# Stylish-TTS/stylish-tts

Measured on AMD Instinct MI355X. Metric: audio frames/sec/GPU (24 kHz) forward+backward; DDP scaling 1/2/4/8 MI355X, higher is better.
Workload: dtype bf16 GEMM operands, f32 accumulation/storage; 1 GPU; c3: B=32/GPU T=520 frames (6.5 s) L=100

## Files before the change

include/stylish_hip.h:

```cpp
#ifndef STYLISH_HIP_H
#define STYLISH_HIP_H

#include <stddef.h>
#include <stdint.h>

#ifdef __cplusplus
extern "C" {
#endif

typedef enum {
  STY_OK = 0,
  STY_EINVAL = -1,
  STY_ESHAPE = -2,
  STY_EHIP = -3,
  STY_ENOMEM = -4,
  STY_ESTATE = -5
} sty_status;

typedef struct sty_model sty_model;

int sty_version(void);
const char *sty_last_error(void);

int sty_model_create(const char *kind, sty_model **out);
void sty_model_destroy(sty_model *m);
int sty_model_bind(sty_model *m, const char *key, const float *ptr, int ndim, const int64_t *shape);
int sty_model_finalize(sty_model *m);
int sty_model_num_keys(const sty_model *m);
const char *sty_model_key(const sty_model *m, int i);
int sty_model_prepare(sty_model *m, void *stream);
int sty_model_invalidate(sty_model *m);

typedef struct {
  int B, T;
  const float *mel, *style, *pitch, *voiced, *noise, *prior_override;
  uint64_t seed;
  float *audio;
  float *tap_conformer_out;
  float *tap_prior;
  float *tap_har_spec;
  float *tap_har_phase;
  float *tap_logamp_prior;
  float *tap_phase_prior;
  float *tap_trunk;
  float *tap_logamp;
} sty_vocoder_io;
int sty_vocoder_workspace_bytes(const sty_model *m, int B, int T, size_t *bytes);
int sty_vocoder_fwd(sty_model *m, const sty_vocoder_io *io, void *workspace, size_t ws_bytes, void *stream);

typedef struct {
  int B, L, T;
  const int64_t *texts, *text_lengths;
  const float *alignment, *pitch, *energy, *voiced, *style, *denormal_pitch, *noise, *prior_override;
  uint64_t seed;
  float *audio;
  float *tap_text_encoding;
  float *tap_decoder_out;
  sty_vocoder_io voc_taps;
  void *style_stream;
} sty_speech_io;
int sty_speech_workspace_bytes(const sty_model *m, int B, int L, int T, size_t *bytes);
int sty_speech_fwd(sty_model *m, const sty_speech_io *io, void *workspace, size_t ws_bytes, void *stream);

int sty_style_workspace_bytes(const sty_model *m, int B, int T, size_t *bytes);
int sty_style_fwd(sty_model *m, int B, int T, const float *mel, float *style, void *workspace, size_t ws_bytes,
                  void *stream);

int sty_mel_workspace_bytes(int B, int N, int n_fft, int hop, size_t *bytes);
int sty_mel_fwd(int B, int N, const float *audio, int n_fft, int win_length, int hop, float mean, float std,
                float *mel, float *energy, void *workspace, size_t ws_bytes, void *stream);

int sty_multispec_workspace_bytes(int B, int N, size_t *bytes);
int sty_multispec_fwd(int B, int N, const float *audio, float *const *mag, float *const *phase,
                      float *const *fft_mag, void *workspace, size_t ws_bytes, void *stream);

int sty_alignment_fwd(int B, int L, int T, const float *durations, float *alignment, void *stream);

int sty_duration_workspace_bytes(const sty_model *m, int B, int L, size_t *bytes);
int sty_duration_fwd(sty_model *m, int B, int L, const int64_t *texts, const int64_t *text_lengths, const float *style,
                     float *dur_pred, void *workspace, size_t ws_bytes, void *stream);
int sty_pitch_energy_workspace_bytes(const sty_model *m, int B, int L, int T, size_t *bytes);
int sty_pitch_energy_fwd(sty_model *m, int B, int L, int T, const int64_t *texts, const int64_t *text_lengths,
                         const float *alignment, const float *style, float *pitch, float *energy, void *workspace,
                         size_t ws_bytes, void *stream);

int sty_pitch_style_workspace_bytes(const sty_model *m, int B, int T, size_t *bytes);
int sty_pitch_style_fwd(sty_model *m, int B, int T, const float *mel, const float *pitch, const float *energy,
                        float *style, void *workspace, size_t ws_bytes, void *stream);

int sty_aligner_workspace_bytes(const sty_model *m, int B, int T, size_t *bytes);
int sty_aligner_fwd(sty_model *m, int B, int T, const float *mel, const int64_t *mel_lengths, float *log_probs,
                    void *workspace, size_t ws_bytes, void *stream);
int sty_forced_align_workspace_bytes(int B, int T, int U, size_t *bytes);
int sty_forced_align(int B, int T, int V1, int U, const float *log_probs, const int64_t *targets,
                     const int64_t *input_lengths, const int64_t *target_lengths, int blank, int32_t *labels,
                     float *scores, int32_t *status, void *workspace, size_t ws_bytes, void *stream);

int sty_aligner_train_workspace_bytes(sty_model *m, int B, int T, size_t *bytes);
int sty_aligner_fwd_train(sty_model *m, int B, int T, const float *mel, const int64_t *mel_lengths, float drop_p,
                          unsigned drop_seed, float *log_probs, void *workspace, size_t ws_bytes, void *stream);
int sty_aligner_bwd(sty_model *m, const float *d_logits, void *stream);
int sty_ctc_loss_workspace_bytes(int B, int T, int V1, int U, size_t *bytes);
int sty_ctc_loss_fwd_bwd(int B, int T, int V1, int U, const float *log_probs, const float *log_priors, float prior_scale,
                         const int64_t *targets, const int64_t *input_lengths, const int64_t *target_lengths, int blank,
                         float weight, double *nll, float *loss, int32_t *status, float *d_logits, void *workspace,
                         size_t ws_bytes, void *stream);

int sty_convnext_fwd(sty_model *m, const char *prefix, int B, int C, int T, const float *x, const float *style,
                     float *y, void *workspace, size_t ws_bytes, void *stream);
int sty_resblock_fwd(sty_model *m, const char *prefix, int B, int T, const float *x, const float *style, float *y,
                     void *workspace, size_t ws_bytes, void *stream);
int sty_block_train_workspace_bytes(sty_model *m, const char *kind, const char *prefix, int B, int C, int T,
                                    size_t *bytes);
int sty_block_fwd_bwd(sty_model *m, const char *kind, const char *prefix, int B, int C, int T, const float *x,
                      const float *style, const float *gy, float *y, float *gx, float *d_style, void *workspace,
                      size_t ws_bytes, void *stream);
int sty_attention_workspace_bytes(int B, int H, int T, size_t *bytes);
int sty_attention_fwd_bwd(int B, int H, int DH, int T, const float *q, const float *k, const float *v,
                          const int64_t *lengths, const float *d_o, float *o, float *dq, float *dk, float *dv,
                          void *workspace, size_t ws_bytes, void *stream);
int sty_stft64_fwd(int B, int N, const float *wave, float *spec, float *phase, void *stream);
void sty_stft64_bases_host(float *out);
int sty_istft64_fwd(int B, int F, const float *logamp, const float *real, const float *imag, float *audio,
                    void *stream);
int sty_source_fwd(int B, int T, const float *pitch, const float *voiced, const float *noise, uint64_t seed,
                   const float *lin_w, const float *lin_b, float *prior, void *workspace, size_t ws_bytes,
                   void *stream);
int sty_source_workspace_bytes(int B, int T, size_t *bytes);

int sty_model_enable_training(sty_model *m);
typedef struct {
  int bn_batch_stats;
  int sn_power_iter;
  int f0_smooth;
  int energy_smooth;
  float bn_momentum;
  unsigned dropout_seed;
  float text_dropout;
  int compute_bf16;
  int frozen;
  float block_dropout;
} sty_train_opts;
int sty_model_set_train_opts(sty_model *m, const sty_train_opts *opts);

typedef void (*sty_grad_hook)(void *user, int segment);
int sty_model_set_grad_hook(sty_model *m, sty_grad_hook hook, void *user);
int sty_model_bind_grad(sty_model *m, const char *key, float *grad);
int sty_vocoder_train_workspace_bytes(sty_model *m, int B, int T, size_t *bytes);
int sty_vocoder_fwd_train(sty_model *m, const sty_vocoder_io *io, void *workspace, size_t ws_bytes, void *stream);
int sty_vocoder_bwd(sty_model *m, const float *d_audio, float *d_mel, float *d_style, void *stream);
int sty_speech_train_workspace_bytes(sty_model *m, int B, int L, int T, size_t *bytes);
int sty_speech_fwd_train(sty_model *m, const sty_speech_io *io, void *workspace, size_t ws_bytes, void *stream);
int sty_speech_bwd(sty_model *m, const float *d_audio, float *d_style, float *d_energy, void *stream);
int sty_speech_prepare_train(sty_model *m, void *stream);
int sty_speech_bwd_pe(sty_model *m, const float *d_audio, float *d_style, float *d_pitch, float *d_energy, void *stream);
int sty_speech_d_style_ready(sty_model *m, void *stream);
int sty_speech_branch_stream(sty_model *m, void **stream);
int sty_style_train_workspace_bytes(sty_model *m, int B, int T, size_t *bytes);
int sty_style_fwd_train(sty_model *m, int B, int T, const float *mel, float *style, void *workspace, size_t ws_bytes,
                        void *stream);
int sty_style_bwd(sty_model *m, const float *d_style, void *stream);
int sty_style_prepare_train(sty_model *m, void *stream);
int sty_style_tap(sty_model *m, int index, int grad, float *dst, int *C, int *H, int *W, void *stream);
int sty_pitch_loss_fwd_bwd(int B, int T, const float *target, const float *pred, float weight, int normalize,
                           float *loss, float *d_pred, void *workspace, size_t ws_bytes, void *stream);
int sty_prediction_to_duration(int B, int L, int NC, const float *pred, const int64_t *text_lengths,
                               const float *class_table, float *duration, void *stream);
int sty_duration_loss_fwd_bwd(int B, int L, int NC, const float *pred, const int64_t *text_lengths,
                              const float *target_dur, const int64_t *target_class, const float *class_table,
                              const float *ce_weight, float w_duration, float w_ce, const float *d_duration_extra,
                              float *losses, float *d_pred, void *workspace, size_t ws_bytes, void *stream);
int sty_duration_train_workspace_bytes(sty_model *m, int B, int L, size_t *bytes);
int sty_duration_fwd_train(sty_model *m, int B, int L, const int64_t *texts, const int64_t *text_lengths,
                           const float *style, float *out, void *workspace, size_t ws_bytes, void *stream);
int sty_duration_bwd(sty_model *m, const float *d_out, float *d_style, void *stream);
int sty_pitch_energy_train_workspace_bytes(sty_model *m, int B, int L, int T, size_t *bytes);
int sty_pitch_energy_fwd_train(sty_model *m, int B, int L, int T, const int64_t *texts, const int64_t *text_lengths,
                               const float *alignment, const float *style, float *pitch, float *energy, void *workspace,
                               size_t ws_bytes, void *stream);
int sty_pitch_energy_bwd(sty_model *m, const float *d_pitch, const float *d_energy, float *d_style, void *stream);
int sty_pitch_style_train_workspace_bytes(sty_model *m, int B, int T, size_t *bytes);
int sty_pitch_style_fwd_train(sty_model *m, int B, int T, const float *mel, const float *pitch, const float *energy,
                              float *style, void *workspace, size_t ws_bytes, void *stream);

int sty_conv1d_workspace_bytes(int Cout, int Cin, int K, size_t *bytes);
int sty_conv1d_fwd(int B, int Cin, int Cout, int K, int dil, int T, const float *x, const float *w, const float *bias,
                   float *y, void *workspace, size_t ws_bytes, int compute_bf16, void *stream);
int sty_conv1d_bwd_workspace_bytes(int B, int Cin, int Cout, int K, int T, size_t *bytes);
int sty_conv1d_bwd(int B, int Cin, int Cout, int K, int dil, int T, const float *x, const float *w, const float *gy,
                   float *dw, float *dbias, float *dx, void *workspace, size_t ws_bytes, int compute_bf16,
                   void *stream);
int sty_partial_sum(int dw_form, const float *part, int C, int K, int nblk, float *dw, float *db, void *stream);

int sty_adamw_step(size_t n, float *p, const float *g, float *m, float *v, float lr, float beta1, float beta2,
                   float eps, float weight_decay, int step, float grad_scale, void *stream);
int sty_adamw_step_scaled(size_t n, float *p, const float *g, float *m, float *v, double lr, const double *lr_mult,
                          float beta1, float beta2, float eps, float weight_decay, int step, float grad_scale,
                          void *stream);
int sty_disc_lr_track(double *state, const float *loss, double ideal_loss, double f_max, double h_min, double x_max,
                      double x_min, void *stream);

int sty_acoustic_loss_workspace_bytes(int B, int N, size_t *bytes);
int sty_acoustic_loss_target(int B, int N, const float *audio_gt, void *workspace, size_t ws_bytes, void *stream);
int sty_acoustic_loss_fwd_bwd(int B, int N, const float *audio_gt, const float *audio_pred, float w_mel,
                              float w_phase, float *losses, float *d_audio_pred, void *workspace, size_t ws_bytes,
                              void *stream);

typedef struct {
  const float *g[10];
  const float *v[10];
  const float *bias[10];
} sty_specdisc_params;
typedef struct {
  float *g[10];
  float *v[10];
  float *bias[10];
} sty_specdisc_grads;
int sty_specdisc_workspace_bytes(int B, int H, int W, int with_grads, size_t *bytes);
int sty_specdisc_forward(const sty_specdisc_params *p, int B, int H, int W, const float *x, float *scores,
                         int compute_bf16, void *workspace, size_t ws_bytes, void *stream);
int sty_specdisc_losses(const sty_specdisc_params *p, int B, int H, int W, const float *target, const float *pred,
                        float gen_scale, float *gen_loss, float *d_pred, float disc_scale, float *disc_loss,
                        const sty_specdisc_grads *grads, int compute_bf16, void *workspace, size_t ws_bytes,
                        void *stream);

int sty_pitchdisc_workspace_bytes(int B, int dim_in, int kernel, int T, int with_grads, size_t *bytes);
int sty_pitchdisc_forward(const sty_specdisc_params *p, int B, int dim_in, int kernel, int T, const float *x,
                          float *scores, void *workspace, size_t ws_bytes, void *stream);
int sty_pitchdisc_losses(const sty_specdisc_params *p, int B, int dim_in, int kernel, int T, const float *target,
                         const float *pred, float gen_scale, float *gen_loss, float *d_pred, float disc_scale,
                         float *disc_loss, const sty_specdisc_grads *grads, void *workspace, size_t ws_bytes,
                         void *stream);

typedef struct {
  const float *conv_w[12];
  const float *conv_b[12];
  const float *bn_w[9];
  const float *bn_b[9];
  float *bn_rm[9];
  float *bn_rv[9];
} sty_cfdisc_params;
typedef struct {
  float *conv_w[12];
  float *conv_b[12];
  float *bn_w[9];
  float *bn_b[9];
} sty_cfdisc_grads;
int sty_cfdisc_workspace_bytes(int B, int N, int with_grads, size_t *bytes);
int sty_cfdisc_forward(const sty_cfdisc_params *p, int B, int N, const float *x, float *scores, float bn_momentum,
                       int compute_bf16, void *workspace, size_t ws_bytes, void *stream);
int sty_cfdisc_losses(const sty_cfdisc_params *p, int B, int N, const float *target, const float *pred, float gen_scale,
                      float *gen_loss, float *d_pred, float disc_scale, float *disc_loss, const sty_cfdisc_grads *grads,
                      float bn_momentum, int compute_bf16, void *workspace, size_t ws_bytes, void *stream);

int sty_acoustic_gan_workspace_bytes(int B, int N, int with_grads, size_t *bytes);
int sty_acoustic_gan_loss_fwd_bwd(int B, int N, const float *audio_gt, const float *audio_pred, float w_mel,
                                  float w_phase, float w_gen, const sty_specdisc_params *mrd, float disc_scale,
                                  const sty_specdisc_grads *mrd_grads, int step_mask, float *losses, float *gan_losses,
                                  float *d_audio_pred, void *workspace, size_t ws_bytes, void *gan_workspace,
                                  size_t gan_ws_bytes, int compute_bf16, void *stream);

typedef struct sty_comm sty_comm;
int sty_comm_unique_id(void *id128);
int sty_comm_init(const void *id128, int rank, int world, int stream_priority, sty_comm **out);
int sty_comm_allreduce_bucket(sty_comm *c, float *buf, size_t n, void *producer_stream);
int sty_comm_wait(sty_comm *c, void *consumer_stream);
int sty_comm_set_stream(sty_comm *c, void *stream);
int sty_comm_stats(sty_comm *c, uint64_t *buckets, uint64_t *reduce_scatter_all_gather, double *bytes);
int sty_comm_destroy(sty_comm *c);

int sty_pack_accumulate(int n, int D, int rows, const float *styles, const int64_t *text_lengths, double *sums,
                        int64_t *counts, void *stream);
int sty_pack_finalize(int rows, int D, const double *sums, const int64_t *counts, const int32_t *lo, const int32_t *hi,
                      float *pack, void *stream);

typedef struct {
  char name[48];
  char inst[144];
  uint64_t launches;
  double ms;
  double flops;
// ... 12 lines not shown
```

stylish_tts_amd/csrc/api.hip:

```cpp
#include <math.h>
#include <stdarg.h>
#include <string.h>
#include <stdlib.h>
#include <cxxabi.h>

#include <map>
#include <string>

#include "model.h"

namespace sty {

static thread_local char g_err[1024] = "";
void set_error(const char* fmt, ...) {
  va_list ap;
  va_start(ap, fmt);
  vsnprintf(g_err, sizeof(g_err), fmt, ap);
  va_end(ap);
}
int hip_fail(hipError_t e, const char* what) {
  set_error("HIP error %d (%s) at %s", (int)e, hipGetErrorString(e), what);
  return STY_EHIP;
}

// ... 2426 lines not shown
  PackedConv pc;
  pc.Cin = Cin;
  pc.Cout = Cout;
  pc.K = K;
  pc.CinP = (int)align_up(Cin, CI_CHUNK);
  pc.CoutP = (int)align_up(Cout, 32);
  float* wp = reinterpret_cast<float*>(align_up(reinterpret_cast<size_t>(workspace), 256));
  float* bp = wp + (size_t)K * pc.CinP * pc.CoutP;
  STY_HIP(hipMemsetAsync(wp, 0, ((size_t)K * pc.CinP * pc.CoutP + pc.CoutP) * sizeof(float), S(stream)));
  rc = launch_pack_conv(w, nullptr, nullptr, bias, Cout, Cin, K, wp, bp, pc.CinP, pc.CoutP, S(stream));
  if (rc) return rc;
  pc.wp = wp;
  pc.bias = bias ? bp : nullptr;
  ConvArgs a;
  a.x[0] = x;
  a.xc[0] = Cin;
  a.nsrc = 1;
  a.B = B;
  a.T = T;
  a.w = pc;
  a.dil = dil;
  a.pad = (K - 1) * dil / 2;
  a.y = y;
  a.bf16 = compute_bf16 != 0;
  if (compute_bf16 == 2) {
    const size_t tw = ((size_t)B * (Cin + Cout) * T) * sizeof(__bf16) + 512;
    if (ws_bytes < need + tw) {
      set_error("sty_conv1d_fwd: compute_bf16 = 2 needs %zu more workspace bytes for the operand twins", tw);
      return STY_EINVAL;
    }
    __bf16* x16 = reinterpret_cast<__bf16*>(align_up(reinterpret_cast<size_t>(static_cast<char*>(workspace) + need), 256));
    if ((rc = launch_twin_cast(x, nullptr, PRO_NONE, B, Cin, T, x16, S(stream)))) return rc;
    a.x16 = x16;
    a.y16 = x16 + (size_t)B * Cin * T;
    a.y16_act = PRO_LRELU;
  }
  return launch_conv1d(a, S(stream));
}
static PackedConv unit_conv_dims(int Cin, int Cout, int K) {
  PackedConv pc;
  pc.Cin = Cin;
  pc.Cout = Cout;
  pc.K = K;
  pc.CinP = (int)align_up(Cin, CI_CHUNK);
  pc.CoutP = (int)align_up(Cout, 32);
  return pc;
}
int sty_conv1d_bwd_workspace_bytes(int B, int Cin, int Cout, int K, int T, size_t* bytes) {
  if (!bytes || B <= 0 || Cin <= 0 || Cout <= 0 || K <= 0 || T <= 0) {
    set_error("sty_conv1d_bwd_workspace_bytes: bad argument");
    return STY_EINVAL;
  }
  const PackedConv pc = unit_conv_dims(Cin, Cout, K);
  const size_t plane = (size_t)K * pc.CinP * pc.CoutP + pc.CoutP;
  *bytes = (3 * plane + wgrad_partial_floats(pc, B, T)) * sizeof(float) + 1024;
  *bytes += (size_t)B * (Cin + Cout) * T * sizeof(__bf16) + 512;
  return STY_OK;
}
int sty_conv1d_bwd(int B, int Cin, int Cout, int K, int dil, int T, const float* x, const float* w, const float* gy,
                   float* dw, float* dbias, float* dx, void* workspace, size_t ws_bytes, int compute_bf16,
                   void* stream) {
  size_t need = 0;
  int rc = sty_conv1d_bwd_workspace_bytes(B, Cin, Cout, K, T, &need);
  if (rc) return rc;
  if (!x || !w || !gy || !dw || !workspace || dil <= 0 || (K - 1) * dil > 128 || ws_bytes < need) {
    set_error("sty_conv1d_bwd: bad argument, halo > 128 or workspace too small");
    return STY_EINVAL;
  }
  hipStream_t st = S(stream);
  PackedConv pc = unit_conv_dims(Cin, Cout, K);
  const size_t plane = (size_t)K * pc.CinP * pc.CoutP;
  float* wp = reinterpret_cast<float*>(align_up(reinterpret_cast<size_t>(workspace), 256));
  float* bp = wp + plane;
  float* gwp = bp + pc.CoutP;
  float* gbp = gwp + plane;
  PackedConv pd;
  pd.Cin = Cout;
  pd.Cout = Cin;
  pd.K = K;
  pd.CinP = pc.CoutP;
  pd.CoutP = pc.CinP;
  float* wd = gbp + pc.CoutP;
  float* partial = wd + plane + pc.CoutP;
  STY_HIP(hipMemsetAsync(wp, 0, (size_t)(partial - wp) * sizeof(float), st));
  rc = launch_pack_conv(w, nullptr, nullptr, nullptr, Cout, Cin, K, wp, bp, pc.CinP, pc.CoutP, st);
  if (rc) return rc;
  pc.wp = wp;
  pc.bias = dbias ? bp : nullptr;
  ConvArgs a;
  a.x[0] = x;
  a.xc[0] = Cin;
  a.nsrc = 1;
  a.B = B;
  a.T = T;
  a.w = pc;
  a.dil = dil;
  a.pad = (K - 1) * dil / 2;
  a.bf16 = compute_bf16 != 0;
  if (compute_bf16 == 3) {
    if (dx || T % 2) {
      set_error("sty_conv1d_bwd: a two-byte x (compute_bf16 = 3) is for dw / dbias only (dx == NULL), T even");
      return STY_EINVAL;
    }
    a.xh = 1;
  }
  if (compute_bf16 == 2) {
    __bf16* x16 = reinterpret_cast<__bf16*>(align_up(reinterpret_cast<size_t>(partial + wgrad_partial_floats(pc, B, T)), 256));
    __bf16* g16 = x16 + (size_t)B * Cin * T;
    if ((rc = launch_twin_cast(x, nullptr, PRO_NONE, B, Cin, T, x16, st))) return rc;
    if ((rc = launch_twin_cast(gy, nullptr, PRO_NONE, B, Cout, T, g16, st))) return rc;
    a.x16 = x16;
    a.g16 = g16;
  }
  bool bias_done = false;
  rc = launch_conv1d_wgrad(a, gy, nullptr, 1.0f, gwp, partial, dbias ? gbp : nullptr, &bias_done, st);
  if (rc) return rc;
  if (dbias && !bias_done) {
    set_error("sty_conv1d_bwd: this conv's bias gradient is a separate pass (launch_bias_grad), not wired here");
    return STY_EINVAL;
  }
  STY_HIP(hipMemsetAsync(dw, 0, (size_t)Cout * Cin * K * sizeof(float), st));
  rc = launch_unpack_grad(gwp, nullptr, nullptr, Cout, Cin, K, pc.CinP, pc.CoutP, dw, nullptr, nullptr, st);
  if (rc) return rc;
  if (dbias) STY_HIP(hipMemcpyAsync(dbias, gbp, (size_t)Cout * sizeof(float), hipMemcpyDeviceToDevice, st));
  if (dx) {
    PackedConv pdm = pd;
    rc = launch_pack_dgrad(wp, K, pc.CinP, pc.CoutP, wd, st);
    if (rc) return rc;
    pdm.wp = wd;
    pdm.bias = nullptr;
    ConvArgs d;
    d.x[0] = gy;
    d.xc[0] = Cout;
    d.nsrc = 1;
    d.B = B;
    d.T = T;
    d.w = pdm;
    d.dil = dil;
    d.pad = (K - 1) * dil - a.pad;
    d.bf16 = a.bf16;
    d.y = dx;
    d.x16 = a.g16;
    rc = launch_conv1d(d, st);
  }
  return rc;
}
int sty_partial_sum(int dw_form, const float* part, int C, int K, int nblk, float* dw, float* db, void* stream) {
  if (!part || !db || C <= 0 || nblk <= 0 || (dw_form && (!dw || K <= 0))) {
    set_error("sty_partial_sum: bad argument");
    return STY_EINVAL;
  }
  return launch_partial_sum(dw_form, part, C, K, nblk, dw, db, S(stream));
}
int sty_mel_workspace_bytes(int B, int N, int n_fft, int hop, size_t* bytes) {
  if (!bytes || B <= 0 || N <= n_fft / 2 || n_fft <= 0 || hop <= 0) {
    set_error("sty_mel_workspace_bytes: bad argument");
    return STY_EINVAL;
  }
  *bytes = mel_workspace_floats(B, N, n_fft, hop, 80) * sizeof(float);
  return STY_OK;
}
int sty_mel_fwd(int B, int N, const float* audio, int n_fft, int win_length, int hop, float mean, float std_,
                float* mel, float* energy, void* workspace, size_t ws_bytes, void* stream) {
  if (!audio || !mel || !workspace || B <= 0 || N <= n_fft / 2 || win_length > n_fft || hop <= 0 || std_ == 0.f) {
    set_error("sty_mel_fwd: bad argument");
    return STY_EINVAL;
  }
  if (ws_bytes < mel_workspace_floats(B, N, n_fft, hop, 80) * sizeof(float)) {
    set_error("sty_mel_fwd: workspace too small");
    return STY_ENOMEM;
  }
  return launch_mel(B, N, audio, n_fft, win_length, hop, 80, 24000, mean, std_, mel, energy, (float*)workspace,
                    S(stream));
}
int sty_multispec_workspace_bytes(int B, int N, size_t* bytes) {
  if (!bytes || B <= 0 || N <= 1024) {
    set_error("sty_multispec_workspace_bytes: bad argument");
    return STY_EINVAL;
  }
  size_t mx = 0;
  const int res[3][2] = {{512, 128}, {1024, 256}, {2048, 512}};
  for (auto& r : res) {
    const size_t n = multispec_workspace_floats(B, N, r[0], r[1]);
    mx = n > mx ? n : mx;
  }
  *bytes = mx * sizeof(float);
  return STY_OK;
}
int sty_multispec_fwd(int B, int N, const float* audio, float* const* mag, float* const* phase, float* const* fft_mag,
                      void* workspace, size_t ws_bytes, void* stream) {
  if (!audio || !mag || !fft_mag || !workspace || B <= 0 || N <= 1024) {
    set_error("sty_multispec_fwd: bad argument");
    return STY_EINVAL;
  }
  size_t need = 0;
  int rc = sty_multispec_workspace_bytes(B, N, &need);
  if (rc) return rc;
  if (ws_bytes < need) {
    set_error("sty_multispec_fwd: workspace too small");
    return STY_ENOMEM;
  }
  const int res[3][2] = {{512, 128}, {1024, 256}, {2048, 512}};
  for (int i = 0; i < 3; ++i) {
    rc = launch_multispec_single(B, N, audio, res[i][0], res[i][1], 24000, mag[i], phase ? phase[i] : nullptr,
                                 fft_mag[i], (float*)workspace, S(stream));
    if (rc) return rc;
  }
  return STY_OK;
}

int sty_acoustic_loss_workspace_bytes(int B, int N, size_t* bytes) {
  if (!bytes || B <= 0 || N <= 1024) {
    set_error("sty_acoustic_loss_workspace_bytes: bad argument");
    return STY_EINVAL;
  }
  *bytes = acoustic_loss_workspace_floats(B, N) * sizeof(float);
  return STY_OK;
}
int sty_acoustic_loss_fwd_bwd(int B, int N, const float* audio_gt, const float* audio_pred, float w_mel, float w_phase,
                              float* losses, float* d_audio_pred, void* workspace, size_t ws_bytes, void* stream) {
  if (!audio_pred || !losses || !d_audio_pred || !workspace || B <= 0 || N <= 1024) {
    set_error("sty_acoustic_loss_fwd_bwd: bad argument");
    return STY_EINVAL;
  }
  if (ws_bytes < acoustic_loss_workspace_floats(B, N) * sizeof(float)) {
    set_error("sty_acoustic_loss_fwd_bwd: workspace too small");
    return STY_ENOMEM;
  }
  return launch_acoustic_loss(B, N, audio_gt, audio_pred, w_mel, w_phase, losses, d_audio_pred, (float*)workspace,
                              S(stream));
}

int sty_acoustic_loss_target(int B, int N, const float* audio_gt, void* workspace, size_t ws_bytes, void* stream) {
  if (!audio_gt || !workspace || B <= 0 || N <= 1024) {
    set_error("sty_acoustic_loss_target: bad argument");
    return STY_EINVAL;
  }
  if (ws_bytes < acoustic_loss_workspace_floats(B, N) * sizeof(float)) {
    set_error("sty_acoustic_loss_target: workspace too small");
    return STY_ENOMEM;
  }
  return launch_acoustic_loss(B, N, audio_gt, nullptr, 0.f, 0.f, nullptr, nullptr, (float*)workspace, S(stream));
}

int sty_acoustic_gan_workspace_bytes(int B, int N, int with_grads, size_t* bytes) {
  if (!bytes || B <= 0 || N <= 1024) {
    set_error("sty_acoustic_gan_workspace_bytes: bad argument");
    return STY_EINVAL;
  }
  *bytes = acoustic_gan_workspace_bytes(B, N, with_grads);
  return STY_OK;
}
int sty_acoustic_gan_loss_fwd_bwd(int B, int N, const float* audio_gt, const float* audio_pred, float w_mel, float w_phase,
                                  float w_gen, const sty_specdisc_params* mrd, float disc_scale,
                                  const sty_specdisc_grads* mrd_grads, int step_mask, float* losses, float* gan_losses,
                                  float* d_audio_pred, void* workspace, size_t ws_bytes, void* gan_workspace,
                                  size_t gan_ws_bytes, int compute_bf16, void* stream) {
  if (!audio_pred || !losses || !gan_losses || !d_audio_pred || !workspace || !gan_workspace || !mrd ||
      B <= 0 || N <= 1024 || (step_mask && !mrd_grads)) {
    set_error("sty_acoustic_gan_loss_fwd_bwd: bad argument");
    return STY_EINVAL;
  }
  if (ws_bytes < acoustic_loss_workspace_floats(B, N) * sizeof(float) ||
      gan_ws_bytes < acoustic_gan_workspace_bytes(B, N, step_mask != 0)) {
    set_error("sty_acoustic_gan_loss_fwd_bwd: workspace too small");
    return STY_ENOMEM;
  }
  AcousticGan gan;
  for (int r = 0; r < 3; ++r) {
    for (int i = 0; i < 10; ++i)
      if (!mrd[r].g[i] || !mrd[r].v[i] || !mrd[r].bias[i] ||
          (((step_mask >> r) & 1) && (!mrd_grads[r].g[i] || !mrd_grads[r].v[i] || !mrd_grads[r].bias[i]))) {
        set_error("sty_acoustic_gan_loss_fwd_bwd: null parameter / gradient pointer (discriminator %d, conv %d)", r, i);
        return STY_EINVAL;
      }
    gan.p[r] = &mrd[r];
    gan.g[r] = ((step_mask >> r) & 1) ? &mrd_grads[r] : nullptr;
  }
  gan.w_gen = w_gen;
  gan.disc_scale = disc_scale;
  gan.out = gan_losses;
  gan.bf16 = compute_bf16;
  gan.ws = gan_workspace;
  gan.ws_bytes = gan_ws_bytes;
  STY_HIP(hipMemsetAsync(gan_losses, 0, 7 * sizeof(float), S(stream)));
  return launch_acoustic_loss_gan(B, N, audio_gt, audio_pred, w_mel, w_phase, losses, d_audio_pred, (float*)workspace, &gan,
                                  S(stream));
}

}
```

stylish_tts_amd/csrc/bwd.hip:

```cpp
#include "sty_common.h"

namespace sty {

__device__ __forceinline__ double wave_sum(double v) {
  for (int o = 32; o > 0; o >>= 1) v += __shfl_xor(v, o);
  return v;
}

template <int N>
__device__ __forceinline__ void block_sum(double (&v)[N], double (*red)[4]) {
  const int lane = threadIdx.x & 63, wave = threadIdx.x >> 6;
#pragma unroll
  for (int i = 0; i < N; ++i) {
    v[i] = wave_sum(v[i]);
    if (lane == 0) red[i][wave] = v[i];
  }
  __syncthreads();
  if (threadIdx.x == 0) {
#pragma unroll
    for (int i = 0; i < N; ++i) v[i] = red[i][0] + red[i][1] + red[i][2] + red[i][3];
  }
}

__global__ __launch_bounds__(256) void pro_bwd_kernel(int mode_, const float* __restrict__ u, int Cu, int cu0,
// ... 151 lines not shown
    const bool big = __any(amax > 8192.0f);
    if (hw && !big) {
#pragma unroll
      for (int e = 0; e < 8; ++e) {
        float sn, cs;
        sty_sincos_hw(al * z[e], sn, cs);
        fin(e, sn, cs);
      }
    } else if (!big) {
#pragma unroll
      for (int e = 0; e < 8; ++e) {
        float sn, cs;
        sty_sincos_fast(al * z[e], sn, cs);
        fin(e, sn, cs);
      }
    } else {
#pragma unroll
      for (int e = 0; e < 8; ++e) {
        float sn, cs;
        sty_sincos(al * z[e], sn, cs);
        fin(e, sn, cs);
      }
    }
  };
  double acc[3] = {0.0, 0.0, 0.0};
  for (int i = threadIdx.x; i < n8; i += 256) {
    float uv[8], xv[8];
    ld8_any(u, r8 + i, uh != 0, uv);
    ld8_any(x, r8 + i, xh != 0, xv);
    float p0 = 0.f, p1 = 0.f, p2 = 0.f, g[8], dal[8];
    deriv8(uv, xv, g, dal);
#pragma unroll
    for (int e = 0; e < 8; ++e) {
      p0 = fmaf(g[e], xv[e], p0);
      p1 += g[e];
      p2 += dal[e];
    }
    acc[0] += (double)p0;
    acc[1] += (double)p1;
    acc[2] += (double)p2;
  }
  block_sum<3>(acc, red);
  if (threadIdx.x == 0) {
    const float mu = mean[row], r = rstd[row], g1 = 1.f + gb[(size_t)b * 2 * C + c];
    const float dA = (float)acc[0], dS = (float)acc[1];
    dgb[(size_t)b * 2 * C + c] += r * (dA - mu * dS);
    dgb[(size_t)b * 2 * C + C + c] += dS;
    const float dmu = -(g1 * r) * dS, dr = g1 * (dA - mu * dS);
    const float k1 = -dr * r * r * r / (float)T;
    cc[1] = k1;
    cc[0] = dmu / (float)T - k1 * mu;
    if (dalpha) atomicAdd(&dalpha[c], (float)acc[2]);
  }
  __syncthreads();
  const float c0 = cc[0], c1 = cc[1];
  for (int i = n8 - 1 - (int)threadIdx.x; i >= 0; i -= 256) {
    float uv[8], xv[8], d[8];
    ld8_any(u, r8 + i, uh != 0, uv);
    ld8_any(x, r8 + i, xh != 0, xv);
    if (accumulate) {
      ld8_any(dsrc ? dsrc : dx, r8 + i, dh != 0, d);
    } else {
#pragma unroll
      for (int e = 0; e < 8; ++e) d[e] = 0.f;
    }
    float g[8], dal[8];
    deriv8(uv, xv, g, dal);
#pragma unroll
    for (int e = 0; e < 8; ++e) d[e] += fmaf(g[e], a, fmaf(c1, xv[e], c0));
    st8_any(dx, r8 + i, dh != 0, d);
  }
}
int launch_pro_bwd_adain(const void* u, int uh, const void* x, int xh, int B, int C, int T, const float* pa, const float* ps,
                         const float* alpha, const float* mean, const float* rstd, const float* gb, void* dx, int dh,
                         int accumulate, float* dgb, float* dalpha, int hw, hipStream_t st, const void* dsrc) {
  if (T % 8 != 0 || ((((size_t)u | (size_t)x | (size_t)dx | (size_t)dsrc) & 15) != 0)) {
    set_error("pro_bwd_adain: T %% 8 != 0 or unaligned rows");
    return STY_EINVAL;
  }
  char detail[40];
  snprintf(detail, sizeof(detail), "C%d T%d acc%d h%d%d%d", C, T, accumulate, uh, xh, dh);
  const double n = (double)B * C * T;
  ProfScope prof("pro_bwd_adain_kernel", 0.0, n * (2.0 * ((uh ? 2 : 4) + (xh ? 2 : 4)) + (accumulate ? 2.0 : 1.0) * (dh ? 2 : 4)), st,
                 detail);
  hipLaunchKernelGGL(pro_bwd_adain_kernel, dim3(C, B), dim3(256), 0, st, u, uh, x, xh, C, T, pa, ps, alpha, mean, rstd, gb, dx,
                     dh, accumulate, dgb, dalpha, hw, dsrc);
  STY_LAUNCH_CHECK();
  return STY_OK;
}

__global__ void adain_fold_bwd_kernel(const float* __restrict__ da, const float* __restrict__ ds,
                                      const float* __restrict__ mean, const float* __restrict__ rstd,
                                      const float* __restrict__ gb, int B, int C, int T, float* __restrict__ dgb,
                                      float* __restrict__ c0, float* __restrict__ c1) {
  const int i = blockIdx.x * blockDim.x + threadIdx.x;
  if (i >= B * C) return;
  const int b = i / C, c = i % C;
  const float mu = mean[i], r = rstd[i], g1 = 1.f + gb[(size_t)b * 2 * C + c];
  const float dA = da[i], dS = ds[i];
  const float a = g1 * r;
  dgb[(size_t)b * 2 * C + c] += r * (dA - mu * dS);
  dgb[(size_t)b * 2 * C + C + c] += dS;
  const float dmu = -a * dS, dr = g1 * (dA - mu * dS);
  const float k1 = -dr * r * r * r / (float)T;
  c1[i] = k1;
  c0[i] = dmu / (float)T - k1 * mu;
}
int launch_adain_fold_bwd(const float* da, const float* ds, const float* mean, const float* rstd, const float* gb, int B,
                          int C, int T, float* dgb, float* c0, float* c1, hipStream_t st) {
  hipLaunchKernelGGL(adain_fold_bwd_kernel, dim3(cdiv(B * C, 256)), dim3(256), 0, st, da, ds, mean, rstd, gb, B, C, T,
                     dgb, c0, c1);
  STY_LAUNCH_CHECK();
  return STY_OK;
}

__global__ void row_axpb_kernel(const float* __restrict__ x, const float* __restrict__ c0,
                                const float* __restrict__ c1, int T, float* __restrict__ dx) {
  const int t = blockIdx.x * 256 + threadIdx.x, row = blockIdx.y;
  if (t >= T) return;
  const size_t o = (size_t)row * T + t;
  dx[o] += c0[row] + c1[row] * x[o];
}
__global__ __launch_bounds__(256) void row_axpb4_kernel(const float* __restrict__ x, const float* __restrict__ c0,
                                                        const float* __restrict__ c1, unsigned T4, unsigned n4,
                                                        float* __restrict__ dx) {
  const unsigned idx = blockIdx.x * 256u + threadIdx.x;
  if (idx >= n4) return;
  const unsigned row = idx / T4;
  const float a = c0[row], b = c1[row];
  const float4 xv = reinterpret_cast<const float4*>(x)[idx];
  float4 d = reinterpret_cast<float4*>(dx)[idx];
  d.x += a + b * xv.x;
  d.y += a + b * xv.y;
  d.z += a + b * xv.z;
  d.w += a + b * xv.w;
  reinterpret_cast<float4*>(dx)[idx] = d;
}
static inline bool vec4_ok(size_t n4, int T, const void* p0, const void* p1, const void* p2 = nullptr) {
  return T % 4 == 0 && n4 < ((size_t)1 << 31) && ((((size_t)p0 | (size_t)p1 | (size_t)p2) & 15) == 0);
}
int launch_row_axpb(const float* x, const float* c0, const float* c1, int rows, int T, float* dx, hipStream_t st) {
  const size_t n4 = (size_t)rows * (T / 4);
  if (vec4_ok(n4, T, x, dx)) {
    hipLaunchKernelGGL(row_axpb4_kernel, dim3((unsigned)((n4 + 255) / 256)), dim3(256), 0, st, x, c0, c1, (unsigned)(T / 4),
                       (unsigned)n4, dx);
    STY_LAUNCH_CHECK();
    return STY_OK;
  }
  hipLaunchKernelGGL(row_axpb_kernel, dim3(cdiv(T, 256), rows), dim3(256), 0, st, x, c0, c1, T, dx);
  STY_LAUNCH_CHECK();
  return STY_OK;
}

__global__ __launch_bounds__(256) void adain_stats_kernel(const double* __restrict__ part, int nseg, int rows, int T,
                                                          float eps, float* __restrict__ mean, float* __restrict__ rstd) {
  const int i = blockIdx.x * 4 + (threadIdx.x >> 6), lane = threadIdx.x & 63;
  if (i >= rows) return;
  double sum = 0.0, sq = 0.0;
  for (int k = lane; k < nseg; k += 64) {
    sum += part[((size_t)i * nseg + k) * 2];
    sq += part[((size_t)i * nseg + k) * 2 + 1];
  }
  for (int o = 32; o > 0; o >>= 1) {
    sum += __shfl_xor(sum, o);
    sq += __shfl_xor(sq, o);
  }
  if (lane) return;
  const double m = sum / T;
  double var = sq / T - m * m;
  if (var < 0.0) var = 0.0;
  mean[i] = (float)m;
  rstd[i] = (float)(1.0 / sqrt(var + (double)eps));
}
int launch_adain_stats(const double* part, int nseg, int rows, int T, float eps, float* mean, float* rstd,
                       hipStream_t st) {
  hipLaunchKernelGGL(adain_stats_kernel, dim3(cdiv(rows, 4)), dim3(256), 0, st, part, nseg, rows, T, eps, mean, rstd);
  STY_LAUNCH_CHECK();
  return STY_OK;
}

template <int TC, int NR>
__global__ __launch_bounds__(256) void chan_ln_bwd_dx_reg_kernel(const float* __restrict__ x, const float* __restrict__ dy,
                                                                 const float* __restrict__ y, int C, int T, float eps,
                                                                 int ada, const float* __restrict__ w,
                                                                 const float* __restrict__ gb, int relu,
                                                                 const float* __restrict__ out_mask,
                                                                 float* __restrict__ dx, int accumulate,
                                                                 float* __restrict__ mu_out, float* __restrict__ r_out) {
  constexpr int CG = 256 / TC;
  __shared__ float red[2][CG][TC];
  const int col = threadIdx.x % TC, cg = threadIdx.x / TC;
  const int t = blockIdx.x * TC + col, b = blockIdx.y;
  const bool in = t < T;
  const size_t base = (size_t)b * C * T + (in ? t : 0);
  auto combine = [&](float a, float bb, float& ra, float& rb) {
    red[0][cg][col] = a;
    red[1][cg][col] = bb;
    __syncthreads();
    float s0 = 0.f, s1 = 0.f;
#pragma unroll
    for (int k = 0; k < CG; ++k) {
      s0 += red[0][k][col];
      s1 += red[1][k][col];
    }
    __syncthreads();
    ra = s0;
    rb = s1;
  };
  const float om = (in && out_mask) ? out_mask[(size_t)b * T + t] : 1.f;
  float xr[NR], gr[NR];
#pragma unroll
  for (int i = 0; i < NR; ++i) {
    const int c = cg + i * CG;
    xr[i] = gr[i] = 0.f;
    if (in && c < C) {
      const size_t o = base + (size_t)c * T;
      xr[i] = x[o];
      float g = dy[o] * om;
      if (relu && !(y[o] > 0.f)) g = 0.f;
      const float A = ada ? 1.f + gb[(size_t)b * 2 * C + c] : w[c];
      gr[i] = g * A;
    }
  }
  float p0 = 0.f, p1 = 0.f, mean, dummy;
#pragma unroll
  for (int i = 0; i < NR; ++i)
    if (in && cg + i * CG < C) p0 += xr[i];
  combine(p0, 0.f, mean, dummy);
  mean /= (float)C;
  p0 = 0.f;
#pragma unroll
  for (int i = 0; i < NR; ++i)
    if (in && cg + i * CG < C) {
      const float d = xr[i] - mean;
      p0 += d * d;
    }
  float var;
  combine(p0, 0.f, var, dummy);
  const float r = 1.0f / sqrtf(var / (float)C + eps);
  p0 = p1 = 0.f;
#pragma unroll
  for (int i = 0; i < NR; ++i)
    if (in && cg + i * CG < C) {
      const float dxh = gr[i], xh = (xr[i] - mean) * r;
      p0 += dxh;
      p1 += dxh * xh;
    }
  float s1, s2;
  combine(p0, p1, s1, s2);
  s1 /= (float)C;
  s2 /= (float)C;
  if (!in) return;
#pragma unroll
  for (int i = 0; i < NR; ++i) {
    const int c = cg + i * CG;
    if (c < C) {
      const size_t o = base + (size_t)c * T;
      const float xh = (xr[i] - mean) * r;
      const float d = r * (gr[i] - s1 - xh * s2);
      dx[o] = accumulate ? dx[o] + d : d;
    }
  }
  if (cg == 0) {
    mu_out[(size_t)b * T + t] = mean;
    r_out[(size_t)b * T + t] = r;
  }
}
template <int TC>
__global__ __launch_bounds__(256) void chan_ln_bwd_dx_kernel(const float* __restrict__ x, const float* __restrict__ dy,
                                                             const float* __restrict__ y, int C, int T, float eps,
                                                             int ada, const float* __restrict__ w,
                                                             const float* __restrict__ gb, int relu,
                                                             const float* __restrict__ out_mask,
                                                             float* __restrict__ dx, int accumulate,
                                                             float* __restrict__ mu_out, float* __restrict__ r_out) {
  constexpr int CG = 256 / TC;
  __shared__ float red[2][CG][TC];
  const int col = threadIdx.x % TC, cg = threadIdx.x / TC;
  const int t = blockIdx.x * TC + col, b = blockIdx.y;
  const bool in = t < T;
  const size_t base = (size_t)b * C * T + (in ? t : 0);
  auto combine = [&](float a, float bb, float& ra, float& rb) {
    red[0][cg][col] = a;
    red[1][cg][col] = bb;
    __syncthreads();
    float s0 = 0.f, s1 = 0.f;
#pragma unroll
    for (int k = 0; k < CG; ++k) {
      s0 += red[0][k][col];
      s1 += red[1][k][col];
    }
    __syncthreads();
    ra = s0;
    rb = s1;
  };
  float p0 = 0.f, p1 = 0.f, mean, dummy;
  if (in)
    for (int c = cg; c < C; c += CG) p0 += x[base + (size_t)c * T];
  combine(p0, 0.f, mean, dummy);
  mean /= (float)C;
  p0 = 0.f;
  if (in)
    for (int c = cg; c < C; c += CG) {
      const float d = x[base + (size_t)c * T] - mean;
      p0 += d * d;
    }
  float var;
  combine(p0, 0.f, var, dummy);
  const float r = 1.0f / sqrtf(var / (float)C + eps);
  const float om = (in && out_mask) ? out_mask[(size_t)b * T + t] : 1.f;
  p0 = p1 = 0.f;
  if (in)
    for (int c = cg; c < C; c += CG) {
      const size_t o = base + (size_t)c * T;
      float g = dy[o] * om;
      if (relu && !(y[o] > 0.f)) g = 0.f;
      const float A = ada ? 1.f + gb[(size_t)b * 2 * C + c] : w[c];
      const float dxh = g * A, xh = (x[o] - mean) * r;
      p0 += dxh;
      p1 += dxh * xh;
    }
  float s1, s2;
  combine(p0, p1, s1, s2);
  s1 /= (float)C;
  s2 /= (float)C;
  if (!in) return;
  for (int c = cg; c < C; c += CG) {
    const size_t o = base + (size_t)c * T;
    float g = dy[o] * om;
    if (relu && !(y[o] > 0.f)) g = 0.f;
    const float A = ada ? 1.f + gb[(size_t)b * 2 * C + c] : w[c];
    const float xh = (x[o] - mean) * r;
    const float d = r * (g * A - s1 - xh * s2);
// ... 23 lines not shown
    const float xh = (x[row + t] - mu[(size_t)b * T + t]) * r[(size_t)b * T + t];
    acc[0] += (double)g * xh;
    acc[1] += (double)g;
  }
  block_sum<2>(acc, red);
  if (threadIdx.x == 0) {
    if (ada) {
      dgb[(size_t)b * 2 * C + c] += (float)acc[0];
      dgb[(size_t)b * 2 * C + C + c] += (float)acc[1];
    } else {
      atomicAdd(&dw[c], (float)acc[0]);
      atomicAdd(&db[c], (float)acc[1]);
    }
  }
}
__global__ __launch_bounds__(256) void chan_ln32_bwd_kernel(const void* __restrict__ x, const void* __restrict__ dy, int T,
                                                            float eps, int ada, const float* __restrict__ w,
                                                            const float* __restrict__ gb, const float* __restrict__ out_mask,
                                                            void* __restrict__ dx, int accumulate, float* __restrict__ part,
                                                            int h16) {
  __shared__ float A_s[32];
  __shared__ float red[64];
  const int tid = threadIdx.x, b = blockIdx.y;
  const int t = blockIdx.x * 256 + tid;
  const bool in = t < T;
  if (tid < 32) A_s[tid] = ada ? 1.f + gb[(size_t)b * 64 + tid] : w[tid];
  if (tid < 64) red[tid] = 0.f;
  __syncthreads();
  const size_t base = (size_t)b * 32 * T + (in ? t : 0);
  float xv[32], gv[32];
#pragma unroll
  for (int c = 0; c < 32; ++c) {
    xv[c] = in ? sty_ld_any(x, base + (size_t)c * T, h16 & 1) : 0.f;
    gv[c] = in ? sty_ld_any(dy, base + (size_t)c * T, h16 & 2) : 0.f;
  }
  const float om = (in && out_mask) ? out_mask[(size_t)b * T + t] : 1.f;
  float mean = 0.f;
#pragma unroll
  for (int c = 0; c < 32; ++c) mean += xv[c];
  mean *= (1.0f / 32.0f);
  float var = 0.f;
#pragma unroll
  for (int c = 0; c < 32; ++c) {
    xv[c] -= mean;
    var = fmaf(xv[c], xv[c], var);
  }
  const float r = 1.0f / sqrtf(var * (1.0f / 32.0f) + eps);
  float s1 = 0.f, s2 = 0.f;
#pragma unroll
  for (int c = 0; c < 32; ++c) {
    xv[c] *= r;
    gv[c] *= om;
    const float dxh = gv[c] * A_s[c];
    s1 += dxh;
    s2 = fmaf(dxh, xv[c], s2);
  }
  s1 *= (1.0f / 32.0f);
  s2 *= (1.0f / 32.0f);
  if (in) {
#pragma unroll
    for (int c = 0; c < 32; ++c) {
      const float d = r * (gv[c] * A_s[c] - s1 - xv[c] * s2);
      if (h16 & 4) {
        sty_st_any(dx, base + (size_t)c * T, d, true);
      } else {
        float* o = reinterpret_cast<float*>(dx) + base + (size_t)c * T;
        *o = accumulate ? *o + d : d;
      }
    }
  }
#pragma unroll
  for (int c = 0; c < 32; ++c) {
    const float a0 = sty_half_sum_to_lane31(gv[c] * xv[c]);
    const float a1 = sty_half_sum_to_lane31(gv[c]);
    if ((tid & 31) == 31) {
      atomicAdd(&red[c], a0);
      atomicAdd(&red[32 + c], a1);
    }
  }
  __syncthreads();
  if (tid < 64) part[((size_t)b * gridDim.x + blockIdx.x) * 64 + tid] = red[tid];
}
__global__ __launch_bounds__(64) void chan_ln32_param_sum_kernel(const float* __restrict__ part, int B, int nblk, int ada,
                                                                 float* __restrict__ dgb, float* __restrict__ dw,
                                                                 float* __restrict__ db) {
  const int i = blockIdx.x, lane = threadIdx.x;
  const int slot = ada ? (i & 63) : i, b0 = ada ? i >> 6 : 0, nb = ada ? 1 : B;
  double s = 0.0;
  for (int b = b0; b < b0 + nb; ++b)
    for (int k = lane; k < nblk; k += 64) s += (double)part[((size_t)b * nblk + k) * 64 + slot];
  s = wave_sum(s);
  if (lane == 0) {
    if (ada)
      dgb[(size_t)b0 * 64 + slot] += (float)s;
    else if (slot < 32)
      dw[slot] += (float)s;
    else
      db[slot - 32] += (float)s;
  }
}

__global__ void cast_any_kernel(const void* __restrict__ x, size_t n, void* __restrict__ y, int to16) {
  const size_t i = (size_t)blockIdx.x * 256 + threadIdx.x;
  if (i < n) sty_st_any(y, i, sty_ld_any(x, i, !to16), to16);
}
int launch_cast_f32_to_16(const float* x, size_t n, void* y16, hipStream_t st) {
  hipLaunchKernelGGL(cast_any_kernel, dim3((unsigned)((n + 255) / 256)), dim3(256), 0, st, x, n, y16, 1);
  STY_LAUNCH_CHECK();
  return STY_OK;
}
int launch_cast_16_to_f32(const void* x16, size_t n, float* y, hipStream_t st) {
  hipLaunchKernelGGL(cast_any_kernel, dim3((unsigned)((n + 255) / 256)), dim3(256), 0, st, x16, n, y, 0);
  STY_LAUNCH_CHECK();
  return STY_OK;
}
bool chan_ln32_eligible(int B, int C, int T, int relu) {
  return C == 32 && !relu && (size_t)B * T >= 65536 && getenv("STY_NO_LN32_BWD") == nullptr;
}
int launch_chan_ln_bwd(const float* x, const float* dy, const float* y, int B, int C, int T, float eps, int ada,
                       const float* w, const float* gb, int relu, const float* out_mask, float* dx, int accumulate,
                       float* mu_tmp, float* r_tmp, float* dgb, float* dw, float* db, hipStream_t st, int h16) {
  const bool no32 = getenv("STY_NO_LN32_BWD") != nullptr;
  if (C == 32 && !relu && (size_t)B * T >= 65536 && !no32) {
    const int nblk = cdiv(T, 256);
    if ((h16 & 4) && accumulate) {
      set_error("chan_ln_bwd: a two-byte dx cannot be accumulated into");
      return STY_EINVAL;
    }
    hipLaunchKernelGGL(chan_ln32_bwd_kernel, dim3(nblk, B), dim3(256), 0, st, x, dy, T, eps, ada, w, gb, out_mask, dx, accumulate,
                       mu_tmp, h16);
    hipLaunchKernelGGL(chan_ln32_param_sum_kernel, dim3(ada ? B * 64 : 64), dim3(64), 0, st, mu_tmp, B, nblk, ada, dgb, dw, db);
    STY_LAUNCH_CHECK();
    return STY_OK;
  }
  if (h16) {
    set_error("chan_ln_bwd: two-byte tensors only on the C = 32 long-row kernel (chan_ln32_eligible)");
    return STY_EINVAL;
  }
  if ((size_t)B * T < 65536 && C <= 256)
    hipLaunchKernelGGL((chan_ln_bwd_dx_reg_kernel<16, 16>), dim3(cdiv(T, 16), B), dim3(256), 0, st, x, dy, y, C, T, eps, ada, w,
                       gb, relu, out_mask, dx, accumulate, mu_tmp, r_tmp);
  else if ((size_t)B * T >= 65536)
    hipLaunchKernelGGL(chan_ln_bwd_dx_kernel<64>, dim3(cdiv(T, 64), B), dim3(256), 0, st, x, dy, y, C, T, eps, ada, w, gb,
                       relu, out_mask, dx, accumulate, mu_tmp, r_tmp);
  else
    hipLaunchKernelGGL(chan_ln_bwd_dx_kernel<16>, dim3(cdiv(T, 16), B), dim3(256), 0, st, x, dy, y, C, T, eps, ada, w, gb,
                       relu, out_mask, dx, accumulate, mu_tmp, r_tmp);
  hipLaunchKernelGGL(chan_ln_bwd_param_kernel, dim3(C, B), dim3(256), 0, st, x, dy, y, mu_tmp, r_tmp, C, T, ada, relu,
                     out_mask, dgb, dw, db);
  STY_LAUNCH_CHECK();
  return STY_OK;
}

__global__ __launch_bounds__(256) void grn_bwd_kernel(const double* __restrict__ part, int nseg,
                                                      const float* __restrict__ gamma,
                                                      const float* __restrict__ ds, int C4,
                                                      float* __restrict__ coef, float* __restrict__ dgamma) {
  __shared__ float gxs[1024];
  __shared__ double red[2][4];
  const int b = blockIdx.x;
  if (nseg < 32) {
    for (int c = threadIdx.x; c < C4; c += 256) {
      double sq = 0.0;
      for (int k = 0; k < nseg; ++k) sq += part[(((size_t)b * C4 + c) * nseg + k) * 2 + 1];
      gxs[c] = (float)sqrt(sq);
    }
  } else {
    const int lane = threadIdx.x & 63, wave = threadIdx.x >> 6;
    for (int c = wave; c < C4; c += 4) {
      const double* pp = part + ((size_t)b * C4 + c) * nseg * 2 + 1;
      double sq = 0.0;
      for (int k = lane; k < nseg; k += 64) sq += pp[(size_t)k * 2];
      for (int o = 32; o > 0; o >>= 1) sq += __shfl_xor(sq, o);
      if (lane == 0) gxs[c] = (float)sqrt(sq);
    }
  }
  __syncthreads();
  double acc[1] = {0.0};
  for (int c = threadIdx.x; c < C4; c += 256) acc[0] += gxs[c];
  __shared__ float mean_s, dot_s;
  block_sum<1>(acc, red);
  if (threadIdx.x == 0) mean_s = (float)(acc[0] / C4);
  __syncthreads();
  const float m = mean_s + 1e-6f;
  double d2[1] = {0.0};
  for (int c = threadIdx.x; c < C4; c += 256) {
    const float dnx = ds[(size_t)b * C4 + c] * gamma[c];
    d2[0] += (double)dnx * gxs[c];
    atomicAdd(&dgamma[c], ds[(size_t)b * C4 + c] * (gxs[c] / m));
  }
  __syncthreads();
  block_sum<1>(d2, red);
  if (threadIdx.x == 0) dot_s = (float)d2[0];
  __syncthreads();
  for (int c = threadIdx.x; c < C4; c += 256) {
    const float dnx = ds[(size_t)b * C4 + c] * gamma[c];
    const float dgx = dnx / m - dot_s / (m * m) / (float)C4;
    coef[(size_t)b * C4 + c] = gxs[c] > 0.f ? dgx / gxs[c] : 0.f;
  }
}
int launch_grn_bwd(const double* part, int nseg, const float* gamma, const float* ds, int B, int C4, float* coef,
                   float* dgamma, hipStream_t st) {
  if (C4 > 1024) {
    set_error("grn_bwd: 4C > 1024");
    return STY_EINVAL;
  }
  hipLaunchKernelGGL(grn_bwd_kernel, dim3(B), dim3(256), 0, st, part, nseg, gamma, ds, C4, coef, dgamma);
  STY_LAUNCH_CHECK();
  return STY_OK;
}

__global__ void act_fwd_kernel(int kind, const float* __restrict__ x, const float* __restrict__ alpha, int C, int T,
                               float* __restrict__ y) {
  const int t = blockIdx.x * 256 + threadIdx.x, c = blockIdx.y, b = blockIdx.z;
  if (t >= T) return;
  if (kind == ACT_GLU) {
    const float a = x[((size_t)b * 2 * C + c) * T + t], g = x[((size_t)b * 2 * C + C + c) * T + t];
    y[((size_t)b * C + c) * T + t] = a / (1.f + expf(-g));
    return;
  }
  const size_t o = ((size_t)b * C + c) * T + t;
  const float v = x[o];
  float r = v;
  if (kind == ACT_RELU) r = fmaxf(v, 0.f);
  else if (kind == ACT_SWISH) r = v / (1.f + expf(-v));
  else if (kind == ACT_SNAKE) r = sty_snake(v, alpha[c], 1.f / alpha[c]);
  else if (kind == 100) r = tanhf(v);
  else if (kind == ACT_GELU) r = 0.5f * v * (1.0f + erff(v * 0.70710678118654752f));
  y[o] = r;
}
__device__ __forceinline__ float act_apply1(int kind, float v, float al, float ral) {
  float r = v;
  if (kind == ACT_RELU) r = fmaxf(v, 0.f);
  else if (kind == ACT_SWISH) r = v / (1.f + expf(-v));
  else if (kind == ACT_SNAKE) r = sty_snake(v, al, ral);
  else if (kind == 100) r = tanhf(v);
  else if (kind == ACT_GELU) r = 0.5f * v * (1.0f + erff(v * 0.70710678118654752f));
  return r;
}
__global__ __launch_bounds__(256) void act_fwd4_kernel(int kind, const float* __restrict__ x, const float* __restrict__ alpha,
                                                       unsigned C, unsigned T4, unsigned n4, float* __restrict__ y) {
  const unsigned idx = blockIdx.x * 256u + threadIdx.x;
  if (idx >= n4) return;
  float al = 1.f, ral = 1.f;
  if (kind == ACT_SNAKE) {
    al = alpha[(idx / T4) % C];
    ral = 1.f / al;
  }
  const float4 v = reinterpret_cast<const float4*>(x)[idx];
  float4 r;
  r.x = act_apply1(kind, v.x, al, ral);
  r.y = act_apply1(kind, v.y, al, ral);
  r.z = act_apply1(kind, v.z, al, ral);
  r.w = act_apply1(kind, v.w, al, ral);
  reinterpret_cast<float4*>(y)[idx] = r;
}
int launch_act_fwd(int kind, const float* x, const float* alpha, int B, int C, int T, float* y, hipStream_t st) {
  const size_t n4 = (size_t)B * C * (T / 4);
  if (kind != ACT_GLU && T % 4 == 0 && n4 < ((size_t)1 << 31) && ((((size_t)x | (size_t)y) & 15) == 0)) {
    hipLaunchKernelGGL(act_fwd4_kernel, dim3((unsigned)((n4 + 255) / 256)), dim3(256), 0, st, kind, x, alpha, (unsigned)C,
                       (unsigned)(T / 4), (unsigned)n4, y);
    STY_LAUNCH_CHECK();
    return STY_OK;
  }
  hipLaunchKernelGGL(act_fwd_kernel, dim3(cdiv(T, 256), C, B), dim3(256), 0, st, kind, x, alpha, C, T, y);
  STY_LAUNCH_CHECK();
  return STY_OK;
}
__global__ __launch_bounds__(256) void act_bwd_kernel(int kind, const float* __restrict__ x,
                                                      const float* __restrict__ dy, const float* __restrict__ alpha,
                                                      int C, int T, float* __restrict__ dx, int accumulate,
                                                      float* __restrict__ dalpha) {
  __shared__ double red[1][4];
  const int c = blockIdx.x, b = blockIdx.y;
  double acc[1] = {0.0};
  if (kind == ACT_GLU) {
    const size_t ra = ((size_t)b * 2 * C + c) * T, rg = ((size_t)b * 2 * C + C + c) * T, ro = ((size_t)b * C + c) * T;
    for (int t = threadIdx.x; t < T; t += 256) {
      const float a = x[ra + t], g = x[rg + t], d = dy[ro + t];
      const float sg = 1.f / (1.f + expf(-g));
      const float da = d * sg, dg = d * a * sg * (1.f - sg);
      dx[ra + t] = accumulate ? dx[ra + t] + da : da;
      dx[rg + t] = accumulate ? dx[rg + t] + dg : dg;
    }
    return;
  }
  const size_t row = ((size_t)b * C + c) * T;
  const float al = kind == ACT_SNAKE ? alpha[c] : 1.f;
  auto one = [&](float v, float d) -> float {
    float g = d;
    if (kind == ACT_RELU) g = v > 0.f ? d : 0.f;
    else if (kind == ACT_SWISH) {
      const float sg = 1.f / (1.f + expf(-v));
      g = d * (sg + v * sg * (1.f - sg));
    } else if (kind == ACT_SNAKE) {
      float sn, cs;
      sty_sincos(al * v, sn, cs);
      const float s2 = sn * sn, s2a = 2.f * sn * cs;
      g = d * (1.f + s2a);
      acc[0] += (double)(d * (v * s2a - s2 / al) / al);
    } else if (kind == 100) {
      const float th = tanhf(v);
      g = d * (1.f - th * th);
    } else if (kind == ACT_GELU) {
      g = d * (0.5f * (1.0f + erff(v * 0.70710678118654752f)) + v * 0.3989422804014327f * expf(-0.5f * v * v));
    }
    return g;
  };
  if ((T & 3) == 0 && ((((size_t)(x + row) | (size_t)(dy + row) | (size_t)(dx + row)) & 15) == 0)) {
    const float4* x4 = reinterpret_cast<const float4*>(x + row);
    const float4* d4 = reinterpret_cast<const float4*>(dy + row);
    float4* o4 = reinterpret_cast<float4*>(dx + row);
    for (int t = threadIdx.x; t < T / 4; t += 256) {
      const float4 v = x4[t], d = d4[t];
      float4 g;
      g.x = one(v.x, d.x);
      g.y = one(v.y, d.y);
      g.z = one(v.z, d.z);
      g.w = one(v.w, d.w);
      if (accumulate) {
        const float4 o = o4[t];
        g = make_float4(o.x + g.x, o.y + g.y, o.z + g.z, o.w + g.w);
      }
      o4[t] = g;
    }
  } else
  for (int t = threadIdx.x; t < T; t += 256) {
    const float v = x[row + t], d = dy[row + t];
    float g = d;
    if (kind == ACT_RELU) g = v > 0.f ? d : 0.f;
    else if (kind == ACT_SWISH) {
      const float sg = 1.f / (1.f + expf(-v));
      g = d * (sg + v * sg * (1.f - sg));
    } else if (kind == ACT_SNAKE) {
      float sn, cs;
      sty_sincos(al * v, sn, cs);
      const float s2 = sn * sn, s2a = 2.f * sn * cs;
      g = d * (1.f + s2a);
      acc[0] += (double)(d * (v * s2a - s2 / al) / al);
    } else if (kind == 100) {
      const float th = tanhf(v);
      g = d * (1.f - th * th);
    } else if (kind == ACT_GELU) {
      g = d * (0.5f * (1.0f + erff(v * 0.70710678118654752f)) + v * 0.3989422804014327f * expf(-0.5f * v * v));
    }
    dx[row + t] = accumulate ? dx[row + t] + g : g;
  }
  if (kind == ACT_SNAKE && dalpha) {
    block_sum<1>(acc, red);
    if (threadIdx.x == 0) atomicAdd(&dalpha[c], (float)acc[0]);
  }
}
int launch_act_bwd(int kind, const float* x, const float* dy, const float* alpha, int B, int C, int T, float* dx,
                   int accumulate, float* dalpha, hipStream_t st) {
  hipLaunchKernelGGL(act_bwd_kernel, dim3(C, B), dim3(256), 0, st, kind, x, dy, alpha, C, T, dx, accumulate, dalpha);
  STY_LAUNCH_CHECK();
  return STY_OK;
}

__global__ void row_scale_add_kernel(const float* __restrict__ src, const float* __restrict__ coef, float k, int T,
                                     float* __restrict__ dst) {
  const int t = blockIdx.x * 256 + threadIdx.x, row = blockIdx.y;
  if (t >= T) return;
  const size_t o = (size_t)row * T + t;
  dst[o] += src[o] * (coef ? coef[row] : k);
}
__global__ __launch_bounds__(256) void row_scale_add4_kernel(const float* __restrict__ src, const float* __restrict__ coef,
                                                             float k, unsigned T4, unsigned n4, float* __restrict__ dst) {
  const unsigned idx = blockIdx.x * 256u + threadIdx.x;
  if (idx >= n4) return;
  const float f = coef ? coef[idx / T4] : k;
  const float4 sv = reinterpret_cast<const float4*>(src)[idx];
  float4 d = reinterpret_cast<float4*>(dst)[idx];
  d.x += sv.x * f;
  d.y += sv.y * f;
  d.z += sv.z * f;
  d.w += sv.w * f;
  reinterpret_cast<float4*>(dst)[idx] = d;
}
int launch_row_scale_add(const float* src, const float* coef, float k, int rows, int T, float* dst, hipStream_t st) {
  const size_t n4 = (size_t)rows * (T / 4);
  if (vec4_ok(n4, T, src, dst)) {
    hipLaunchKernelGGL(row_scale_add4_kernel, dim3((unsigned)((n4 + 255) / 256)), dim3(256), 0, st, src, coef, k,
                       (unsigned)(T / 4), (unsigned)n4, dst);
    STY_LAUNCH_CHECK();
    return STY_OK;
  }
  hipLaunchKernelGGL(row_scale_add_kernel, dim3(cdiv(T, 256), rows), dim3(256), 0, st, src, coef, k, T, dst);
  STY_LAUNCH_CHECK();
  return STY_OK;
}

__global__ void dwconv_fwd_kernel(const float* __restrict__ x, const float* __restrict__ w,
                                  const float* __restrict__ bias, int C, int T, int K, int pad,
                                  float* __restrict__ y) {
  const int t = blockIdx.x * 256 + threadIdx.x, c = blockIdx.y, b = blockIdx.z;
  if (t >= T) return;
  const float* p = x + ((size_t)b * C + c) * T;
  float acc = bias ? bias[c] : 0.f;
  for (int k = 0; k < K; ++k) {
    const int tt = t - pad + k;
    if (tt >= 0 && tt < T) acc = fmaf(w[c * K + k], p[tt], acc);
  }
  y[((size_t)b * C + c) * T + t] = acc;
}
template <int MAXK>
__global__ __launch_bounds__(256) void dwconv_fwd4_kernel(const float* __restrict__ x, const float* __restrict__ w,
                                                          const float* __restrict__ bias, int C, int T, int K, int pad,
                                                          float* __restrict__ y) {
  const int t0 = (blockIdx.x * 256 + threadIdx.x) * 4, c = blockIdx.y, b = blockIdx.z;
  if (t0 >= T) return;
  const float* p = x + ((size_t)b * C + c) * T;
  float wk[MAXK];
#pragma unroll
  for (int k = 0; k < MAXK; ++k) wk[k] = k < K ? w[c * K + k] : 0.f;
  float g[MAXK + 3];
#pragma unroll
  for (int j = 0; j < MAXK + 3; ++j) {
    const int tt = t0 - pad + j;
    g[j] = (tt >= 0 && tt < T && j < K + 3) ? p[tt] : 0.f;
  }
  const float b0 = bias ? bias[c] : 0.f;
  float acc[4] = {b0, b0, b0, b0};
#pragma unroll
  for (int e = 0; e < 4; ++e)
#pragma unroll
    for (int k = 0; k < MAXK; ++k) acc[e] = fmaf(wk[k], g[e + k], acc[e]);
  const size_t o = ((size_t)b * C + c) * T + t0;
  if (t0 + 3 < T && (o & 3) == 0) {
    *reinterpret_cast<float4*>(y + o) = make_float4(acc[0], acc[1], acc[2], acc[3]);
  } else {
    for (int e = 0; e < 4 && t0 + e < T; ++e) y[o + e] = acc[e];
  }
}
__global__ __launch_bounds__(256) void dwconv7_fwd_kernel(const float* __restrict__ x, const float* __restrict__ w,
                                                          const float* __restrict__ bias, int C, int T4, unsigned ngroups,
                                                          float* __restrict__ y) {
  const unsigned idx = blockIdx.x * 256u + threadIdx.x;
  if (idx >= ngroups) return;
  const unsigned row = idx / (unsigned)T4;
  const int q = (int)(idx - row * (unsigned)T4), c = (int)(row % (unsigned)C);
  const float4* p4 = reinterpret_cast<const float4*>(x) + (size_t)row * T4;
  const float4 z = make_float4(0.f, 0.f, 0.f, 0.f);
  const float4 a = q > 0 ? p4[q - 1] : z, b = p4[q], d = q + 1 < T4 ? p4[q + 1] : z;
  const float g[12] = {a.x, a.y, a.z, a.w, b.x, b.y, b.z, b.w, d.x, d.y, d.z, d.w};
  float wk[7];
#pragma unroll
  for (int k = 0; k < 7; ++k) wk[k] = w[c * 7 + k];
  const float b0 = bias ? bias[c] : 0.f;
  float acc[4] = {b0, b0, b0, b0};
#pragma unroll
  for (int e = 0; e < 4; ++e)
#pragma unroll
    for (int k = 0; k < 7; ++k) acc[e] = fmaf(wk[k], g[e + 1 + k], acc[e]);
  reinterpret_cast<float4*>(y)[idx] = make_float4(acc[0], acc[1], acc[2], acc[3]);
}
int launch_dwconv_fwd(const float* x, const float* w, const float* bias, int B, int C, int T, int K, int pad, float* y,
                      hipStream_t st) {
  const size_t ng = (size_t)B * C * (T / 4);
  if (K == 7 && pad == 3 && T % 4 == 0 && ((((size_t)x | (size_t)y) & 15) == 0) && ng < ((size_t)1 << 31)) {
    hipLaunchKernelGGL(dwconv7_fwd_kernel, dim3((unsigned)((ng + 255) / 256)), dim3(256), 0, st, x, w, bias, C, T / 4, (unsigned)ng, y);
    STY_LAUNCH_CHECK();
    return STY_OK;
  }
  if (K <= 31) {
    if (K <= 7)
      hipLaunchKernelGGL(dwconv_fwd4_kernel<7>, dim3(cdiv(T, 1024), C, B), dim3(256), 0, st, x, w, bias, C, T, K, pad, y);
    else
      hipLaunchKernelGGL(dwconv_fwd4_kernel<31>, dim3(cdiv(T, 1024), C, B), dim3(256), 0, st, x, w, bias, C, T, K, pad, y);
    STY_LAUNCH_CHECK();
    return STY_OK;
  }
  hipLaunchKernelGGL(dwconv_fwd_kernel, dim3(cdiv(T, 256), C, B), dim3(256), 0, st, x, w, bias, C, T, K, pad, y);
  STY_LAUNCH_CHECK();
  return STY_OK;
}
template <int MAXK>
__global__ __launch_bounds__(256) void dwconv_bwd_dx_kernel(const float* __restrict__ dy, const float* __restrict__ w, int C,
                                                            int T, int K, int pad, float* __restrict__ dx, int accumulate,
                                                            const float* __restrict__ src) {
  const int t0 = (blockIdx.x * 256 + threadIdx.x) * 4, c = blockIdx.y, b = blockIdx.z;
  if (t0 >= T) return;
  const float* p = dy + ((size_t)b * C + c) * T;
  float wk[MAXK];
#pragma unroll
  for (int k = 0; k < MAXK; ++k) wk[k] = k < K ? w[c * K + k] : 0.f;
  float g[MAXK + 3];
  const int lo = t0 + pad - (MAXK - 1);
#pragma unroll
  for (int j = 0; j < MAXK + 3; ++j) {
    const int tt = lo + j;
    g[j] = (tt >= 0 && tt < T) ? p[tt] : 0.f;
  }
  float acc[4] = {0.f, 0.f, 0.f, 0.f};
#pragma unroll
  for (int e = 0; e < 4; ++e)
#pragma unroll
    for (int k = 0; k < MAXK; ++k) acc[e] = fmaf(wk[k], g[e + (MAXK - 1) - k], acc[e]);
  const size_t o = ((size_t)b * C + c) * T + t0;
  const bool wide = t0 + 3 < T && (o & 3) == 0;
  if (wide) {
    float4 r = make_float4(acc[0], acc[1], acc[2], acc[3]);
    if (src) {
      const float4 sv = *reinterpret_cast<const float4*>(src + o);
      r = make_float4(r.x + sv.x, r.y + sv.y, r.z + sv.z, r.w + sv.w);
    } else if (accumulate) {
      const float4 dv = *reinterpret_cast<const float4*>(dx + o);
      r = make_float4(r.x + dv.x, r.y + dv.y, r.z + dv.z, r.w + dv.w);
    }
    *reinterpret_cast<float4*>(dx + o) = r;
  } else {
    for (int e = 0; e < 4 && t0 + e < T; ++e)
      dx[o + e] = src ? src[o + e] + acc[e] : (accumulate ? dx[o + e] + acc[e] : acc[e]);
  }
}
__global__ __launch_bounds__(256) void dwconv7_bwd_dx_kernel(const float* __restrict__ dy, const float* __restrict__ w, int C,
                                                             int T4, unsigned ngroups, float* __restrict__ dx, int accumulate,
                                                             const float* __restrict__ src) {
  const unsigned idx = blockIdx.x * 256u + threadIdx.x;
  if (idx >= ngroups) return;
  const unsigned row = idx / (unsigned)T4;
  const int q = (int)(idx - row * (unsigned)T4), c = (int)(row % (unsigned)C);
  const float4* p4 = reinterpret_cast<const float4*>(dy) + (size_t)row * T4;
  const float4 z = make_float4(0.f, 0.f, 0.f, 0.f);
  const float4 a = q > 0 ? p4[q - 1] : z, b = p4[q], d = q + 1 < T4 ? p4[q + 1] : z;
  const float g[12] = {a.x, a.y, a.z, a.w, b.x, b.y, b.z, b.w, d.x, d.y, d.z, d.w};
  float wk[7];
#pragma unroll
  for (int k = 0; k < 7; ++k) wk[k] = w[c * 7 + k];
  float acc[4] = {0.f, 0.f, 0.f, 0.f};
#pragma unroll
  for (int e = 0; e < 4; ++e)
#pragma unroll
// ... 502 lines not shown
```

stylish_tts_amd/csrc/model.h:

```cpp
#pragma once
#include <string>
#include <unordered_map>
#include <vector>

#include "sty_common.h"
#include "weights.h"

namespace sty {

struct Param {
  const float* p = nullptr;
  std::vector<int64_t> shape;
};

int convnext32_ntiles(int T);
int launch_convnext32(const Cnx32Args& a, int B, int pass, hipStream_t st);
int launch_attention(const AttnArgs& a, int B, int DH, hipStream_t st);
int launch_rope_n(float* q, float* k, int B, int H, int DH, int L, int d, hipStream_t st, float sgn = 1.0f);
int launch_style_expand(const float* style, int B, int S, int L, float* y, hipStream_t st);
int launch_row_sum_add(const float* src, int rows, int L, float* dst, hipStream_t st);
int launch_wn_dw_bwd(const float* dw, const float* g, const float* v, int C, int K, float* dg, float* dv, hipStream_t st);
int launch_dur_post_bwd(const float* d, const float* mask, const float* go, int B, int NC, int L, float* gd, hipStream_t st);
int trainer_duration_forward(struct Trainer* t, int B, int L, const int64_t* texts, const int64_t* lengths, const float* style,
                             float* out, void* ws, size_t ws_bytes, hipStream_t st, size_t* need);
// ... 86 lines not shown

struct Conformer {
  AdaFc ff1n, ff2n, attn_n, conv_n, post_n;
  PackedConv ff1a, ff1b, ff2a, ff2b, to_q, to_kv, to_out, pw1, pw2;
  const float *dw_w, *dw_b, *bn_w, *bn_b, *bn_rm, *bn_rv;
};

struct VocoderPlan {
  PackedConv amp_input_conv;
  const float *amp_norm_w, *amp_norm_b;
  Conformer conf;
  std::vector<ConvNeXt> amp_convnext;
  PackedConv upconv[3];
  ConvNeXt upblock[3];
  const float *lin_w, *lin_b;
  const float *stft_fr, *stft_fi, *stft_br, *stft_bi;
  PackedConv amp_prior_conv, phase_prior_conv, phase_input_conv, amp_output_conv, real_conv, imag_conv;
  ResBlock32 amp_prior_block, phase_prior_block;
  const float *phase_norm_w, *phase_norm_b, *amp_fln_w, *amp_fln_b, *phase_fln_w, *phase_fln_b;
  std::vector<ConvNeXt> phase_convnext;
  int hidden = 256;
};

struct TextEncLayer {
  PackedConv q, k, v, o, f1, f2;
  const float *n1g, *n1b, *n2g, *n2b;
};
struct TextEncPlan {
  const float* emb = nullptr;
  int tokens = 0, H = 0;
  PackedConv pre[3], proj, proj_m;
  const float *pre_g[3], *pre_b[3];
  std::vector<TextEncLayer> layers;
  float theta[4];
};

struct DecBlock {
  int Cin = 0, Cout = 0;
  PackedConv c1, c2, sc;
  bool has_sc = false;
  AdaFc n1, n2;
};
struct DecoderPlan {
  DecBlock encode, decode[4];
  PackedConv asr_res;
  float* fnv_w = nullptr;
  const float *f0_g, *f0_v, *f0_b, *n_g, *n_v, *n_b, *v_g, *v_v, *v_b;
};

struct ProsodyLayer {
  PackedConv q, k, v, o, f1, f2, proj;
  AdaFc n1, n2;
};
struct DurationPlan {
  AdaFc qn, kn;
  PackedConv cq, ck, cv, co, post, proj;
  const float *dw_g = nullptr, *dw_v = nullptr, *dw_b = nullptr;
  std::vector<ConvNeXt> cnx;
  int classes = 16;
};
struct PitchEnergyPlan {
  std::vector<ProsodyLayer> layers;
  DecBlock f0[4], nn[4];
  PackedConv f0p, np;
  int heads = 2;
};

struct AlignerPlan {
  PackedConv tdnn[3], ffn[5], out;
  const float *rm[3] = {nullptr, nullptr, nullptr}, *rv[3] = {nullptr, nullptr, nullptr};
  float *bn_scale[3] = {nullptr, nullptr, nullptr}, *bn_shift[3] = {nullptr, nullptr, nullptr};
  float *bn_one = nullptr, *bn_zero = nullptr;
  int hidden = 640, n_mels = 80, classes = 179;
};
int launch_aligner_bn_prep(const float* mean, const float* var, int C, float eps, float* scale, float* shift, hipStream_t st);
int launch_aligner_bn(float* x, int B, int C, int T, const float* scale, const float* shift, hipStream_t st);
int launch_log_softmax_rows(const float* x, int B, int V, int T, float* out, hipStream_t st);
int launch_fill_f32(float* x, int n, float v, hipStream_t st);

struct Trainer;
struct StyleResBlk {
  int Cin = 0, Cout = 0;
  bool down = false, has_sc = false;
  PackedConv c1, c2, sc;
  const float* dw_w9 = nullptr;
  const float* dw_b = nullptr;
};
struct StylePlan {
  int n_mels = 80, style_dim = 64;
  PackedConv stem;
  StyleResBlk blk[4];
  PackedConv head;
  const float *fc_w = nullptr, *fc_b = nullptr;
};

}

struct sty_model {
  std::string kind;
  std::unordered_map<std::string, sty::Param> params;
  std::vector<std::string> requested;
  bool finalized = false, prepared = false;
  bool train_prepared = false;
  hipEvent_t prepared_ev = nullptr;
  int style_dim = 64;
  char* arena = nullptr;
  size_t arena_bytes = 0;
  sty::Bump ab;
  std::vector<sty::PackJob> jobs;
  std::vector<sty::StyleFcDesc> fcs;
  sty::StyleFcDesc* fcs_dev = nullptr;
  size_t gb_floats_per_batch = 0;
  std::string missing;
  sty::VocoderPlan voc;
  sty::TextEncPlan te;
  sty::DecoderPlan dec;
  sty::StylePlan sty_enc;
  sty::DurationPlan dur;
  sty::PitchEnergyPlan pe;
  sty::AlignerPlan ali;
  sty::PackedConv pse_pre;
  float* stft_default = nullptr;
  bool train_enabled = false;
  char* garena = nullptr;
  std::unordered_map<const float*, float*> pgrad;
  std::unordered_map<std::string, float*> pgrad_by_key;
  std::unordered_map<const float*, sty::PackedConv> dgrad;
  std::unordered_map<const float*, sty::PackedConv> plain_of;
  void* fcs_bwd_dev = nullptr;
  sty::WeightTables wt;
  size_t seg_job_split = 0;
  sty_grad_hook grad_hook = nullptr;
  void* grad_hook_user = nullptr;
  sty_train_opts topts = {0, 0, 0, 0, 0.1f, 0u, 0.2f, 0, 0};
  struct sty::Trainer* trainer = nullptr;
};

#include <functional>
#include <unordered_set>
namespace sty {
inline ConvRoute plan_route(const sty_model* m, ConvArgs a) {
  a.bf16 = m->topts.compute_bf16;
  return conv1d_route(a);
}
int launch_pro_bwd(int mode, const float* u, int Cu, int cu0, const float* x, int B, int C, int T, const float* pa,
                   const float* ps, int pC, int pc0, const float* alpha, const float* mask, float* dx, int accumulate,
                   float* dpa, float* dps, float* dalpha, hipStream_t st);
int launch_adain_fold_bwd(const float* da, const float* ds, const float* mean, const float* rstd, const float* gb, int B,
                          int C, int T, float* dgb, float* c0, float* c1, hipStream_t st);
int launch_row_axpb(const float* x, const float* c0, const float* c1, int rows, int T, float* dx, hipStream_t st);
int launch_pro_bwd_adain(const void* u, int uh, const void* x, int xh, int B, int C, int T, const float* pa, const float* ps,
                         const float* alpha, const float* mean, const float* rstd, const float* gb, void* dx, int dh,
                         int accumulate, float* dgb, float* dalpha, int hw, hipStream_t st, const void* dsrc = nullptr);
int launch_adain_stats(const double* part, int nseg, int rows, int T, float eps, float* mean, float* rstd,
                       hipStream_t st);
int launch_cast_f32_to_16(const float* x, size_t n, void* y16, hipStream_t st);
int launch_cast_16_to_f32(const void* x16, size_t n, float* y, hipStream_t st);
bool chan_ln32_eligible(int B, int C, int T, int relu);
int launch_chan_ln_bwd(const float* x, const float* dy, const float* y, int B, int C, int T, float eps, int ada,
                       const float* w, const float* gb, int relu, const float* out_mask, float* dx, int accumulate,
                       float* mu_tmp, float* r_tmp, float* dgb, float* dw, float* db, hipStream_t st, int h16 = 0);
int launch_grn_bwd(const double* part, int nseg, const float* gamma, const float* ds, int B, int C4, float* coef,
                   float* dgamma, hipStream_t st);
int launch_act_fwd(int kind, const float* x, const float* alpha, int B, int C, int T, float* y, hipStream_t st);
int launch_act_bwd(int kind, const float* x, const float* dy, const float* alpha, int B, int C, int T, float* dx,
                   int accumulate, float* dalpha, hipStream_t st);
int launch_row_scale_add(const float* src, const float* coef, float k, int rows, int T, float* dst, hipStream_t st);
int launch_dwconv_fwd(const float* x, const float* w, const float* bias, int B, int C, int T, int K, int pad, float* y,
                      hipStream_t st);
size_t dwconv_bwd_scratch_floats(int B, int C, int T, int K);
int launch_dwconv_bwd(const float* x, const float* dy, const float* w, int B, int C, int T, int K, int pad, float* dx,
                      int accumulate, float* dw, float* db, float* scratch, hipStream_t st, const float* dx_src = nullptr,
                      int x16 = 0, int dy16 = 0);
int launch_bn_eval_fwd(const float* x, const float* w, const float* b, const float* rm, const float* rv, float eps,
                       int B, int C, int T, float* y, hipStream_t st);
int launch_bn_eval_bwd(const float* x, const float* dy, const float* w, const float* rm, const float* rv, float eps,
                       int B, int C, int T, float* dx, float* dw, float* db, hipStream_t st);
size_t bias_grad_scratch_floats(int B, int C, int T);
int launch_partial_sum(int dw_form, const float* part, int C, int K, int nblk, float* dw, float* db, hipStream_t st);
int launch_bias_grad(const float* g, const float* mask, int B, int C, int T, int shuffle, float scale, float* db,
                     float* scratch, hipStream_t st);
int launch_style_fc_bwd(const void* descs_dev, int nlayers, int B, int style_dim, const float* style,
                        const float* dgb_base, float* dstyle, hipStream_t st);
int launch_istft64_bwd(int B, int F, const float* audio, const float* daudio, const float* logamp, const float* real,
                       const float* imag, const float* bbr, const float* bbi, float* dlogamp, float* dreal,
                       float* dimag, hipStream_t st);
size_t wgrad_partial_floats(const PackedConv& w, int B, int T);
struct WgReduceDefer;
WgReduceDefer* wgrad_defer_create();
void wgrad_defer_destroy(WgReduceDefer* d);
WgReduceDefer* wgrad_defer_set(WgReduceDefer* d);
size_t wgrad_defer_pending(const WgReduceDefer* d);
int wgrad_defer_flush(WgReduceDefer* d, int site, hipStream_t st);
int launch_attention_bwd(const AttnArgs& a, const float* dO, float* dQ, float* dK, float* dV, size_t dqbs, size_t dkbs,
                         size_t dvbs, size_t dobs, int B, int DH, float* ws, hipStream_t st, int overwrite = 0);
bool attention_bwd_can_overwrite(const AttnArgs& a, int DH);
bool attention_bwd_mfma_dh(int DH);
size_t attention_bwd_ws_floats(int B, int H, int T);
int launch_rope_signed(float* q, float* k, int B, int H, int DH, int L, int d, const float* theta4, float sgn,
                       hipStream_t st);
int launch_embedding_bwd(const int64_t* tokens, const float* g, int B, int L, int H, int ntok, float scale, float* demb,
                         hipStream_t st);
int launch_bmm_ct_bwd(const float* g, const float* ali, int B, int C, int L, int T, float* denc, hipStream_t st);
int launch_slice_add(const float* src, int Csrc, int c0, int B, int C, int T, float* dst, hipStream_t st);
int launch_fnv_bwd(const float* pitch, const float* energy, const float* voiced, const float* w34, const float* g, int B,
                   int T, float* dw34, float* dp, float* de, float* dv, hipStream_t st);
int launch_fnv_unpack(const float* dw34, const float* g0, const float* v0, const float* g1, const float* v1,
                      const float* g2, const float* v2, float* dg0, float* dv0, float* db0, float* dg1, float* dv1,
                      float* db1, float* dg2, float* dv2, float* db2, hipStream_t st);
size_t dwconv2d_s2_bwd_scratch_floats(int B, int C, int H, int W);
int launch_dwconv2d_s2_bwd(const float* x, const float* gy, const float* gate, const float* w9, int B, int C, int H, int W, float* dx,
                           int accumulate, float* dw9, float* db, float* scratch, hipStream_t st, __bf16* dx16 = nullptr,
                           const float* mask16 = nullptr);
int launch_pad_cols(const float* x, size_t rows, int W, float* y, hipStream_t st);
int launch_flat_mask(int B, int H, int Wp, int Hv, int Wv, float* m, hipStream_t st);
int launch_dw2d_sn_unpack(const float* g9, const float* w, const float* u, const float* v, const float* t, int C,
                          float* dW, hipStream_t st);
int launch_avgpool2_bwd(const float* gy, int BC, int H, int W, float scale, float* dx, const float* gate, hipStream_t st,
                        __bf16* dx16 = nullptr, const float* mask16 = nullptr, int C = 0);
int launch_pool_fc_bwd(const float* x, int B, int C, int n, int count, const float* W, int S, const float* gs,
                       float* dW, float* db, float* dx, int accumulate, hipStream_t st);
int launch_bn_train_fwd(const float* x, const float* w, const float* b, float* rm, float* rv, float eps, float momentum,
                        int B, int C, int T, float* y, float* mean, float* rstd, double* part, hipStream_t st);
int launch_bn_train_bwd(const float* x, const float* dy, const float* w, const float* mean, const float* rstd, int B,
                        int C, int T, float* dx, int accumulate, float* dw, float* db, float* sums, hipStream_t st);
int launch_dropout(const float* x, const float* res, size_t n, float p, unsigned seed, unsigned site, float* y,
                   int accumulate, hipStream_t st, size_t group = 1);
int launch_box_smooth(const float* x, int B, int T, int width, float* y, int accumulate, hipStream_t st);
size_t sn_power_iter_scratch_floats(int Cout, int n);
int trainer_style_forward(struct Trainer* t, int B, int T, const float* mel, float* style, void* ws, size_t ws_bytes,
                          hipStream_t st, size_t* need, const float* pitch = nullptr, const float* energy = nullptr);
int trainer_style_backward(struct Trainer* t, const float* d_style, hipStream_t st);
int trainer_style_tap(struct Trainer* t, int i, int grad, float* dst, int* C, int* H, int* W, hipStream_t st);
inline sty_vocoder_io vocoder_io_of(const sty_speech_io& io) {
  sty_vocoder_io v = io.voc_taps;
  v.B = io.B;
  v.T = io.T;
  v.style = io.style;
  v.pitch = io.denormal_pitch;
  v.voiced = io.voiced;
  v.noise = io.noise;
  v.prior_override = io.prior_override;
  v.seed = io.seed;
  v.audio = io.audio;
  return v;
}
struct Trainer;
Trainer* trainer_create(sty_model* m);
int trainer_speech_forward(Trainer* t, const sty_speech_io* io, void* ws, size_t ws_bytes, hipStream_t st,
                           size_t* need);
int trainer_speech_backward(Trainer* t, const float* d_audio, float* d_style, float* d_energy, hipStream_t st,
                            float* d_pitch = nullptr);
int trainer_block_fwd_bwd(Trainer* t, int kind, const void* blk, int B, int C, int T, const float* x, const float* style,
                          const float* gy, float* y, float* gx, float* d_style, void* ws, size_t ws_bytes, hipStream_t st,
                          size_t* need);
void trainer_set_segment_hook(Trainer* t, std::function<void(int)> fn);
bool single_stream_mode();
int trainer_wait_d_style(Trainer* t, hipStream_t stream);
void* trainer_branch_stream(Trainer* t);
int trainer_pitch_energy_forward(Trainer* t, int B, int L, int T, const int64_t* texts, const int64_t* lengths,
                                 const float* alignment, const float* style, float* pitch, float* energy, void* ws,
                                 size_t ws_bytes, hipStream_t st, size_t* need);
int trainer_pitch_energy_backward(Trainer* t, const float* d_pitch, const float* d_energy, float* d_style, hipStream_t st);
void trainer_destroy(Trainer* t);
int trainer_vocoder_forward(Trainer* t, const sty_vocoder_io* io, void* ws, size_t ws_bytes, hipStream_t st,
                            size_t* need);
int trainer_vocoder_backward(Trainer* t, const float* d_audio, float* d_mel, float* d_style, hipStream_t st);
}
```

stylish_tts_amd/csrc/norms.hip:

```cpp
#include "sty_common.h"

namespace sty {

__global__ __launch_bounds__(256) void style_fc_kernel(const StyleFcDesc* __restrict__ descs, int style_dim,
                                                       const float* __restrict__ style, float* __restrict__ gb_base,
                                                       int B) {
  __shared__ float s[256];
  const StyleFcDesc d = descs[blockIdx.x];
  const int b = blockIdx.y;
  for (int i = threadIdx.x; i < style_dim; i += 256) s[i] = style[(size_t)b * style_dim + i];
  __syncthreads();
  for (int j = threadIdx.x; j < d.n; j += 256) {
    const float* w = d.W + (size_t)j * style_dim;
    float acc = 0.f;
    for (int k = 0; k < style_dim; ++k) acc = fmaf(s[k], w[k], acc);
    gb_base[d.off * B + (size_t)b * d.n + j] = acc + d.b[j];
  }
}

int launch_style_fc(const StyleFcDesc* descs_dev, int nlayers, int B, int style_dim, const float* style,
                    float* gb_base, hipStream_t st) {
  if (style_dim > 256) {
    set_error("style_fc: style_dim %d > 256", style_dim);
    return STY_EINVAL;
  }
  hipLaunchKernelGGL(style_fc_kernel, dim3(nlayers, B), dim3(256), 0, st, descs_dev, style_dim, style, gb_base, B);
  STY_LAUNCH_CHECK();
  return STY_OK;
}

constexpr int SEG = 4096;
int row_stats_nseg(int T) { return cdiv(T, SEG); }

__global__ __launch_bounds__(256) void row_stats_kernel(const float* __restrict__ x, int T, int nseg,
                                                        double* __restrict__ part) {
  __shared__ double rs[8], rq[8];
  const int seg = blockIdx.x, row = blockIdx.y;
  const float* p = x + (size_t)row * T;
  const int beg = seg * SEG, end = min(beg + SEG, T);
  double s = 0.0, q = 0.0;
  for (int i = beg + threadIdx.x; i < end; i += 256) {
    const double v = (double)p[i];
    s += v;
    q += v * v;
  }
  for (int o = 32; o > 0; o >>= 1) {
    s += __shfl_xor(s, o);
    q += __shfl_xor(q, o);
  }
  const int wave = threadIdx.x >> 6;
  if ((threadIdx.x & 63) == 0) {
    rs[wave] = s;
    rq[wave] = q;
  }
  __syncthreads();
  if (threadIdx.x == 0) {
    double ts = rs[0] + rs[1] + rs[2] + rs[3], tq = rq[0] + rq[1] + rq[2] + rq[3];
    part[((size_t)row * nseg + seg) * 2 + 0] = ts;
    part[((size_t)row * nseg + seg) * 2 + 1] = tq;
  }
}

int launch_row_stats(const float* x, int rows, int T, double* part, hipStream_t st) {
  const int nseg = row_stats_nseg(T);
  hipLaunchKernelGGL(row_stats_kernel, dim3(nseg, rows), dim3(256), 0, st, x, T, nseg, part);
  STY_LAUNCH_CHECK();
  return STY_OK;
}

__global__ __launch_bounds__(256) void adain_finalize_kernel(const double* __restrict__ part, int nseg,
                                                             const float* __restrict__ gb, int B, int C, int T, float eps,
                                                             float* __restrict__ a, float* __restrict__ s) {
  const int i = blockIdx.x * 4 + (threadIdx.x >> 6), lane = threadIdx.x & 63;
  if (i >= B * C) return;
  const int b = i / C, c = i % C;
  double sum = 0.0, sq = 0.0;
  for (int k = lane; k < nseg; k += 64) {
    sum += part[((size_t)i * nseg + k) * 2];
    sq += part[((size_t)i * nseg + k) * 2 + 1];
  }
  for (int o = 32; o > 0; o >>= 1) {
    sum += __shfl_xor(sum, o);
    sq += __shfl_xor(sq, o);
  }
  if (lane) return;
  const double mean = sum / T;
  double var = sq / T - mean * mean;
  if (var < 0.0) var = 0.0;
  const float rstd = (float)(1.0 / sqrt(var + (double)eps));
  const float g = 1.f + gb[(size_t)b * 2 * C + c], be = gb[(size_t)b * 2 * C + C + c];
  const float av = g * rstd;
  a[i] = av;
  s[i] = be - av * (float)mean;
}

int launch_adain_finalize(const double* part, int nseg, const float* gb, int B, int C, int T, float eps, float* a,
                          float* s, hipStream_t st) {
  hipLaunchKernelGGL(adain_finalize_kernel, dim3(cdiv(B * C, 4)), dim3(256), 0, st, part, nseg, gb, B, C, T, eps, a, s);
  STY_LAUNCH_CHECK();
  return STY_OK;
}

__global__ __launch_bounds__(1024) void grn_finalize_kernel(const double* __restrict__ part, int nseg, int G,
                                                            const float* __restrict__ gamma, int C4,
                                                            float* __restrict__ scale) {
  __shared__ float red[16];
  __shared__ float gxs[1024];
  const int b = blockIdx.x, wave = threadIdx.x >> 6, lane = threadIdx.x & 63;
  const int cpw = 64 / G, sub = lane / G, gl = lane % G;
  float loc = 0.f;
  for (int c0 = wave * cpw; c0 < C4; c0 += 16 * cpw) {
    const int c = c0 + sub;
    double sq = 0.0;
    if (c < C4) {
      const double* p = part + ((size_t)b * C4 + c) * nseg * 2 + 1;
      for (int k = gl; k < nseg; k += G) sq += p[(size_t)k * 2];
    }
    for (int o = G >> 1; o > 0; o >>= 1) sq += __shfl_xor(sq, o);
    if (gl == 0 && c < C4) {
      const float gx = (float)sqrt(sq);
      gxs[c] = gx;
      loc += gx;
    }
  }
  for (int o = 32; o > 0; o >>= 1) loc += __shfl_xor(loc, o);
  if (lane == 0) red[wave] = loc;
  __syncthreads();
  float tot = 0.f;
#pragma unroll
  for (int i = 0; i < 16; ++i) tot += red[i];
  const float mean = tot / (float)C4;
  for (int c = threadIdx.x; c < C4; c += 1024) scale[(size_t)b * C4 + c] = 1.f + gamma[c] * (gxs[c] / (mean + 1e-6f));
}

int launch_grn_finalize(const double* part, int nseg, const float* gamma, int B, int C4, float* scale,
                        hipStream_t st) {
  if (C4 > 1024) {
    set_error("grn_finalize: 4C = %d > 1024", C4);
    return STY_EINVAL;
  }
  int G = 1;
  while (G < 64 && G < nseg) G <<= 1;
  hipLaunchKernelGGL(grn_finalize_kernel, dim3(B), dim3(1024), 0, st, part, nseg, G, gamma, C4, scale);
  STY_LAUNCH_CHECK();
  return STY_OK;
}

__global__ __launch_bounds__(64) void chan_layernorm_kernel(const float* __restrict__ x, float* __restrict__ y, int C,
                                                            int T, float eps, int ada, const float* __restrict__ w,
                                                            const float* __restrict__ bvec,
                                                            const float* __restrict__ gb, int relu,
                                                            const float* __restrict__ out_mask) {
  const int t = blockIdx.x * 64 + threadIdx.x;
  const int b = blockIdx.y;
  if (t >= T) return;
  const float* p = x + (size_t)b * C * T + t;
  float mean = 0.f;
  for (int c = 0; c < C; ++c) mean += p[(size_t)c * T];
  mean /= (float)C;
  float var = 0.f;
  for (int c = 0; c < C; ++c) {
    const float d = p[(size_t)c * T] - mean;
    var += d * d;
  }
  const float rstd = 1.0f / sqrtf(var / (float)C + eps);
  float* q = y + (size_t)b * C * T + t;
  for (int c = 0; c < C; ++c) {
    const float n = (p[(size_t)c * T] - mean) * rstd;
    float sc, sh;
    if (ada) {
      sc = 1.f + gb[(size_t)b * 2 * C + c];
      sh = gb[(size_t)b * 2 * C + C + c];
    } else {
      sc = w[c];
      sh = bvec[c];
    }
    float o = n * sc + sh;
    if (relu) o = fmaxf(o, 0.f);
    if (out_mask) o *= out_mask[(size_t)b * T + t];
    q[(size_t)c * T] = o;
  }
}

template <int CPT>
__global__ __launch_bounds__(256) void chan_layernorm_reg_kernel(const float* __restrict__ x, float* __restrict__ y,
                                                                 int T, float eps, int ada,
                                                                 const float* __restrict__ w,
                                                                 const float* __restrict__ bvec,
                                                                 const float* __restrict__ gb, int relu,
                                                                 const float* __restrict__ out_mask) {
  constexpr int C = 4 * CPT;
  __shared__ float red[4][64];
  const int lane = threadIdx.x & 63, wave = threadIdx.x >> 6;
  const int t = blockIdx.x * 64 + lane, b = blockIdx.y;
  const bool in = t < T;
  const float* p = x + (size_t)b * C * T + t;
  float v[CPT];
  float s = 0.f;
#pragma unroll
  for (int i = 0; i < CPT; ++i) {
    v[i] = in ? p[(size_t)(wave + 4 * i) * T] : 0.f;
    s += v[i];
  }
  red[wave][lane] = s;
  __syncthreads();
  const float mean = (red[0][lane] + red[1][lane] + red[2][lane] + red[3][lane]) * (1.0f / C);
  __syncthreads();
  float q = 0.f;
#pragma unroll
  for (int i = 0; i < CPT; ++i) {
    const float d = v[i] - mean;
    q += d * d;
  }
  red[wave][lane] = q;
  __syncthreads();
  const float rstd = 1.0f / sqrtf((red[0][lane] + red[1][lane] + red[2][lane] + red[3][lane]) * (1.0f / C) + eps);
  if (!in) return;
  const float om = out_mask ? out_mask[(size_t)b * T + t] : 1.f;
  float* o = y + (size_t)b * C * T + t;
#pragma unroll
  for (int i = 0; i < CPT; ++i) {
    const int c = wave + 4 * i;
    float sc, sh;
    if (ada) {
      sc = 1.f + gb[(size_t)b * 2 * C + c];
      sh = gb[(size_t)b * 2 * C + C + c];
    } else {
      sc = w[c];
      sh = bvec[c];
    }
    float r = (v[i] - mean) * rstd * sc + sh;
    if (relu) r = fmaxf(r, 0.f);
    o[(size_t)c * T] = r * om;
  }
}

int launch_chan_layernorm(const float* x, float* y, int B, int C, int T, float eps, int ada, const float* w,
                          const float* bvec, const float* gb, int relu, const float* out_mask, hipStream_t st) {
  const dim3 grid(cdiv(T, 64), B);
#define STY_LN_CASE(CPT)                                                                                          \
  case 4 * CPT:                                                                                                    \
    hipLaunchKernelGGL(chan_layernorm_reg_kernel<CPT>, grid, dim3(256), 0, st, x, y, T, eps, ada, w, bvec, gb, relu, \
                       out_mask);                                                                                  \
    break;
  switch (C) {
    STY_LN_CASE(8)
    STY_LN_CASE(16)
    STY_LN_CASE(32)
    STY_LN_CASE(64)
    STY_LN_CASE(80)
    STY_LN_CASE(96)
    STY_LN_CASE(128)
    default:
      hipLaunchKernelGGL(chan_layernorm_kernel, grid, dim3(64), 0, st, x, y, C, T, eps, ada, w, bvec, gb, relu,
                         out_mask);
  }
#undef STY_LN_CASE
  STY_LAUNCH_CHECK();
  return STY_OK;
}

template <int KT>
__global__ __launch_bounds__(256) void dwconv_adaln_kernel(const float* __restrict__ x, const float* __restrict__ w,
                                                           const float* __restrict__ bias, int C, int T, int K,
                                                           float eps, const float* __restrict__ gb,
                                                           float* __restrict__ y, int TT) {
  extern __shared__ __attribute__((aligned(16))) float u[];
  float* smean = u + (size_t)C * TT;
  float* srstd = smean + TT;
  float* part = srstd + TT;
  const int b = blockIdx.y, t0 = blockIdx.x * TT;
  const int pad = K / 2;
  const int tid = threadIdx.x;
  const int lane = tid % TT, grp = tid / TT, ngrp = 256 / TT;
  const int t = t0 + lane;
  float psum = 0.f;
  for (int c = grp; c < C; c += ngrp) {
    const float* p = x + ((size_t)b * C + c) * T;
    float acc = bias[c];
    if constexpr (KT > 0) {
      float xv[KT];
#pragma unroll
      for (int k = 0; k < KT; ++k) {
        const int tt = t - KT / 2 + k;
        xv[k] = (tt >= 0 && tt < T) ? p[tt] : 0.f;
      }
#pragma unroll
      for (int k = 0; k < KT; ++k) acc = fmaf(w[c * KT + k], xv[k], acc);
    } else {
      for (int k = 0; k < K; ++k) {
        const int tt = t - pad + k;
        if (tt >= 0 && tt < T) acc = fmaf(w[c * K + k], p[tt], acc);
      }
    }
    u[c * TT + lane] = acc;
    psum += acc;
// ... 90 lines not shown
```

stylish_tts_amd/csrc/sty_common.h:

```cpp
#pragma once
#include <hip/hip_runtime.h>
#include <stdint.h>
#include <stdio.h>

#include "../../include/stylish_hip.h"

namespace sty {

void set_error(const char* fmt, ...);
int hip_fail(hipError_t e, const char* what);

#define STY_HIP(expr)                                      \
  do {                                                     \
    hipError_t _e = (expr);                                \
    if (_e != hipSuccess) return sty::hip_fail(_e, #expr); \
  } while (0)

#define STY_LAUNCH_CHECK() STY_HIP(hipGetLastError())

extern thread_local const void* g_last_kernel;
template <class R, class... A>
inline const void* kernel_handle(R (*f)(A...)) {
  return reinterpret_cast<const void*>(f);
}
// ... 97 lines not shown
  int Cin = 0, Cout = 0, K = 1, CinP = 0, CoutP = 0;
  const void* wf = nullptr;
};

constexpr int CI_CHUNK = 32;

enum ConvPro : int {
  PRO_NONE = 0,
  PRO_AFFINE = 1,
  PRO_AFFINE_SNAKE = 2,
  PRO_AFFINE_LRELU = 3,
  PRO_LN_AFFINE = 4,
  PRO_MASK = 5,
  PRO_SCALE = 6,
  PRO_LRELU = 7,
};
enum ConvAct : int { ACT_NONE = 0, ACT_RELU = 1, ACT_SWISH = 2, ACT_SNAKE = 3, ACT_GLU = 4, ACT_GELU = 5,
                     ACT_LRELU01 = 6 };

struct ConvArgs {
  const float* x[3] = {nullptr, nullptr, nullptr};
  int xc[3] = {0, 0, 0};
  int nsrc = 1;
  int B = 0, T = 0;
  int Tin = 0;
  int dil = 1, pad = 0;
  int hpad = 0, Cin2d = 0;
  int flatW = 0;
  int ksplit_max = 4;
  int bf16 = 0;
  int in_shuffle = 0;
  PackedConv w;
  int pro = PRO_NONE;
  const float* pa = nullptr;
  const float* ps = nullptr;
  const float* palpha = nullptr;
  const float* pbeta = nullptr;
  float ln_eps = 1e-6f;
  const float* mask = nullptr;
  int act = ACT_NONE;
  const float* act_alpha = nullptr;
  float out_scale = 1.f;
  const float* residual = nullptr;
  const float* out_mask = nullptr;
  int out_mask_post = 0;
  int shuffle = 1;
  int ln_out = 0;
  const float* ln_w = nullptr;
  const float* ln_b = nullptr;
  float* y = nullptr;
  float* y_split = nullptr;
  double* stat_part = nullptr;
  const __bf16* x16 = nullptr;
  const __bf16* g16 = nullptr;
  __bf16* y16 = nullptr;
  int y16_act = PRO_NONE;
  const float* up_g = nullptr;
  const __bf16* up_gate16 = nullptr;
  const float* up_mask = nullptr;
  float up_scale = 1.f;
  int up_H = 0;
  int xh = 0, yh = 0, rh = 0, gh = 0;
  int w_row = 0, w_tap = 0;
};
int launch_twin_cast(const float* x, const float* mask, int pro, int B, int C, int T, __bf16* y16, hipStream_t st);
int launch_wgradb16(const ConvArgs& fwd, int nsplit, float* partial, int want_bias, hipStream_t st);

enum ConvKernel : int {
  CONV_STEM2D,
  CONV_32P,
  CONV_K1,
  CONV_Q,
  CONV_P16,
  CONV_TILED,
};
enum ConvRefusal : int { CONV_OK = 0, CONV_NO_UP_STAGE, CONV_NO_TWO_BYTE, CONV_NO_STATS };
struct ConvRoute {
  ConvKernel kernel = CONV_TILED;
  ConvRefusal refusal = CONV_OK;
  bool x16_only = false;
  bool up_stage = false;
  bool writes_y16() const { return kernel == CONV_STEM2D || kernel == CONV_Q || kernel == CONV_P16; }
  bool stats() const { return kernel == CONV_32P; }
  bool two_byte() const { return kernel == CONV_32P; }
};
ConvRoute conv1d_route(const ConvArgs& a);
int launch_conv1d(const ConvArgs& a, hipStream_t st);
int conv32p_stat_nseg(int T);
inline int num_cus() {
  static int n = 0;
  if (!n) {
    int dev = 0;
    if (hipGetDevice(&dev) != hipSuccess || hipDeviceGetAttribute(&n, hipDeviceAttributeMultiprocessorCount, dev) != hipSuccess || n <= 0)
      n = 256;
  }
  return n;
}
enum WgradKernel : int {
  WGRAD_B,
  WGRAD_B16,
  WGRAD_K1,
  WGRAD_64,
  WGRAD_ROWS32,
  WGRAD_STEM,
  WGRAD_P32,
  WGRAD_TILED,
};
struct WgradRoute {
  WgradKernel kernel = WGRAD_TILED;
  int nsplit = 1;
  size_t plane = 0;
  bool fuses_bias = true;
  bool twins_only = false;
  bool refused = false;
};
WgradRoute conv1d_wgrad_route(const ConvArgs& fwd, const float* g, const float* gmask);
bool wgrad_fuses_bias(const ConvArgs& fwd);
int launch_conv1d_wgrad(const ConvArgs& fwd, const float* g, const float* gmask, float scale, float* gwp,
                        float* partial, float* gbias, bool* bias_done, hipStream_t st);
int launch_wgradb(const ConvArgs& ax, const ConvArgs& ag, int nsplit, float* partial, int want_bias, hipStream_t st);
int wgradb_chunks(const PackedConv& w, int B, int T, int dil);
int wgradp32_chunks(const ConvArgs& fwd);
int launch_wgradp32(const ConvArgs& ax, const ConvArgs& ag, int nsplit, float* partial, int want_bias, hipStream_t st);
int wgrad_cnx_nsplit(int B, int T);
int launch_conv_wgrad_cnx(int x_wide, const void* wide, const float* narrow, int B, int T, float* gwp, float* partial,
                          float* gbias, hipStream_t st, int narrow16 = 0);
int wgrad_cnx_per_b(int B, int T);
int launch_wgrad_cnx(int x_wide, const void* wide, const float* narrow, int B, int T, float* partial, int want_bias,
                     hipStream_t st, int per_b = 0, int narrow16 = 0);
int convp16_repack_range(const void* lo, const void* hi, hipStream_t st);
void convp16_forget_range(const void* lo, const void* hi);


struct StyleFcDesc {
  const float* W;
  const float* b;
  size_t off;
  int n;
  int pad;
};
int launch_style_fc(const StyleFcDesc* descs_dev, int nlayers, int B, int style_dim, const float* style,
                    float* gb_base, hipStream_t st);
struct StyleFcBwdDesc {
  const float* W;
  float* dW;
  float* db;
  size_t off;
  int n;
  int pad;
};
int row_stats_nseg(int T);
int launch_row_stats(const float* x, int rows, int T, double* part, hipStream_t st);
int launch_adain_finalize(const double* part, int nseg, const float* gb, int B, int C, int T, float eps, float* a,
                          float* s, hipStream_t st);
int launch_grn_finalize(const double* part, int nseg, const float* gamma, int B, int C4, float* scale, hipStream_t st);
int launch_chan_layernorm(const float* x, float* y, int B, int C, int T, float eps, int ada, const float* w,
                          const float* bvec, const float* gb, int relu, const float* out_mask, hipStream_t st);
int launch_embedding(const int64_t* tokens, const float* emb, int B, int L, int H, int ntok, float scale, float* y,
                     hipStream_t st);
int launch_length_mask(const int64_t* lengths, int B, int L, float* mask, hipStream_t st);
int launch_bmm_ct(const float* enc, const float* ali, int B, int C, int L, int T, float* y, hipStream_t st);
int launch_concat(const float* const* src, const int* ch, int nsrc, int B, int T, float* y, hipStream_t st);
int launch_fnv(const float* pitch, const float* energy, const float* voiced, const float* w34, int B, int T, float* y,
               hipStream_t st);
int launch_prep_fnv(const float* g0, const float* v0, const float* b0, const float* g1, const float* v1,
                    const float* b1, const float* g2, const float* v2, const float* b2, float* w34, hipStream_t st);
int launch_alignment(const float* dur, int B, int L, int T, float* ali, hipStream_t st);
int launch_axpy(const float* x, float a, float* y, size_t n, hipStream_t st);
int launch_dwconv_adaln(const float* x, const float* w, const float* bias, int B, int C, int T, int K, float eps,
                        const float* gb, float* y, hipStream_t st);
int launch_dwconv_bn_swish(const float* x, const float* w, const float* bias, const float* bn_w, const float* bn_b,
                           const float* bn_rm, const float* bn_rv, float bn_eps, int B, int C, int T, int K,
                           float* y, hipStream_t st);
}

namespace sty {
struct Cnx32Args {
  const float* x;
  const float* dw_w;
  const float* dw_b;
  const float* gb;
  const float* w1p;
  const float* b1;
  const float* alpha;
  const float* w2a;
  const float* b2eff;
  const float* scale;
  double* part;
  float* y;
  int T, ntiles;
  int bf16 = 0;
  void* h16 = nullptr;
};

struct Cnx32BwdArgs {
  const float* x;
  const float* gy;
  const float *dw_w, *dw_b;
  const float* gb;
  const float* w1p;
  const float* w1;
  const float* w2;
  const float *b1, *alpha;
  const float* scale;
  const float* coef;
  double* part;
  double* part_gb;
  float *hs, *gh0;
  float *xn, *gu;
  int T, ntiles;
  int bf16 = 0;
  int out_bf16 = 0;
  int lean = 0;
  const void* wfrag = nullptr;
  float* gx = nullptr;
  int xn16 = 0;
  int gy16 = 0, gx16 = 0, gu16 = 0;
  int x16 = 0;
};
constexpr int CNX_BWD_FUSED_STRIDE = 248;
int convnext32_bwd_ntiles(int T, int fused);
constexpr size_t CNX_FRAG_HALFS = 3 * 4 * 2 * 64 * 8;
int launch_cnx_frag_pack(const float* w1p, const float* w2raw, const float* w1raw, void* wfrag, hipStream_t st);
int launch_cnx_m_finish(float* partial, int B, int SB, const float* w2raw, const float* scale, float* ds, float* gw2,
                        float* gb2, hipStream_t st);
int launch_cnx_dalpha(const float* w1raw, const float* b1, const float* alpha, const float* gw1, const float* gb1,
                      const float* scale, const float* ds, const float* coef, const double* part, int nseg, int B,
                      float* dalpha, hipStream_t st);
int launch_convnext32_bwd(const Cnx32BwdArgs& a, int B, int pass, hipStream_t st);
int launch_cnx_partial_sum(const double* part, int B, int C, int ntiles, int mode, float* out, hipStream_t st);

constexpr int W2A_MAXJ = 16;
struct W2aJobs {
  const float* w2[W2A_MAXJ];
  const float* b2[W2A_MAXJ];
  const float* gb[W2A_MAXJ];
  float* w2a[W2A_MAXJ];
  float* b2eff[W2A_MAXJ];
  int C[W2A_MAXJ];
  int n = 0;
};
int launch_pack_w2a_multi(const W2aJobs& jobs, hipStream_t st);
struct AttnArgs {
  const float* q;
  const float* k;
  const float* v;
  float* o;
  size_t qbs, kbs, vbs, obs;
  int T, H;
  float scale;
  const int64_t* lengths;
  float drop_p = 0.f;
  unsigned drop_seed = 0, drop_site = 0;
  float* lse = nullptr;
  int bf16 = 0;
};
bool attention16_eligible(const AttnArgs& a, int DH);
int launch_attention16(const AttnArgs& a, int B, hipStream_t st);
int launch_attention16_bwd(const AttnArgs& a, const float* dO, float* dQ, float* dK, float* dV, size_t dqbs, size_t dkbs,
                           size_t dvbs, size_t dobs, int B, float* ws, hipStream_t st);
}

#ifdef __HIPCC__
namespace sty {
__device__ __forceinline__ float sty_hash_u(unsigned seed, unsigned site, unsigned idx) {
  unsigned x = idx * 0x9E3779B1u + site * 0x85EBCA77u + seed * 0xC2B2AE3Du;
  x ^= x >> 16;
  x *= 0x7FEB352Du;
  x ^= x >> 15;
  x *= 0x846CA68Bu;
  x ^= x >> 16;
  return (float)(x >> 8) * (1.0f / 16777216.0f);
}
__device__ __forceinline__ void sty_unit_vec(float re, float im, float& c, float& s) {
  const float h2 = re * re + im * im;
  if (h2 > 0.f && h2 < 3.0e38f) {
    const float r = 1.0f / sqrtf(h2);
    c = re * r;
    s = im * r;
  } else {
    const float ph = atan2f(im, re);
    c = cosf(ph);
    s = sinf(ph);
  }
}
static __device__ __attribute__((noinline)) float sty_sinf_slow(float x) { return sinf(x); }
__device__ __forceinline__ float sty_sinf(float x) {
  if (__builtin_expect(fabsf(x) > 8192.0f, 0)) return sty_sinf_slow(x);
  const float kf = rintf(x * 0.636619772f);
  const int k = (int)kf;
  float r = fmaf(-kf, 1.57079637050628662109375f, x);
  r = fmaf(-kf, -4.37113900018624283e-8f, r);
  r = fmaf(-kf, -1.71512449e-15f, r);
  const float r2 = r * r;
  const float ps = fmaf(r2, fmaf(r2, -1.9515295891e-4f, 8.3321608736e-3f), -1.6666654611e-1f);
  const float s = fmaf(r * r2, ps, r);
  const float pc = fmaf(r2, fmaf(r2, 2.443315711809948e-5f, -1.388731625493765e-3f), 4.166664568298827e-2f);
  const float c = fmaf(r2 * r2, pc, fmaf(r2, -0.5f, 1.0f));
  const float res = (k & 1) ? c : s;
  return (k & 2) ? -res : res;
}
__device__ __forceinline__ float sty_sin2_fast(float x) {
  const float kf = rintf(x * 0.636619772f);
  float r = fmaf(-kf, 1.57079637050628662109375f, x);
  r = fmaf(-kf, -4.37113900018624283e-8f, r);
  const float z = r * r;
  float p = fmaf(z, -4.27556050e-6f, 1.41093474e-4f);
  p = fmaf(p, z, -3.17460317e-3f);
// ... 110 lines not shown
```

stylish_tts_amd/csrc/train.hip:

```cpp
#include <stdlib.h>
#include <string.h>

#include <map>
#include <memory>
#include <unordered_map>

#include "model.h"

namespace sty {

struct Trainer {
  sty_model* m = nullptr;
  hipStream_t st = nullptr;
  int B = 0, T = 0;
  Bump ws;
  int rc = STY_OK;
  float* gb = nullptr;
  float* dgb = nullptr;
  const float* style = nullptr;
  float* audio = nullptr;
  std::vector<std::function<void()>> tape;
  std::unordered_map<const float*, float*> gmap;
  std::unordered_set<const float*> nograd;
  float* scratch_param = nullptr;
  size_t scratch_param_n = 0;
  const float* mel_in = nullptr;
  size_t peak = 0;

  bool dry = false;
  bool live() const { return !dry && ws.base != nullptr && rc == STY_OK; }
  void chk(int r) {
    if (rc == STY_OK && r != STY_OK) rc = r;
  }
  static constexpr size_t kDryBase = size_t(1) << 30, kDryCap = size_t(1) << 46;
  static constexpr size_t kSlack = 64 << 20, kSlackStyle = 16 << 20;
  static inline float kDryMel = 0.f, kDryStyle = 0.f;
  void open(int B_, int T_, void* ws_, size_t ws_bytes, hipStream_t st_, bool dry_) {
    st = st_;
    B = B_;
    T = T_;
    rc = STY_OK;
    ws = Bump();
    dry = dry_;
    ws.base = dry ? reinterpret_cast<char*>(kDryBase) : (char*)ws_;
    ws.cap = dry ? kDryCap : ws_bytes;
    peak = 0;
  }
  void reset_step() {
    tape.clear();
    gmap.clear();
    tw_x[0].clear();
    tw_x[1].clear();
    tw_want.clear();
    tw_g.clear();
    g_twin_only.clear();
    g_no_fp32.clear();
    lazy_mask.clear();
    pend_up.clear();
    nograd.clear();
    half_.clear();
    g16_ok.clear();
    adain_of.clear();
    ungated.clear();
    side_need = 0;
    wg_sum = 0;
    drop_site = 0;
    drop_seed_arg = nullptr;
    branch_st = nullptr;
    branch_can_beside = false;
    branch_lo = branch_hi = branch_join = 0;
  }
  int close_forward(size_t* need, size_t ws_bytes, size_t slack, const char* what) {
    if (need) {
      *need = align_up(peak, 256) + slack;
      tape.clear();
      return rc;
    }
    if (ws.overflow) {
      set_error("%s workspace too small: need %zu bytes, have %zu", what, peak, ws_bytes);
      return STY_ENOMEM;
    }
    return rc;
  }
  int close_backward() {
    if (ws.overflow) {
      set_error("training workspace too small in backward: need %zu bytes", peak);
      return STY_ENOMEM;
    }
    return rc;
  }
  void copy_f32(float* dst, const float* src, size_t n, const char* what) {
    if (!live()) return;
    hipError_t e = hipMemcpyAsync(dst, src, n * sizeof(float), hipMemcpyDeviceToDevice, st);
    if (e != hipSuccess) rc = hip_fail(e, what);
  }
  float* seed(const float* act, const float* d, size_t n) {
    float* g = G(act, n);
    if (d) copy_f32(g, d, n, "seed copy");
    return g;
  }
  void run_tape(const std::function<void()>& seeds, bool flush_up, bool fc, float* d_style) {
    side_begin();
    if (fc) {
      d_style_out = d_style;
      fc_bwd_done = false;
    }
    seeds();
    const bool br = branch_lo < branch_hi && branch_hi <= branch_join && branch_join < tape.size();
    const bool br_beside = br && (branch_st || (dry && branch_can_beside));
    hipEvent_t br_end = nullptr;
    for (size_t i = tape.size(); i-- > 0 && rc == STY_OK;) {
      if (br_beside && i >= branch_lo && i < branch_hi) {
        if (i + 1 == branch_hi && br_end) {
          hipError_t r = hipStreamWaitEvent(st, br_end, 0);
          if (r != hipSuccess) rc = hip_fail(r, "prior branch backward join");
          br_end = nullptr;
        }
        continue;
      }
      tape[i]();
      if (rc != STY_OK || !br_beside || i != branch_join) continue;
      hipStream_t const main_st = st;
      if (branch_st) {
        stream_after(branch_st, main_st, "prior branch backward fork");
        st = branch_st;
      }
      keep_temps = true;
      for (size_t j = branch_hi; j-- > branch_lo && rc == STY_OK;) tape[j]();
      keep_temps = false;
      st = main_st;
      if (branch_st && live()) {
        const int rc0 = rc;
        rc = STY_OK;
        br_end = next_event();
        if (rc == STY_OK && hipEventRecord(br_end, branch_st) != hipSuccess) {
          br_end = nullptr;
          rc = hip_fail(hipGetLastError(), "prior branch backward end");
        }
        if (rc0 != STY_OK) rc = rc0;
      }
    }
    if (br_end) (void)hipStreamWaitEvent(st, br_end, 0);
    while (flush_up && rc == STY_OK && !pend_up.empty()) up_flush(pend_up.begin()->first);
    side_join();
    if (fc && rc == STY_OK) style_fc_backward();
  }

  hipStream_t branch_st = nullptr;
  bool branch_can_beside = false;
  size_t branch_lo = 0, branch_hi = 0, branch_join = 0;

  std::vector<char> fcs_bwd_sent;
  hipStream_t st2 = nullptr;
  bool side_on = getenv("STY_NO_SIDE_STREAM") == nullptr;
  std::vector<hipEvent_t> evs;
  size_t ev_used = 0;
  std::unordered_set<const float*> side_reads;
  bool side_dirty = false;
  size_t side_need = 0;
  float* side_partial = nullptr;
  WgReduceDefer* defer = wgrad_defer_create();
  bool defer_on = getenv("STY_NO_DEFERRED_REDUCE") == nullptr;
  size_t wg_sum = 0, wg_off = 0;
  float* wg_base = nullptr;
  int flush_site = 0;
  std::vector<std::function<void(hipStream_t)>> after_reduce;
  bool deferring() const { return wg_base != nullptr; }
  float* wg_take(size_t n) {
    n = (n + 63) & ~size_t(63);
    float* p = wg_base + wg_off;
    wg_off += n;
    if (wg_off > wg_sum && rc == STY_OK) {
      set_error("training: weight-gradient partial region too small (%zu > %zu floats)", wg_off, wg_sum);
      rc = STY_ESTATE;
    }
    return p;
  }
  void wg_need(size_t n) { wg_sum += (n + 63) & ~size_t(63); }
  struct DeferScope {
    WgReduceDefer* old;
    explicit DeferScope(Trainer* t) { old = wgrad_defer_set(t->deferring() && t->live() ? t->defer : nullptr); }
    ~DeferScope() { (void)wgrad_defer_set(old); }
  };
  void reduce_flush(hipStream_t s) {
    if (!deferring() || !live()) {
      after_reduce.clear();
      return;
    }
    chk(wgrad_defer_flush(defer, flush_site++, s));
    WgReduceDefer* cur = wgrad_defer_set(nullptr);
    if (rc == STY_OK)
      for (auto& fn : after_reduce) fn(s);
    (void)wgrad_defer_set(cur);
    after_reduce.clear();
  }
  bool twins_env = getenv("STY_NO_TWINS") == nullptr;
  bool twins_on() const { return twins_env && m->topts.compute_bf16 != 0; }
  std::unordered_map<const float*, __bf16*> tw_x[2];
  std::unordered_set<const float*> tw_want;
  std::unordered_map<const float*, std::pair<__bf16*, const float*>> tw_g;
  static int tw_slot(int pro) { return pro == PRO_LRELU ? 1 : 0; }
  void twin_register(const float* x, int pro, __bf16* t) { tw_x[tw_slot(pro)][x] = t; }
  const __bf16* xtwin(const float* x, int pro, int C, int n) {
    auto& mp = tw_x[tw_slot(pro)];
    auto it = mp.find(x);
    if (it != mp.end()) return it->second;
    __bf16* t = take<__bf16>((size_t)B * C * n);
    if (live()) chk(launch_twin_cast(x, nullptr, pro, B, C, n, t, st));
    mp[x] = t;
    return t;
  }
  std::unordered_set<const float*> g_twin_only, g_no_fp32;
  struct LazyMask {
    const float* src;
    const float* mask;
    int C, n;
    float* dst;
  };
  std::unordered_map<const float*, LazyMask> lazy_mask;
  bool mask_pending(const float* act) const { return !lazy_mask.empty() && lazy_mask.count(act) != 0; }
  void mask_flush(const float* act) {
    auto it = lazy_mask.find(act);
    if (it == lazy_mask.end()) return;
    const LazyMask z = it->second;
    lazy_mask.erase(it);
    if (live())
      chk(launch_pro_bwd(PRO_MASK, z.src, z.C, 0, z.src, B, z.C, z.n, nullptr, nullptr, z.C, 0, nullptr, z.mask, z.dst, 0,
                         nullptr, nullptr, nullptr, st));
  }
  struct PendUp {
    const float* g;
    const float* mask;
    float scale;
    int BC, C, H, W, n;
  };
  std::unordered_map<const float*, PendUp> pend_up;
  void up_apply(const float* src, const PendUp& u) {
    const bool gated = gate_pending(src);
    if (gated) ungated.erase(src);
    float* gs = G(src, (size_t)u.BC * u.n);
    __bf16* g16 = twins_on() && tw_want.count(src) && u.n % 4 == 0 ? take<__bf16>((size_t)u.BC * u.n) : nullptr;
    if (g16) tw_g[gs] = std::make_pair(g16, u.mask);
    if (live()) chk(launch_avgpool2_bwd(u.g, u.BC, u.H, u.W, u.scale, gs, gated ? src : nullptr, st, g16, u.mask, u.C));
  }
  void up_flush(const float* act) {
    auto it = pend_up.find(act);
    if (it == pend_up.end()) return;
    const PendUp u = it->second;
    pend_up.erase(it);
    up_apply(act, u);
  }
  ~Trainer() {
    wgrad_defer_destroy(defer);
    for (hipEvent_t e : evs) (void)hipEventDestroy(e);
    if (d_style_done) (void)hipEventDestroy(d_style_done);
    if (st2) (void)hipStreamDestroy(st2);
  }
  hipEvent_t next_event() {
    if (ev_used == evs.size()) {
      hipEvent_t e = nullptr;
      hipError_t r = hipEventCreateWithFlags(&e, hipEventDisableTiming);
      if (r != hipSuccess) rc = hip_fail(r, "event");
      evs.push_back(e);
    }
    return evs[ev_used++];
  }
  void side_begin() {
    ev_used = 0;
    side_reads.clear();
    side_dirty = false;
    const bool on = side_on && !single_stream_mode();
    side_partial = on && side_need ? take<float>(side_need) : nullptr;
    wg_base = defer_on && wg_sum ? take<float>(wg_sum) : nullptr;
    wg_off = 0;
    flush_site = 0;
    after_reduce.clear();
    if (on && !st2 && live()) {
      int least = 0, greatest = 0;
      (void)hipDeviceGetStreamPriorityRange(&least, &greatest);
      hipError_t r = hipStreamCreateWithPriority(&st2, hipStreamNonBlocking, least);
      if (r != hipSuccess) rc = hip_fail(r, "side stream");
    }
  }
  bool side_ready() const { return side_partial != nullptr; }
  void side_push(const float* gbuf, const std::function<void(hipStream_t)>& fn) {
    side_reads.insert(gbuf);
    if (!live() || !st2) return;
    hipEvent_t e = next_event();
    if (rc == STY_OK) {
      hipError_t r = hipEventRecord(e, st);
      if (r == hipSuccess) r = hipStreamWaitEvent(st2, e, 0);
      if (r != hipSuccess) rc = hip_fail(r, "side fork");
    }
    if (rc == STY_OK) {
      DeferScope ds(this);
      fn(st2);
    }
    side_dirty = true;
  }
  void side_reduce_nowait() {
    if (side_dirty && st2) reduce_flush(st2);
  }
  void side_join() {
    reduce_flush(side_dirty && st2 ? st2 : st);
    if (side_dirty && st2) {
      hipEvent_t e = next_event();
      hipError_t r = hipEventRecord(e, st2);
      if (r == hipSuccess) r = hipStreamWaitEvent(st, e, 0);
      if (r != hipSuccess) rc = hip_fail(r, "side join");
    }
    side_reads.clear();
    side_dirty = false;
  }
  float* side_cow(const float* act, float* g, size_t n) {
    if (side_reads.empty() || !side_reads.count(g)) return g;
    return fresh_copy(act, g, n);
  }
  float* fresh_copy(const float* act, float* g, size_t n) {
    float* g2 = take<float>(n);
    copy_f32(g2, g, n, "grad copy");
    gmap[act] = g2;
    return g2;
  }
  bool alias_grad(const float* act, float* g) {
    if (gmap.count(act)) return false;
    gmap[act] = g;
    return true;
  }
  const float* gbp(const AdaFc& a) const { return gb ? gb + a.off * B : nullptr; }
  float* dgbp(const AdaFc& a) const { return dgb ? dgb + a.off * B : nullptr; }

  template <typename Tp>
  Tp* take(size_t n) {
    Tp* p = ws.take<Tp>(n);
    peak = ws.off > peak ? ws.off : peak;
    return p;
  }
  bool keep_temps = false;
  void release(size_t mark) {
    if (!keep_temps) ws.off = mark;
  }
  std::unordered_set<const void*> half_;
  bool act16_env = getenv("STY_NO_ACT16") == nullptr;
  bool act16_on() const { return act16_env && m->topts.compute_bf16 != 0; }
  bool is16(const void* p) const { return p && !half_.empty() && half_.count(p) != 0; }
  float* take_act(size_t n, bool h) {
    if (!h) return take<float>(n);
    float* p = reinterpret_cast<float*>(take<__bf16>((n + 7) & ~size_t(7)));
    half_.insert(p);
    return p;
  }
  std::unordered_set<const float*> g16_ok;
  bool grad16_env = getenv("STY_NO_GRAD16") == nullptr && getenv("STY_NO_CNX_GX") == nullptr;
  bool grad16_on() const { return grad16_env && act16_on(); }
  bool grad16_stream_env = getenv("STY_GRAD16_STREAM") != nullptr && atoi(getenv("STY_GRAD16_STREAM")) != 0;
  bool grad16_stream_on() const { return grad16_stream_env && grad16_on(); }
  float* G16(const float* act, size_t n) {
    auto it = gmap.find(act);
    if (it != gmap.end() && is16(it->second)) return it->second;
    return G(act, n);
  }
  std::map<const float*, std::pair<int, int>> ungated;
  bool gate_pending(const float* act) const { return !ungated.empty() && ungated.count(act) != 0; }
  void gate_flush(const float* act) {
    auto it = ungated.find(act);
    if (it == ungated.end()) return;
    const int C = it->second.first, n = it->second.second;
    ungated.erase(it);
    auto gi = gmap.find(act);
    if (gi == gmap.end() || !live()) return;
    float* g = gi->second;
    chk(launch_pro_bwd(PRO_LRELU, g, C, 0, act, B, C, n, nullptr, nullptr, C, 0, nullptr, nullptr, g, 0, nullptr, nullptr,
                       nullptr, st));
  }
  float* G(const float* act, size_t n, bool raw = false, bool keep_lazy = false) {
    if (!pend_up.empty()) up_flush(act);
    if (!raw && !ungated.empty()) gate_flush(act);
    if (!keep_lazy && !lazy_mask.empty()) mask_flush(act);
    auto it = gmap.find(act);
    if (it != gmap.end() && is16(it->second)) {
      set_error("a two-byte gradient buffer reached a consumer without a two-byte form");
      rc = STY_ESTATE;
    }
    if (it != gmap.end()) return side_cow(act, it->second, n);
    float* g = take<float>(n);
    if (live()) {
      hipError_t e = hipMemsetAsync(g, 0, n * sizeof(float), st);
      if (e != hipSuccess) rc = hip_fail(e, "grad memset");
    }
    gmap[act] = g;
    return g;
  }
  float* Gw(const float* act, size_t n, int& acc) {
    if (!pend_up.empty()) up_flush(act);
    if (!ungated.empty()) gate_flush(act);
    if (mask_pending(act)) {
      tw_g.erase(lazy_mask[act].dst);
      mask_flush(act);
    }
    auto it = gmap.find(act);
    if (it != gmap.end() && is16(it->second)) {
      set_error("a two-byte gradient buffer reached a second writer");
      rc = STY_ESTATE;
    }
    if (it != gmap.end()) {
      acc = 1;
      return side_cow(act, it->second, n);
    }
    float* g = take<float>(n);
    gmap[act] = g;
    acc = 0;
    return g;
  }
  bool wants(const float* act) const { return !nograd.count(act); }
  float* PGpacked(const float* packed) const {
    if (!packed || !m->garena) return nullptr;
    return reinterpret_cast<float*>(m->garena + (reinterpret_cast<const char*>(packed) - m->arena));
  }
  float* PG(const float* param, size_t n) {
    auto it = m->pgrad.find(param);
    if (it != m->pgrad.end()) return it->second;
    if (n > scratch_param_n) return nullptr;
    return scratch_param;
  }

  ConvArgs base(const PackedConv& w, const float* x, int Tt, float* y) {
    ConvArgs a;
    a.x[0] = x;
    a.xc[0] = w.Cin;
    a.nsrc = 1;
    a.B = B;
    a.T = Tt;
    a.w = w;
    a.pad = (w.K - 1) / 2;
    a.y = y;
    a.bf16 = m->topts.compute_bf16;
    return a;
  }

  void conv(const ConvArgs& a0) {
    ConvArgs a = a0;
    a.bf16 = m->topts.compute_bf16;
    a.xh = is16(a.x[0]);
    a.yh = is16(a.y);
    a.rh = is16(a.residual);
    if (a.nsrc > 1 && (is16(a.x[1]) || is16(a.x[2]))) {
      set_error("training: a bf16-stored tensor as source 1 / 2 of a channel-concatenated conv");
      rc = STY_ESTATE;
      return;
    }
    const size_t pn = wgrad_partial_floats(a.w, B, a.T);
    side_need = pn > side_need ? pn : side_need;
    wg_need(pn);
    bias_pass_sizing(a);
    if (live()) chk(launch_conv1d(a, st));
    ConvArgs f = a;
    tape.push_back([this, f]() { conv_bwd(f); });
  }
  void bias_pass_sizing(const ConvArgs& a) {
    if (!a.w.bias || wgrad_fuses_bias(a)) return;
    const size_t bn = bias_grad_scratch_floats(B, a.w.Cout, a.T);
    side_need = bn > side_need ? bn : side_need;
    wg_need(bn);
  }
  void conv_wgrad(const ConvArgs& f, float* gY, const float* gmask, int shuffle) {
    const PackedConv& w = f.w;
    const int Tt = f.T;
    bool bias_done = false;
    float* gbias = w.bias ? PGpacked(w.bias) : nullptr;
    if (m->topts.frozen) {
      bias_done = true;
    } else if (side_ready()) {
      float* sp = deferring() ? wg_take(wgrad_partial_floats(w, B, Tt)) : side_partial;
      float* gwp = PGpacked(w.wp);
      const float osc = f.out_scale;
      side_push(gY, [=](hipStream_t s) { chk(launch_conv1d_wgrad(f, gY, gmask, osc, gwp, sp, gbias, nullptr, s)); });
      bias_done = wgrad_fuses_bias(f);
      if (w.bias && !bias_done) {
        float* bs = deferring() ? wg_take(bias_grad_scratch_floats(B, w.Cout, Tt)) : side_partial;
        side_push(gY, [=](hipStream_t s) { chk(launch_bias_grad(gY, gmask, B, w.Cout, Tt, shuffle, osc, gbias, bs, s)); });
        bias_done = true;
      }
    } else {
      const size_t pn = wgrad_partial_floats(w, B, Tt);
      float* partial = deferring() ? wg_take(pn) : take<float>(pn);
      DeferScope ds(this);
      if (live()) chk(launch_conv1d_wgrad(f, gY, gmask, f.out_scale, PGpacked(w.wp), partial, gbias, &bias_done, st));
    }
    if (w.bias && !bias_done) {
      float* bs = take<float>(bias_grad_scratch_floats(B, w.Cout, Tt));
      if (live()) chk(launch_bias_grad(gY, gmask, B, w.Cout, Tt, shuffle, f.out_scale, PGpacked(w.bias), bs, st));
    }
  }
  void conv_bwd(const ConvArgs& f) {
    const PackedConv& w = f.w;
    const int Tt = f.T;
    const size_t ny = (size_t)B * w.Cout * Tt;
    float* gY = G(f.y, ny);
    float* gR = nullptr;
    if (f.residual && wants(f.residual)) {
      if (!gmap.count(f.residual) && !(f.out_mask && f.out_mask_post) && f.shuffle <= 1)
        gmap[f.residual] = gY;
      else
        gR = G(f.residual, ny);
    }
    float* gX[3] = {nullptr, nullptr, nullptr};
    int accX[3] = {1, 1, 1};
    bool any = false;
    const float* gX_src = nullptr;
    if (f.nsrc == 1 && f.pro == PRO_AFFINE_SNAKE && Tt % 8 == 0 && wants(f.x[0]) && !side_reads.empty()) {
      auto ia = adain_of.find(f.pa);
      auto ig = gmap.find(f.x[0]);
      if (ia != adain_of.end() && ia->second.x == f.x[0] && ia->second.s == f.ps && !*ia->second.done && ig != gmap.end() &&
          side_reads.count(ig->second) && !is16(ig->second) && (ungated.empty() || !ungated.count(f.x[0]))) {
        gX_src = ig->second;
        gX[0] = take<float>((size_t)B * f.xc[0] * Tt);
        gmap[f.x[0]] = gX[0];
        accX[0] = 1;
        any = true;
      }
    }
    for (int i = 0; i < f.nsrc; ++i)
      if (wants(f.x[i]) && !(i == 0 && gX_src)) {
        gX[i] = Gw(f.x[i], (size_t)B * f.xc[i] * Tt, accX[i]);
        any = true;
      }
    for (int i = 1; i < f.nsrc; ++i)
      for (int j = 0; j < i; ++j)
        if (gX[i] && gX[i] == gX[j]) accX[i] = 1;
    if (side_ready())
      for (int i = 0; i < f.nsrc; ++i)
        if (gX[i] && gX[i] == gY) gX[i] = fresh_copy(f.x[i], gY, (size_t)B * f.xc[i] * Tt);
    float* dpa = nullptr;
    float* dps = nullptr;
    float* dal = nullptr;
    AdainInfo* fuse = nullptr;
    if (any && f.pro == PRO_AFFINE_SNAKE && f.nsrc == 1 && Tt % 8 == 0) {
      auto it = adain_of.find(f.pa);
      if (it != adain_of.end() && it->second.x == f.x[0] && it->second.s == f.ps && !*it->second.done) fuse = &it->second;
    }
    if (any && fuse) {
      dal = PG(f.palpha, w.Cin);
    } else if (any) {
      if (f.pro == PRO_AFFINE_SNAKE || f.pro == PRO_AFFINE_LRELU || f.pro == PRO_AFFINE) {
        int dummy;
        dpa = Gw(f.pa, (size_t)B * w.Cin, dummy);
        dps = Gw(f.ps, (size_t)B * w.Cin, dummy);
      } else if (f.pro == PRO_SCALE) {
        int dummy;
        dpa = Gw(f.pa, (size_t)B * w.Cin, dummy);
      }
      if (f.pro == PRO_AFFINE_SNAKE) dal = PG(f.palpha, w.Cin);
    }
    const size_t mark = ws.off;
    const float* gmask = f.out_mask;
    if (gR && live()) {
      if (f.out_mask && f.out_mask_post)
        chk(launch_pro_bwd(PRO_MASK, gY, w.Cout, 0, gY, B, w.Cout, Tt, nullptr, nullptr, w.Cout, 0, nullptr, f.out_mask,
                           gR, 1, nullptr, nullptr, nullptr, st));
      else
        chk(launch_row_scale_add(gY, nullptr, 1.0f, B * w.Cout, Tt, gR, st));
    }
    conv_wgrad(f, gY, gmask, f.shuffle);
    if (any) {
      auto it = m->dgrad.find(w.wp);
      if (it == m->dgrad.end()) {
        set_error("training: no input-gradient weights for a conv (model not finalized for training?)");
        rc = STY_ESTATE;
        return;
      }
      const bool u16 = f.xh && f.nsrc == 1 && act16_on();
      float* U = take_act((size_t)B * w.Cin * Tt, u16);
      struct UGuard {
        Trainer* t;
        float* U;
        size_t mark;
        ~UGuard() {
          t->half_.erase(U);
          t->release(mark);
        }
      } u_guard{this, U, mark};
      ConvArgs d;
      d.x[0] = gY;
      d.xc[0] = w.Cout;
      d.nsrc = 1;
      d.B = B;
      d.T = Tt;
      d.w = it->second;
      d.dil = f.dil;
      d.bf16 = f.bf16;
      d.pad = (w.K - 1) * f.dil - f.pad;
      d.out_scale = f.out_scale;
      d.in_shuffle = f.shuffle > 1 ? f.shuffle : 0;
      if (gmask) {
        d.pro = PRO_MASK;
        d.mask = gmask;
      }
      d.y = U;
      d.yh = u16;
      d.xh = is16(gY);
      if (f.nsrc == 1 && (f.pro == PRO_NONE || f.pro == PRO_MASK) && gX[0] != gY) {
        d.y = gX[0];
        d.yh = is16(gX[0]);
        d.rh = d.yh;
        d.residual = accX[0] ? gX[0] : nullptr;
        if (f.pro == PRO_MASK) {
          d.out_mask = f.mask;
          d.out_mask_post = 0;
        }
        if (live()) chk(launch_conv1d(d, st));
        release(mark);
        return;
      }
      if (live()) chk(launch_conv1d(d, st));
      if (fuse) {
        *fuse->done = true;
        if (live())
          chk(launch_pro_bwd_adain(U, u16, f.x[0], f.xh, B, w.Cin, Tt, f.pa, f.ps, f.palpha, fuse->mean, fuse->rstd, fuse->gbl,
                                   gX[0], is16(gX[0]), accX[0], fuse->dgl, dal, f.bf16 ? 1 : 0, st, gX_src));
        half_.erase(U);
        release(mark);
        return;
      }
      if (gX_src) {
        set_error("training: out-of-place prologue backward planned without the fused kernel");
        rc = STY_ESTATE;
        return;
      }
      if (u16 || f.xh) {
        half_.erase(U);
        set_error("training: bf16-stored conv input without the fused prologue backward");
        rc = STY_ESTATE;
        return;
      }
      int c0 = 0;
      for (int i = 0; i < f.nsrc; ++i) {
        if (gX[i] && live())
          chk(launch_pro_bwd(f.pro | (f.bf16 ? 0x100 : 0), U, w.Cin, c0, f.x[i], B, f.xc[i], Tt, f.pa, f.ps, w.Cin, c0, f.palpha, f.mask, gX[i],
                             accX[i], dpa, dps, dal, st));
        c0 += f.xc[i];
      }
    }
    release(mark);
  }

  float* act(int kind, const float* x, const float* alpha, int C, int Tt) {
    float* y = take<float>((size_t)B * C * Tt);
    if (live()) chk(launch_act_fwd(kind, x, alpha, B, C, Tt, y, st));
    tape.push_back([=]() {
      const int Cin = kind == ACT_GLU ? 2 * C : C;
      float* gY = G(y, (size_t)B * C * Tt);
      int acc = 1;
      float* gX = Gw(x, (size_t)B * Cin * Tt, acc);
      float* dal = kind == ACT_SNAKE ? PG(alpha, C) : nullptr;
      if (live()) chk(launch_act_bwd(kind, x, gY, alpha, B, C, Tt, gX, acc, dal, st));
    });
    return y;
  }

  unsigned drop_site = 0;
  const unsigned* drop_seed_arg = nullptr;
  unsigned drop_seed_val = 0;
  bool dropout_on() const { return m->topts.dropout_seed != 0; }
  float* dropout(const float* x, float p, int C, int Tt, const float* residual, size_t group = 1) {
    const size_t n = (size_t)B * C * Tt;
    float* y = take<float>(n);
    const unsigned seed = drop_seed_arg ? *drop_seed_arg : m->topts.dropout_seed, site = drop_site++;
    if (live()) chk(launch_dropout(x, residual, n, p, seed, site, y, 0, st, group));
    tape.push_back([=]() {
      float* gY = G(y, n);
      if (residual && wants(residual)) {
        if (!gmap.count(residual)) {
          gmap[residual] = gY;
        } else {
          float* gR = G(residual, n);
          if (live()) chk(launch_row_scale_add(gY, nullptr, 1.0f, 1, (int)n, gR, st));
        }
      }
      int acc = 1;
      float* gX = Gw(x, n, acc);
      if (gX == gY) {
        set_error("dropout backward: aliased gradient buffers");
        rc = STY_ESTATE;
        return;
      }
      if (live()) chk(launch_dropout(gY, nullptr, n, p, seed, site, gX, acc, st, group));
    });
    return y;
  }

  float* layernorm(const float* x, int C, int Tt, float eps, const AdaFc* fc, const float* w, const float* bvec,
                   int relu = 0, const float* omask = nullptr) {
    float* y = take<float>((size_t)B * C * Tt);
    const float* gbl = fc ? gbp(*fc) : nullptr;
    float* dgl = fc ? dgbp(*fc) : nullptr;
    if (live()) chk(launch_chan_layernorm(x, y, B, C, Tt, eps, fc ? 1 : 0, w, bvec, gbl, relu, omask, st));
    const bool ln32 = grad16_on() && chan_ln32_eligible(B, C, Tt, relu);
    if (ln32 && grad16_stream_on()) g16_ok.insert(y);
    tape.push_back([=]() {
      const size_t nel = (size_t)B * C * Tt;
      float* gY = ln32 ? G16(y, nel) : G(y, nel);
      int acc = 1, h16 = is16(gY) ? 2 : 0;
      float* gX;
      if (ln32 && g16_ok.count(x) && !gmap.count(x)) {
        gX = take_act(nel, true);
        gmap[x] = gX;
        acc = 0;
        h16 |= 4;
      } else {
        gX = Gw(x, nel, acc);
      }
      const size_t mark = ws.off;
      float* mu = take<float>((size_t)B * Tt);
      float* r = take<float>((size_t)B * Tt);
      float* dw = fc ? nullptr : PG(w, C);
      float* db = fc ? nullptr : PG(bvec, C);
      if (live())
        chk(launch_chan_ln_bwd(x, gY, y, B, C, Tt, eps, fc ? 1 : 0, w, gbl, relu, omask, gX, acc, mu, r, dgl, dw, db, st, h16));
      ws.off = mark;
    });
    return y;
  }

  struct AdainInfo {
    const float *x, *s, *mean, *rstd, *gbl;
    float* dgl;
    std::shared_ptr<bool> done;
  };
  std::unordered_map<const float*, AdainInfo> adain_of;
  void adain(const float* x, int C, int Tt, const AdaFc& fc, float*& a, float*& s, const double* have_part = nullptr,
             int have_nseg = 0) {
    a = take<float>((size_t)B * C);
    s = take<float>((size_t)B * C);
    float* mean = take<float>((size_t)B * C);
    float* rstd = take<float>((size_t)B * C);
    const int nseg = have_part ? have_nseg : row_stats_nseg(Tt);
    const double* part = have_part;
    if (!have_part) {
      double* p2 = take<double>((size_t)B * C * nseg * 2);
      if (live()) chk(launch_row_stats(x, B * C, Tt, p2, st));
      part = p2;
    }
    if (live()) {
      chk(launch_adain_finalize(part, nseg, gbp(fc), B, C, Tt, 1e-5f, a, s, st));
      chk(launch_adain_stats(part, nseg, B * C, Tt, 1e-5f, mean, rstd, st));
    }
    const float* gbl = gbp(fc);
    float* dgl = dgbp(fc);
    float* aa = a;
    float* ss = s;
    auto done = std::make_shared<bool>(false);
    adain_of[aa] = AdainInfo{x, ss, mean, rstd, gbl, dgl, done};
    if (!have_part && is16(x)) {
      set_error("training: instance-norm statistics pass over a bf16-stored tensor (the producing conv leaves them behind)");
      rc = STY_ESTATE;
    }
    tape.push_back([=]() {
      if (*done) return;
      if (is16(x)) {
        set_error("training: AdaIN backward over a bf16-stored tensor outside the fused prologue backward");
        rc = STY_ESTATE;
        return;
      }
      float* da = G(aa, (size_t)B * C);
      float* ds = G(ss, (size_t)B * C);
      float* gX = G(x, (size_t)B * C * Tt);
      const size_t mark = ws.off;
      float* c0 = take<float>((size_t)B * C);
      float* c1 = take<float>((size_t)B * C);
      if (live()) {
        chk(launch_adain_fold_bwd(da, ds, mean, rstd, gbl, B, C, Tt, dgl, c0, c1, st));
        chk(launch_row_axpb(x, c0, c1, B * C, Tt, gX, st));
      }
      release(mark);
    });
  }

  float* dwconv(const float* x, const float* w, const float* bias, int C, int Tt, int K, int pad) {
    float* y = take<float>((size_t)B * C * Tt);
    if (live()) chk(launch_dwconv_fwd(x, w, bias, B, C, Tt, K, pad, y, st));
    tape.push_back([=]() {
      float* gY = G(y, (size_t)B * C * Tt);
      int acc = 1;
      float* gX = wants(x) ? Gw(x, (size_t)B * C * Tt, acc) : nullptr;
      float* gw = PG(w, (size_t)C * K);
      float* gb = PG(bias, C);
      if (side_ready() && gX != gY) {
        float* sc = take<float>(dwconv_bwd_scratch_floats(B, C, Tt, K));
        side_push(gY, [=](hipStream_t s2) {
          chk(launch_dwconv_bwd(x, gY, w, B, C, Tt, K, pad, nullptr, 0, gw, gb, sc, s2));
        });
        if (live() && gX) chk(launch_dwconv_bwd(x, gY, w, B, C, Tt, K, pad, gX, acc, nullptr, nullptr, nullptr, st));
        return;
      }
      const size_t mark = ws.off;
      float* sc = take<float>(dwconv_bwd_scratch_floats(B, C, Tt, K));
      if (live()) chk(launch_dwconv_bwd(x, gY, w, B, C, Tt, K, pad, gX, acc, gw, gb, sc, st));
      ws.off = mark;
    });
    return y;
  }

  size_t cnx_partial_floats(const PackedConv& w, int Tt) const {
    const size_t a = wgrad_partial_floats(w, B, Tt), b = (size_t)wgrad_cnx_nsplit(B, Tt) * (4096 + 128);
    return a > b ? a : b;
  }
  float* convnext32_fused(const ConvNeXt& c, const float* x, int Tt) {
    const int nt = convnext32_ntiles(Tt);
    const size_t n32 = (size_t)B * 32 * Tt, n128 = (size_t)B * 128 * Tt;
    double* part = take<double>((size_t)B * 128 * nt * 2);
    float* scale = take<float>((size_t)B * 128);
    float* y = take<float>(n32);
    const bool lean = m->topts.compute_bf16 && Tt % 8 == 0 && getenv("STY_NO_WGRADB") == nullptr &&
                      getenv("STY_NO_CNX_LEAN") == nullptr;
    __bf16* h16 = lean ? take<__bf16>(n128) : nullptr;
    __bf16* wfrag = m->topts.compute_bf16 ? take<__bf16>(CNX_FRAG_HALFS) : nullptr;
    if (live() && wfrag) chk(launch_cnx_frag_pack(c.w1p, c.w2_raw, c.w1_raw, wfrag, st));
    if (live()) {
      Cnx32Args a;
      a.x = x;
      a.dw_w = c.dw_w;
      a.dw_b = c.dw_b;
      a.gb = gbp(c.norm);
      a.w1p = c.w1p;
      a.b1 = c.b1;
      a.alpha = c.alpha;
      a.w2a = c.w2a;
      a.b2eff = c.pw2.bias;
      a.scale = scale;
      a.part = part;
      a.y = y;
      a.T = Tt;
      a.ntiles = nt;
      a.bf16 = m->topts.compute_bf16;
      a.h16 = h16;
      chk(launch_convnext32(a, B, 1, st));
      chk(launch_grn_finalize(part, nt, c.grn_gamma, B, 128, scale, st));
      chk(launch_convnext32(a, B, 2, st));
    }
    if (lean && grad16_stream_on()) g16_ok.insert(y);
    const float* gbl = gbp(c.norm);
    float* dgl = dgbp(c.norm);
    {
      const size_t p1n = cnx_partial_floats(c.pw1, Tt), p2n = cnx_partial_floats(c.pw2, Tt);
      side_need = p1n > side_need ? p1n : side_need;
      side_need = p2n > side_need ? p2n : side_need;
      wg_need(p1n);
      wg_need(p2n);
    }
    tape.push_back([=]() {
      float* gY = lean ? G16(y, n32) : G(y, n32);
      const bool gy16 = is16(gY);
      const bool side = side_ready();
      float* gX;
      const float* gx_src = nullptr;
      const bool fuse_gx = !gmap.count(x) && Tt % 4 == 0 && getenv("STY_NO_CNX_GX") == nullptr;
      const bool xn16 = lean && getenv("STY_NO_CNX_XN16") == nullptr;
      const bool gx16 = fuse_gx && lean && grad16_on() && g16_ok.count(x) != 0;
      const bool gu16 = fuse_gx && lean && grad16_on();
      if (gy16 && !fuse_gx) {
        set_error("convnext32: a two-byte output gradient needs the fused input-gradient path");
        rc = STY_ESTATE;
        return;
      }
      if (!gmap.count(x)) {
        if (side || fuse_gx) {
          gX = take_act(n32, gx16);
          gmap[x] = gX;
          gx_src = gY;
        } else {
          gmap[x] = gY;
          gX = gY;
        }
      } else {
        gX = G(x, n32);
        if (live()) chk(launch_row_scale_add(gY, nullptr, 1.0f, 1, (int)n32, gX, st));
      }
      const int nt_b = convnext32_bwd_ntiles(Tt, fuse_gx);
      float* hs_p = side && !lean ? take<float>(n128) : nullptr;
      float* gh0_p = side ? take<float>(lean ? n128 / 2 : n128) : nullptr;
      float* ds_p = (side || deferring()) && lean ? take<float>((size_t)B * 128) : nullptr;
      float* coef_p = (side || deferring()) && lean ? take<float>((size_t)B * 128) : nullptr;
      float* xn_p = side ? take<float>(xn16 ? n32 / 2 : n32) : nullptr;
      float* gu_p = side ? take<float>(gu16 ? n32 / 2 : n32) : nullptr;
      float* dsc_p = side ? take<float>(dwconv_bwd_scratch_floats(B, 32, Tt, 7)) : nullptr;
      const size_t mark = ws.off;
      double* pds = take<double>((size_t)B * 128 * nt_b);
      double* pgb = take<double>((size_t)B * 64 * nt_b);
      float* ds = ds_p ? ds_p : take<float>((size_t)B * 128);
      float* coef = coef_p ? coef_p : take<float>((size_t)B * 128);
      float* hs = lean ? nullptr : (side ? hs_p : take<float>(n128));
      float* gh0 = side ? gh0_p : take<float>(lean ? n128 / 2 : n128);
      float* xn = side ? xn_p : take<float>(xn16 ? n32 / 2 : n32);
      float* gu = side ? gu_p : take<float>(gu16 ? n32 / 2 : n32);
      Cnx32BwdArgs a;
      a.x = x;
      a.gy = gY;
      a.dw_w = c.dw_w;
      a.dw_b = c.dw_b;
      a.gb = gbl;
      a.w1p = c.w1p;
      a.w1 = c.w1_raw;
      a.w2 = c.w2_raw;
      a.b1 = c.b1;
      a.alpha = c.alpha;
      a.scale = scale;
      a.coef = coef;
      a.part = pds;
      a.part_gb = pgb;
      a.hs = hs;
      a.gh0 = gh0;
      a.xn = xn;
      a.gu = gu;
      a.T = Tt;
      a.ntiles = nt_b;
      a.gx = fuse_gx ? gX : nullptr;
      a.xn16 = xn16;
      a.gy16 = gy16;
      a.gx16 = gx16;
      a.gu16 = gu16;
      a.bf16 = m->topts.compute_bf16;
      a.wfrag = wfrag;
      const bool cnx16 = a.bf16 && Tt % 8 == 0 && getenv("STY_NO_WGRADB") == nullptr;
      a.out_bf16 = cnx16;
      ConvArgs f2 = base(c.pw2, hs, Tt, nullptr);
      ConvArgs f1 = base(c.pw1, xn, Tt, nullptr);
      const size_t p1n_ = cnx_partial_floats(c.pw1, Tt), p2n_ = cnx_partial_floats(c.pw2, Tt);
      float* p2 = deferring() ? wg_take(p2n_) : side ? side_partial : take<float>(p2n_);
      float* p1 = deferring() ? wg_take(p1n_) : side ? side_partial : take<float>(p1n_);
      float* dsc = side ? dsc_p : take<float>(dwconv_bwd_scratch_floats(B, 32, Tt, 7));
      float* gw2 = PGpacked(c.pw2.wp);
      float* gb2 = PGpacked(c.pw2.bias);
      float* gw1 = PGpacked(c.pw1.wp);
      float* gb1 = PGpacked(c.pw1.bias);
      const bool frozen = m->topts.frozen;
      float* dal = PG(c.alpha, 128);
      if (lean) {
        const int SB = wgrad_cnx_per_b(B, Tt);
        float* pM = take<float>((size_t)B * SB * (4096 + 32));
        a.lean = 1;
        if (live()) {
          chk(launch_wgrad_cnx(1, h16, gY, B, Tt, pM, 1, st, 1, gy16));
          chk(launch_cnx_m_finish(pM, B, SB, c.w2_raw, scale, ds, frozen ? nullptr : gw2, frozen ? nullptr : gb2, st));
          chk(launch_grn_bwd(part, nt, c.grn_gamma, ds, B, 128, coef, PG(c.grn_gamma, 128), st));
          chk(launch_convnext32_bwd(a, B, 2, st));
          chk(launch_cnx_partial_sum(pgb, B, 64, nt_b, 2, dgl, st));
        }
      } else if (live()) {
        Cnx32BwdArgs a1 = a;
        a1.gx = nullptr;
        a1.ntiles = nt;
        chk(launch_convnext32_bwd(a1, B, 1, st));
        chk(launch_cnx_partial_sum(pds, B, 128, nt, 0, ds, st));
        chk(launch_grn_bwd(part, nt, c.grn_gamma, ds, B, 128, coef, PG(c.grn_gamma, 128), st));
        chk(launch_convnext32_bwd(a, B, 2, st));
        chk(launch_cnx_partial_sum(pds, B, 128, nt_b, 1, dal, st));
        chk(launch_cnx_partial_sum(pgb, B, 64, nt_b, 2, dgl, st));
      }
      const float *w1r = c.w1_raw, *b1p = c.b1, *alp = c.alpha;
      auto lean_w1 = [=](hipStream_t s_) {
        chk(launch_conv_wgrad_cnx(0, gh0, xn, B, Tt, gw1, p1, gb1, s_, xn16));
        auto dalpha = [=](hipStream_t s3) {
          chk(launch_cnx_dalpha(w1r, b1p, alp, gw1, gb1, scale, ds, coef, part, nt, B, dal, s3));
        };
        if (deferring())
          after_reduce.push_back(dalpha);
        else
          dalpha(s_);
      };
      float* gdw = PG(c.dw_w, 32 * 7);
      float* gdb = PG(c.dw_b, 32);
      const float* dww = c.dw_w;
      if (m->topts.frozen) {
        if (live() && !fuse_gx) chk(launch_dwconv_bwd(x, gu, dww, B, 32, Tt, 7, 3, gX, 1, nullptr, nullptr, nullptr, st, gx_src));
      } else if (side) {
        side_push(gY, [=](hipStream_t s2) {
          if (lean) {
            lean_w1(s2);
          } else if (cnx16) {
            chk(launch_conv_wgrad_cnx(1, hs, gY, B, Tt, gw2, p2, gb2, s2));
            chk(launch_conv_wgrad_cnx(0, gh0, xn, B, Tt, gw1, p1, gb1, s2));
          } else {
            chk(launch_conv1d_wgrad(f2, gY, nullptr, 1.0f, gw2, p2, gb2, nullptr, s2));
            chk(launch_conv1d_wgrad(f1, gh0, nullptr, 1.0f, gw1, p1, gb1, nullptr, s2));
          }
          chk(launch_dwconv_bwd(x, gu, dww, B, 32, Tt, 7, 3, nullptr, 0, gdw, gdb, dsc, s2, nullptr, 0, gu16));
        });
        if (live() && !fuse_gx) chk(launch_dwconv_bwd(x, gu, dww, B, 32, Tt, 7, 3, gX, 1, nullptr, nullptr, nullptr, st, gx_src));
      } else if (live()) {
        bool done = false;
        DeferScope dsc_(this);
        if (lean) {
          lean_w1(st);
        } else if (cnx16) {
          chk(launch_conv_wgrad_cnx(1, hs, gY, B, Tt, gw2, p2, gb2, st));
          chk(launch_conv_wgrad_cnx(0, gh0, xn, B, Tt, gw1, p1, gb1, st));
        } else {
          chk(launch_conv1d_wgrad(f2, gY, nullptr, 1.0f, gw2, p2, gb2, &done, st));
          chk(launch_conv1d_wgrad(f1, gh0, nullptr, 1.0f, gw1, p1, gb1, &done, st));
        }
        if (fuse_gx)
          chk(launch_dwconv_bwd(x, gu, dww, B, 32, Tt, 7, 3, nullptr, 0, gdw, gdb, dsc, st, nullptr, 0, gu16));
        else
          chk(launch_dwconv_bwd(x, gu, dww, B, 32, Tt, 7, 3, gX, 1, gdw, gdb, dsc, st));
      }
      ws.off = mark;
    });
    return y;
  }

  float* convnext(const ConvNeXt& c, const float* x, int Tt, bool branch_only = false) {
    const int C = c.C;
    if (C == 32 && c.w2a && c.w1_raw && c.w2_raw) return convnext32_fused(c, x, Tt);
    float* u = dwconv(x, c.dw_w, c.dw_b, C, Tt, 7, 3);
    float* xn = layernorm(u, C, Tt, 1e-6f, &c.norm, nullptr, nullptr);
    float* h0 = take<float>((size_t)B * 4 * C * Tt);
    conv(base(c.pw1, xn, Tt, h0));
    float* h = c.alpha ? act(ACT_SNAKE, h0, c.alpha, 4 * C, Tt)
                       : act(ACT_GELU, h0, nullptr, 4 * C, Tt);
    const int nseg = row_stats_nseg(Tt);
    double* part = take<double>((size_t)B * 4 * C * nseg * 2);
    float* scale = take<float>((size_t)B * 4 * C);
    if (live()) {
      chk(launch_row_stats(h, B * 4 * C, Tt, part, st));
      chk(launch_grn_finalize(part, nseg, c.grn_gamma, B, 4 * C, scale, st));
    }
    const float* gamma = c.grn_gamma;
    tape.push_back([=]() {
      float* dsc = G(scale, (size_t)B * 4 * C);
      float* gH = G(h, (size_t)B * 4 * C * Tt);
      const size_t mark = ws.off;
      float* coef = take<float>((size_t)B * 4 * C);
      if (live()) {
        chk(launch_grn_bwd(part, nseg, gamma, dsc, B, 4 * C, coef, PG(gamma, 4 * C), st));
        chk(launch_row_scale_add(h, coef, 0.f, B * 4 * C, Tt, gH, st));
      }
      ws.off = mark;
    });
    float* y = take<float>((size_t)B * C * Tt);
    ConvArgs b2 = base(c.pw2, h, Tt, y);
    b2.pro = PRO_SCALE;
    b2.pa = scale;
    if (!branch_only) b2.residual = x;
    conv(b2);
    return y;
  }

  static ConvArgs cat3_slice(const ConvArgs& a3, const PackedConv& w, int i, bool dgrad) {
    ConvArgs s = a3;
    s.nsrc = 1;
    s.xc[0] = 32;
    s.x[1] = s.x[2] = nullptr;
    s.xc[1] = s.xc[2] = 0;
    s.w = w;
    s.w.Cin = s.w.CinP = 32;
    s.w.Cout = s.w.CoutP = 32;
    if (dgrad) {
      s.w.wp = w.wp + 32 * i;
      s.w_row = w.CoutP;
      s.w_tap = w.CinP * w.CoutP;
    } else {
      s.w.wp = w.wp + (size_t)32 * i * w.CoutP;
      s.w_row = w.CoutP;
      s.w_tap = w.CinP * w.CoutP;
    }
    return s;
  }
  bool cat3_ok(const ConvArgs& a3) const {
    if (!m->topts.compute_bf16 || getenv("STY_NO_CAT3") || a3.nsrc != 3 || a3.w.CinP != 96 || a3.w.CoutP != 32) return false;
    for (int i = 0; i < 3; ++i)
      if (a3.xc[i] != 32 || is16(a3.x[i])) return false;
    if (a3.pro != PRO_NONE || a3.residual || a3.out_mask || a3.act != ACT_NONE || a3.shuffle != 1) return false;
    auto it = m->dgrad.find(a3.w.wp);
    if (it == m->dgrad.end()) return false;
    ConvArgs f = cat3_slice(a3, a3.w, 0, false), d = cat3_slice(a3, it->second, 0, true);
    d.pad = (a3.w.K - 1) * a3.dil - a3.pad;
    return plan_route(m, f).kernel == CONV_32P && plan_route(m, d).kernel == CONV_32P;
  }
  void conv_cat3(const ConvArgs& a0) {
    ConvArgs a3 = a0;
    a3.bf16 = m->topts.compute_bf16;
    const size_t pn = wgrad_partial_floats(a3.w, B, a3.T);
    side_need = pn > side_need ? pn : side_need;
    wg_need(pn);
    bias_pass_sizing(a3);
    for (int i = 0; i < 3 && live(); ++i) {
      ConvArgs s = cat3_slice(a3, a3.w, i, false);
      s.x[0] = a3.x[i];
      if (i) {
        s.w.bias = nullptr;
        s.residual = a3.y;
      }
      chk(launch_conv1d(s, st));
    }
    tape.push_back([this, a3]() {
      const PackedConv& w = a3.w;
      const int Tt = a3.T;
      const size_t ny = (size_t)B * 32 * Tt;
      float* gY = G(a3.y, ny);
      float* gX[3];
      int accX[3] = {1, 1, 1};
      for (int i = 0; i < 3; ++i) gX[i] = wants(a3.x[i]) ? Gw(a3.x[i], ny, accX[i]) : nullptr;
      const size_t mark = ws.off;
      conv_wgrad(a3, gY, nullptr, 1);
      const PackedConv& wd = m->dgrad.find(w.wp)->second;
      for (int i = 0; i < 3; ++i) {
        if (!gX[i] || !live()) continue;
        ConvArgs d = cat3_slice(a3, wd, i, true);
        d.x[0] = gY;
        d.w.bias = nullptr;
        d.pad = (w.K - 1) * a3.dil - a3.pad;
        d.y = gX[i];
        d.residual = accX[i] ? gX[i] : nullptr;
        chk(launch_conv1d(d, st));
      }
      ws.off = mark;
    });
  }
  bool resblock16(const ResBlock32& r, int Tt) const {
    if (!act16_on() || Tt % 8 != 0) return false;
    const int dil[3] = {1, 3, 5};
    for (int i = 0; i < 3; ++i) {
      ConvArgs c1, c2;
      c1.B = c2.B = B, c1.T = c2.T = Tt, c1.nsrc = c2.nsrc = 1, c1.w = r.c1[i], c2.w = r.c2[i];
      c1.xc[0] = c2.xc[0] = 32;
      c1.dil = dil[i], c1.pad = 5 * dil[i], c2.pad = 5;
      c1.pro = c2.pro = PRO_AFFINE_SNAKE;
      c1.xh = c1.yh = c2.xh = c2.yh = c2.rh = 1;
      if (!plan_route(m, c1).two_byte() || !plan_route(m, c2).two_byte()) return false;
    }
    return true;
  }
  float* resblock(const ResBlock32& r, float* x, int Tt, const double* part_x = nullptr) {
    const int dil[3] = {1, 3, 5};
    const int nseg_p = conv32p_stat_nseg(Tt);
    const bool h16 = resblock16(r, Tt);
    if (is16(x) && (!h16 || !part_x)) {
      set_error("training: bf16-stored resblock input without the two-byte path");
      rc = STY_ESTATE;
      return x;
    }
    for (int i = 0; i < 3; ++i) {
      float *a, *s;
      adain(x, 32, Tt, r.n1[i], a, s, part_x, nseg_p);
      float* xt = take_act((size_t)B * 32 * Tt, h16);
      ConvArgs c1 = base(r.c1[i], x, Tt, xt);
      c1.dil = dil[i];
      c1.pad = 5 * dil[i];
      c1.pro = PRO_AFFINE_SNAKE;
      c1.pa = a;
      c1.ps = s;
      c1.palpha = r.a1[i];
      double* part_t = nullptr;
      if (plan_route(m, c1).stats()) c1.stat_part = part_t = take<double>((size_t)B * 32 * nseg_p * 2);
      conv(c1);
      adain(xt, 32, Tt, r.n2[i], a, s, part_t, nseg_p);
      float* xn = take_act((size_t)B * 32 * Tt, h16 && i + 1 < 3);
      ConvArgs c2 = base(r.c2[i], xt, Tt, xn);
      c2.pro = PRO_AFFINE_SNAKE;
      c2.pa = a;
      c2.ps = s;
      c2.palpha = r.a2[i];
      c2.residual = x;
      part_x = nullptr;
      if (plan_route(m, c2).stats() && i + 1 < 3) {
        double* p = take<double>((size_t)B * 32 * nseg_p * 2);
        c2.stat_part = p;
        part_x = p;
      }
      conv(c2);
      x = xn;
    }
    return x;
  }

  float* attention(const float* q, const float* kv, int inner, int Tt) {
    float* o = take<float>((size_t)B * inner * Tt);
    AttnArgs at;
    at.q = q;
    at.k = kv;
    at.v = kv + (size_t)inner * Tt;
    at.o = o;
    at.qbs = (size_t)inner * Tt;
    at.kbs = at.vbs = (size_t)2 * inner * Tt;
    at.obs = (size_t)inner * Tt;
    at.T = Tt;
    at.H = 8;
    at.scale = 1.0f / sqrtf((float)(inner / 8));
    at.lengths = nullptr;
    at.bf16 = m->topts.compute_bf16;
// ... 1558 lines not shown
```

stylish_tts_amd/lib.py:

```python
import ctypes as C
import os

os.environ.setdefault("GPU_MAX_HW_QUEUES", "2")

HERE = os.path.dirname(os.path.abspath(__file__))
LIB_PATH = os.path.join(HERE, "libstylish_hip.so")


class StyError(RuntimeError):
    pass


class VocoderIO(C.Structure):
    _fields_ = [("B", C.c_int), ("T", C.c_int)] + [
        (n, C.c_void_p) for n in ("mel", "style", "pitch", "voiced", "noise", "prior_override")
    ] + [("seed", C.c_uint64), ("audio", C.c_void_p)] + [
        (n, C.c_void_p) for n in ("tap_conformer_out", "tap_prior", "tap_har_spec", "tap_har_phase",
                                  "tap_logamp_prior", "tap_phase_prior", "tap_trunk", "tap_logamp")
    ]


class SpeechIO(C.Structure):
    _fields_ = [("B", C.c_int), ("L", C.c_int), ("T", C.c_int)] + [
        (n, C.c_void_p) for n in ("texts", "text_lengths", "alignment", "pitch", "energy", "voiced", "style",
                                  "denormal_pitch", "noise", "prior_override")
    ] + [("seed", C.c_uint64), ("audio", C.c_void_p), ("tap_text_encoding", C.c_void_p),
         ("tap_decoder_out", C.c_void_p), ("voc_taps", VocoderIO), ("style_stream", C.c_void_p)]


class TrainOpts(C.Structure):
    _fields_ = [("bn_batch_stats", C.c_int), ("sn_power_iter", C.c_int), ("f0_smooth", C.c_int),
                ("energy_smooth", C.c_int), ("bn_momentum", C.c_float), ("dropout_seed", C.c_uint),
                ("text_dropout", C.c_float), ("compute_bf16", C.c_int), ("frozen", C.c_int),
                ("block_dropout", C.c_float)]


class SpecDiscPtrs(C.Structure):
    _fields_ = [("g", C.c_void_p * 10), ("v", C.c_void_p * 10), ("bias", C.c_void_p * 10)]


class CfDiscParams(C.Structure):
    _fields_ = [("conv_w", C.c_void_p * 12), ("conv_b", C.c_void_p * 12), ("bn_w", C.c_void_p * 9), ("bn_b", C.c_void_p * 9),
                ("bn_rm", C.c_void_p * 9), ("bn_rv", C.c_void_p * 9)]


class CfDiscGrads(C.Structure):
    _fields_ = [("conv_w", C.c_void_p * 12), ("conv_b", C.c_void_p * 12), ("bn_w", C.c_void_p * 9), ("bn_b", C.c_void_p * 9)]


_P, _I, _SZP = C.c_void_p, C.c_int, C.POINTER(C.c_size_t)
SYMBOLS = {
    "sty_version": (C.c_int, []),
    "sty_last_error": (C.c_char_p, []),
    "sty_stft64_bases_host": (None, [_P]),
    "sty_model_create": (C.c_int, [C.c_char_p, C.POINTER(_P)]),
    "sty_model_destroy": (None, [_P]),
    "sty_model_bind": (C.c_int, [_P, C.c_char_p, _P, _I, C.POINTER(C.c_int64)]),
    "sty_model_finalize": (C.c_int, [_P]),
    "sty_model_num_keys": (C.c_int, [_P]),
    "sty_model_key": (C.c_char_p, [_P, _I]),
    "sty_model_prepare": (C.c_int, [_P, _P]),
    "sty_model_invalidate": (C.c_int, [_P]),
    "sty_vocoder_workspace_bytes": (C.c_int, [_P, _I, _I, _SZP]),
    "sty_vocoder_fwd": (C.c_int, [_P, C.POINTER(VocoderIO), _P, C.c_size_t, _P]),
    "sty_speech_workspace_bytes": (C.c_int, [_P, _I, _I, _I, _SZP]),
    "sty_speech_fwd": (C.c_int, [_P, C.POINTER(SpeechIO), _P, C.c_size_t, _P]),
    "sty_style_workspace_bytes": (C.c_int, [_P, _I, _I, _SZP]),
    "sty_style_fwd": (C.c_int, [_P, _I, _I, _P, _P, _P, C.c_size_t, _P]),
    "sty_mel_workspace_bytes": (C.c_int, [_I, _I, _I, _I, _SZP]),
    "sty_mel_fwd": (C.c_int, [_I, _I, _P, _I, _I, _I, C.c_float, C.c_float, _P, _P, _P, C.c_size_t, _P]),
    "sty_multispec_workspace_bytes": (C.c_int, [_I, _I, _SZP]),
    "sty_multispec_fwd": (C.c_int, [_I, _I, _P, C.POINTER(_P), C.POINTER(_P), C.POINTER(_P), _P, C.c_size_t, _P]),
    "sty_alignment_fwd": (C.c_int, [_I, _I, _I, _P, _P, _P]),
    "sty_convnext_fwd": (C.c_int, [_P, C.c_char_p, _I, _I, _I, _P, _P, _P, _P, C.c_size_t, _P]),
    "sty_resblock_fwd": (C.c_int, [_P, C.c_char_p, _I, _I, _P, _P, _P, _P, C.c_size_t, _P]),
    "sty_block_train_workspace_bytes": (C.c_int, [_P, C.c_char_p, C.c_char_p, _I, _I, _I, _SZP]),
    "sty_block_fwd_bwd": (C.c_int, [_P, C.c_char_p, C.c_char_p, _I, _I, _I, _P, _P, _P, _P, _P, _P, _P, C.c_size_t, _P]),
    "sty_attention_workspace_bytes": (C.c_int, [_I, _I, _I, _SZP]),
    "sty_attention_fwd_bwd": (C.c_int, [_I, _I, _I, _I, _P, _P, _P, _P, _P, _P, _P, _P, _P, _P, C.c_size_t, _P]),
    "sty_stft64_fwd": (C.c_int, [_I, _I, _P, _P, _P, _P]),
    "sty_istft64_fwd": (C.c_int, [_I, _I, _P, _P, _P, _P, _P]),
    "sty_source_fwd": (C.c_int, [_I, _I, _P, _P, _P, C.c_uint64, _P, _P, _P, _P, C.c_size_t, _P]),
    "sty_source_workspace_bytes": (C.c_int, [_I, _I, _SZP]),
    "sty_model_enable_training": (C.c_int, [_P]),
    "sty_model_bind_grad": (C.c_int, [_P, C.c_char_p, _P]),
    "sty_model_set_train_opts": (C.c_int, [_P, C.POINTER(TrainOpts)]),
    "sty_vocoder_train_workspace_bytes": (C.c_int, [_P, _I, _I, _SZP]),
    "sty_vocoder_fwd_train": (C.c_int, [_P, C.POINTER(VocoderIO), _P, C.c_size_t, _P]),
    "sty_vocoder_bwd": (C.c_int, [_P, _P, _P, _P, _P]),
    "sty_speech_train_workspace_bytes": (C.c_int, [_P, _I, _I, _I, _SZP]),
    "sty_speech_fwd_train": (C.c_int, [_P, C.POINTER(SpeechIO), _P, C.c_size_t, _P]),
    "sty_speech_bwd": (C.c_int, [_P, _P, _P, _P, _P]),
    "sty_speech_prepare_train": (C.c_int, [_P, _P]),
    "sty_speech_bwd_pe": (C.c_int, [_P, _P, _P, _P, _P, _P]),
    "sty_speech_d_style_ready": (C.c_int, [_P, _P]),
    "sty_speech_branch_stream": (C.c_int, [_P, C.POINTER(C.c_void_p)]),
    "sty_style_train_workspace_bytes": (C.c_int, [_P, _I, _I, _SZP]),
    "sty_style_fwd_train": (C.c_int, [_P, _I, _I, _P, _P, _P, C.c_size_t, _P]),
    "sty_style_prepare_train": (C.c_int, [_P, _P]),
    "sty_style_bwd": (C.c_int, [_P, _P, _P]),
    "sty_style_tap": (C.c_int, [_P, _I, _I, _P, C.POINTER(C.c_int), C.POINTER(C.c_int), C.POINTER(C.c_int), _P]),
    "sty_duration_workspace_bytes": (C.c_int, [_P, _I, _I, _SZP]),
    "sty_duration_fwd": (C.c_int, [_P, _I, _I, _P, _P, _P, _P, _P, C.c_size_t, _P]),
    "sty_pitch_energy_workspace_bytes": (C.c_int, [_P, _I, _I, _I, _SZP]),
    "sty_pitch_energy_fwd": (C.c_int, [_P, _I, _I, _I, _P, _P, _P, _P, _P, _P, _P, C.c_size_t, _P]),
    "sty_pitch_style_workspace_bytes": (C.c_int, [_P, _I, _I, _SZP]),
    "sty_pitch_style_fwd": (C.c_int, [_P, _I, _I, _P, _P, _P, _P, _P, C.c_size_t, _P]),
    "sty_conv1d_workspace_bytes": (C.c_int, [_I, _I, _I, _SZP]),
    "sty_conv1d_fwd": (C.c_int, [_I, _I, _I, _I, _I, _I, _P, _P, _P, _P, _P, C.c_size_t, _I, _P]),
    "sty_conv1d_bwd_workspace_bytes": (C.c_int, [_I, _I, _I, _I, _I, _SZP]),
    "sty_conv1d_bwd": (C.c_int, [_I, _I, _I, _I, _I, _I, _P, _P, _P, _P, _P, _P, _P, C.c_size_t, _I, _P]),
    "sty_partial_sum": (C.c_int, [_I, _P, _I, _I, _I, _P, _P, _P]),
    "sty_adamw_step": (C.c_int, [C.c_size_t, _P, _P, _P, _P, C.c_float, C.c_float, C.c_float, C.c_float, C.c_float,
                                 _I, C.c_float, _P]),
    "sty_adamw_step_scaled": (C.c_int, [C.c_size_t, _P, _P, _P, _P, C.c_double, _P, C.c_float, C.c_float, C.c_float,
                                        C.c_float, _I, C.c_float, _P]),
    "sty_disc_lr_track": (C.c_int, [_P, _P, C.c_double, C.c_double, C.c_double, C.c_double, C.c_double, _P]),
    "sty_model_set_grad_hook": (C.c_int, [_P, _P, _P]),
    "sty_acoustic_loss_workspace_bytes": (C.c_int, [_I, _I, _SZP]),
    "sty_acoustic_loss_target": (C.c_int, [_I, _I, _P, _P, C.c_size_t, _P]),
    "sty_acoustic_loss_fwd_bwd": (C.c_int, [_I, _I, _P, _P, C.c_float, C.c_float, _P, _P, _P, C.c_size_t, _P]),
    "sty_specdisc_workspace_bytes": (C.c_int, [_I, _I, _I, _I, _SZP]),
    "sty_specdisc_forward": (C.c_int, [_P, _I, _I, _I, _P, _P, _I, _P, C.c_size_t, _P]),
    "sty_specdisc_losses": (C.c_int, [_P, _I, _I, _I, _P, _P, C.c_float, _P, _P, C.c_float, _P, _P, _I, _P, C.c_size_t,
                                      _P]),
    "sty_prediction_to_duration": (C.c_int, [_I, _I, _I, _P, _P, _P, _P, _P]),
    "sty_duration_loss_fwd_bwd": (C.c_int, [_I, _I, _I, _P, _P, _P, _P, _P, _P, C.c_float, C.c_float, _P, _P, _P, _P,
                                            C.c_size_t, _P]),
    "sty_duration_train_workspace_bytes": (C.c_int, [_P, _I, _I, _SZP]),
    "sty_duration_fwd_train": (C.c_int, [_P, _I, _I, _P, _P, _P, _P, _P, C.c_size_t, _P]),
    "sty_duration_bwd": (C.c_int, [_P, _P, _P, _P]),
    "sty_pitch_loss_fwd_bwd": (C.c_int, [_I, _I, _P, _P, C.c_float, _I, _P, _P, _P, C.c_size_t, _P]),
    "sty_pitch_energy_train_workspace_bytes": (C.c_int, [_P, _I, _I, _I, _SZP]),
    "sty_pitch_energy_fwd_train": (C.c_int, [_P, _I, _I, _I, _P, _P, _P, _P, _P, _P, _P, C.c_size_t, _P]),
    "sty_pitch_energy_bwd": (C.c_int, [_P, _P, _P, _P, _P]),
    "sty_pitch_style_train_workspace_bytes": (C.c_int, [_P, _I, _I, _SZP]),
    "sty_pitch_style_fwd_train": (C.c_int, [_P, _I, _I, _P, _P, _P, _P, _P, C.c_size_t, _P]),
    "sty_pitchdisc_workspace_bytes": (C.c_int, [_I, _I, _I, _I, _I, _SZP]),
    "sty_pitchdisc_forward": (C.c_int, [_P, _I, _I, _I, _I, _P, _P, _P, C.c_size_t, _P]),
    "sty_pitchdisc_losses": (C.c_int, [_P, _I, _I, _I, _I, _P, _P, C.c_float, _P, _P, C.c_float, _P, _P, _P, C.c_size_t,
                                       _P]),
    "sty_cfdisc_workspace_bytes": (C.c_int, [_I, _I, _I, _SZP]),
    "sty_cfdisc_forward": (C.c_int, [_P, _I, _I, _P, _P, C.c_float, _I, _P, C.c_size_t, _P]),
    "sty_cfdisc_losses": (C.c_int, [_P, _I, _I, _P, _P, C.c_float, _P, _P, C.c_float, _P, _P, C.c_float, _I, _P,
                                    C.c_size_t, _P]),
    "sty_acoustic_gan_workspace_bytes": (C.c_int, [_I, _I, _I, _SZP]),
    "sty_acoustic_gan_loss_fwd_bwd": (C.c_int, [_I, _I, _P, _P, C.c_float, C.c_float, C.c_float, _P, C.c_float, _P, _I, _P,
                                                _P, _P, _P, C.c_size_t, _P, C.c_size_t, _I, _P]),
    "sty_comm_unique_id": (C.c_int, [_P]),
    "sty_comm_init": (C.c_int, [_P, _I, _I, _I, C.POINTER(C.c_void_p)]),
    "sty_comm_allreduce_bucket": (C.c_int, [_P, _P, C.c_size_t, _P]),
    "sty_comm_wait": (C.c_int, [_P, _P]),
    "sty_comm_set_stream": (C.c_int, [_P, _P]),
    "sty_comm_stats": (C.c_int, [_P, C.POINTER(C.c_uint64), C.POINTER(C.c_uint64), C.POINTER(C.c_double)]),
    "sty_comm_destroy": (C.c_int, [_P]),
    "sty_pack_accumulate": (C.c_int, [_I, _I, _I, _P, _P, _P, _P, _P]),
    "sty_pack_finalize": (C.c_int, [_I, _I, _P, _P, _P, _P, _P, _P]),
    "sty_aligner_workspace_bytes": (C.c_int, [_P, _I, _I, _SZP]),
    "sty_aligner_fwd": (C.c_int, [_P, _I, _I, _P, _P, _P, _P, C.c_size_t, _P]),
    "sty_forced_align_workspace_bytes": (C.c_int, [_I, _I, _I, _SZP]),
    "sty_forced_align": (C.c_int, [_I, _I, _I, _I, _P, _P, _P, _P, _I, _P, _P, _P, _P, C.c_size_t, _P]),
    "sty_aligner_train_workspace_bytes": (C.c_int, [_P, _I, _I, _SZP]),
    "sty_aligner_fwd_train": (C.c_int, [_P, _I, _I, _P, _P, C.c_float, C.c_uint, _P, _P, C.c_size_t, _P]),
    "sty_aligner_bwd": (C.c_int, [_P, _P, _P]),
    "sty_ctc_loss_workspace_bytes": (C.c_int, [_I, _I, _I, _I, _SZP]),
    "sty_ctc_loss_fwd_bwd": (C.c_int, [_I, _I, _I, _I, _P, _P, C.c_float, _P, _P, _P, _I, C.c_float, _P, _P, _P, _P, _P,
                                       C.c_size_t, _P]),
    "sty_prof_enable": (C.c_int, [_I]),
    "sty_prof_only": (C.c_int, [C.c_char_p]),
    "sty_set_single_stream": (C.c_int, [_I]),
    "sty_prof_report": (C.c_int, [_P, _I]),
}


class ProfRow(C.Structure):
    _fields_ = [("name", C.c_char * 48), ("inst", C.c_char * 144), ("launches", C.c_uint64), ("ms", C.c_double),
                ("flops", C.c_double), ("bytes", C.c_double)]


def prof_report(cap=64, by_inst=False):
    cap = max(cap, 4096)
    rows = (ProfRow * cap)()
    n = LIB.sty_prof_report(C.cast(rows, C.c_void_p), cap)
    if n < 0:
        check(n)
    raw = [dict(name=r.name.decode(), inst=r.inst.decode(), launches=int(r.launches), ms=r.ms, flops=r.flops, bytes=r.bytes)
           for r in rows[:min(n, cap)]]
    return raw if by_inst else group_families(raw)


def group_families(raw):
    fam = {}
    for r in raw:
        f = fam.setdefault(r["name"], dict(name=r["name"], launches=0, ms=0.0, flops=0.0, bytes=0.0, insts={}))
        for k in ("launches", "ms", "flops", "bytes"):
            f[k] += r[k]
        if r["inst"]:
            f["insts"][r["inst"]] = f["insts"].get(r["inst"], 0) + r["launches"]
    return list(fam.values())

GRAD_HOOK = C.CFUNCTYPE(None, C.c_void_p, C.c_int)

LIB = None


def load():
    global LIB
    if LIB is not None:
        return LIB
    if not os.path.exists(LIB_PATH):
        raise StyError(f"{LIB_PATH} not found: build it with `python __graft_entry__.py` (hipcc, gfx950). "
                       "There is no CPU fallback.")
    lib = C.CDLL(LIB_PATH)
    for name, (res, args) in SYMBOLS.items():
        fn = getattr(lib, name)
        fn.restype = res
        fn.argtypes = args
    LIB = lib
    return lib


def check(rc):
    if rc != 0:
        raise StyError(f"libstylish_hip: status {rc}: {LIB.sty_last_error().decode()}")


def ptr(t):
    return None if t is None else C.c_void_p(t.data_ptr())
```

Before: 395,500 frames/s.

## Defer GRN row-scale gradient into activation backward and fuse AdaIN stats

```diff
diff --git a/include/stylish_hip.h b/include/stylish_hip.h
--- a/include/stylish_hip.h
+++ b/include/stylish_hip.h
@@ -127,6 +127,13 @@
                    const float *lin_w, const float *lin_b, float *prior, void *workspace, size_t ws_bytes,
                    void *stream);
 int sty_source_workspace_bytes(int B, int T, size_t *bytes);
+int sty_grn_bwd_workspace_bytes(int B, int C4, int T, size_t *bytes);
+int sty_grn_bwd(int B, int C4, int T, const float *h, const float *ds, const float *gamma, int from_gx, float *coef,
+                float *dgamma, void *workspace, size_t ws_bytes, void *stream);
+int sty_act_bwd(int kind, int B, int C, int T, const float *x, float *dy, const float *alpha, const float *h,
+                const float *coef, int fused, float *dx, int accumulate, float *dalpha, void *stream);
+int sty_adain_finalize(int B, int C, int T, int nseg, const double *part, const float *gb, float eps, float *a, float *s,
+                       float *mean, float *rstd, void *stream);
 
 int sty_model_enable_training(sty_model *m);
 typedef struct {
diff --git a/stylish_tts_amd/csrc/api.hip b/stylish_tts_amd/csrc/api.hip
--- a/stylish_tts_amd/csrc/api.hip
+++ b/stylish_tts_amd/csrc/api.hip
@@ -2602,6 +2602,59 @@
   }
   return launch_partial_sum(dw_form, part, C, K, nblk, dw, db, S(stream));
 }
+static size_t grn_bwd_ws_bytes(int B, int C4, int T) {
+  return (size_t)B * C4 * row_stats_nseg(T) * 2 * sizeof(double) + (size_t)2 * B * C4 * sizeof(float);
+}
+int sty_grn_bwd_workspace_bytes(int B, int C4, int T, size_t* bytes) {
+  if (!bytes || B <= 0 || C4 <= 0 || T <= 0) {
+    set_error("sty_grn_bwd_workspace_bytes: bad argument");
+    return STY_EINVAL;
+  }
+  *bytes = grn_bwd_ws_bytes(B, C4, T);
+  return STY_OK;
+}
+int sty_grn_bwd(int B, int C4, int T, const float* h, const float* ds, const float* gamma, int from_gx, float* coef,
+                float* dgamma, void* workspace, size_t ws_bytes, void* stream) {
+  if (!h || !ds || !gamma || !coef || !dgamma || !workspace || B <= 0 || C4 <= 0 || T <= 0) {
+    set_error("sty_grn_bwd: bad argument");
+    return STY_EINVAL;
+  }
+  if (ws_bytes < grn_bwd_ws_bytes(B, C4, T)) {
+    set_error("sty_grn_bwd: workspace too small");
+    return STY_ENOMEM;
+  }
+  hipStream_t st = S(stream);
+  const int nseg = row_stats_nseg(T);
+  double* part = (double*)workspace;
+  float* scale = (float*)(part + (size_t)B * C4 * nseg * 2);
+  float* gx = scale + (size_t)B * C4;
+  int rc = launch_row_stats(h, B * C4, T, part, st);
+  if (rc) return rc;
+  if ((rc = launch_grn_finalize(part, nseg, gamma, B, C4, scale, st, gx))) return rc;
+  return launch_grn_bwd(from_gx ? gx : nullptr, part, nseg, gamma, ds, B, C4, coef, dgamma, st);
+}
+int sty_act_bwd(int kind, int B, int C, int T, const float* x, float* dy, const float* alpha, const float* h,
+                const float* coef, int fused, float* dx, int accumulate, float* dalpha, void* stream) {
+  if (!x || !dy || !dx || B <= 0 || C <= 0 || T <= 0 || (kind == ACT_SNAKE && !alpha) || ((h != nullptr) != (coef != nullptr))) {
+    set_error("sty_act_bwd: bad argument");
+    return STY_EINVAL;
+  }
+  hipStream_t st = S(stream);
+  if (h && !fused) {
+    const int rc = launch_row_scale_add(h, coef, 0.f, B * C, T, dy, st);
+    if (rc) return rc;
+    h = coef = nullptr;
+  }
+  return launch_act_bwd(kind, x, dy, alpha, B, C, T, dx, accumulate, dalpha, st, h, coef);
+}
+int sty_adain_finalize(int B, int C, int T, int nseg, const double* part, const float* gb, float eps, float* a, float* s,
+                       float* mean, float* rstd, void* stream) {
+  if (!part || !gb || !a || !s || B <= 0 || C <= 0 || T <= 0 || nseg <= 0 || ((mean != nullptr) != (rstd != nullptr))) {
+    set_error("sty_adain_finalize: bad argument");
+    return STY_EINVAL;
+  }
+  return launch_adain_finalize(part, nseg, gb, B, C, T, eps, a, s, S(stream), mean, rstd);
+}
 int sty_mel_workspace_bytes(int B, int N, int n_fft, int hop, size_t* bytes) {
   if (!bytes || B <= 0 || N <= n_fft / 2 || n_fft <= 0 || hop <= 0) {
     set_error("sty_mel_workspace_bytes: bad argument");
diff --git a/stylish_tts_amd/csrc/bwd.hip b/stylish_tts_amd/csrc/bwd.hip
--- a/stylish_tts_amd/csrc/bwd.hip
+++ b/stylish_tts_amd/csrc/bwd.hip
@@ -327,33 +327,6 @@
   return STY_OK;
 }
 
-__global__ __launch_bounds__(256) void adain_stats_kernel(const double* __restrict__ part, int nseg, int rows, int T,
-                                                          float eps, float* __restrict__ mean, float* __restrict__ rstd) {
-  const int i = blockIdx.x * 4 + (threadIdx.x >> 6), lane = threadIdx.x & 63;
-  if (i >= rows) return;
-  double sum = 0.0, sq = 0.0;
-  for (int k = lane; k < nseg; k += 64) {
-    sum += part[((size_t)i * nseg + k) * 2];
-    sq += part[((size_t)i * nseg + k) * 2 + 1];
-  }
-  for (int o = 32; o > 0; o >>= 1) {
-    sum += __shfl_xor(sum, o);
-    sq += __shfl_xor(sq, o);
-  }
-  if (lane) return;
-  const double m = sum / T;
-  double var = sq / T - m * m;
-  if (var < 0.0) var = 0.0;
-  mean[i] = (float)m;
-  rstd[i] = (float)(1.0 / sqrt(var + (double)eps));
-}
-int launch_adain_stats(const double* part, int nseg, int rows, int T, float eps, float* mean, float* rstd,
-                       hipStream_t st) {
-  hipLaunchKernelGGL(adain_stats_kernel, dim3(cdiv(rows, 4)), dim3(256), 0, st, part, nseg, rows, T, eps, mean, rstd);
-  STY_LAUNCH_CHECK();
-  return STY_OK;
-}
-
 template <int TC, int NR>
 __global__ __launch_bounds__(256) void chan_ln_bwd_dx_reg_kernel(const float* __restrict__ x, const float* __restrict__ dy,
                                                                  const float* __restrict__ y, int C, int T, float eps,
@@ -683,14 +656,16 @@
   return STY_OK;
 }
 
-__global__ __launch_bounds__(256) void grn_bwd_kernel(const double* __restrict__ part, int nseg,
+__global__ __launch_bounds__(256) void grn_bwd_kernel(const float* __restrict__ gx, const double* __restrict__ part, int nseg,
                                                       const float* __restrict__ gamma,
                                                       const float* __restrict__ ds, int C4,
                                                       float* __restrict__ coef, float* __restrict__ dgamma) {
   __shared__ float gxs[1024];
   __shared__ double red[2][4];
   const int b = blockIdx.x;
-  if (nseg < 32) {
+  if (gx) {
+    for (int c = threadIdx.x; c < C4; c += 256) gxs[c] = gx[(size_t)b * C4 + c];
+  } else if (nseg < 32) {
     for (int c = threadIdx.x; c < C4; c += 256) {
       double sq = 0.0;
       for (int k = 0; k < nseg; ++k) sq += part[(((size_t)b * C4 + c) * nseg + k) * 2 + 1];
@@ -730,13 +705,18 @@
     coef[(size_t)b * C4 + c] = gxs[c] > 0.f ? dgx / gxs[c] : 0.f;
   }
 }
-int launch_grn_bwd(const double* part, int nseg, const float* gamma, const float* ds, int B, int C4, float* coef,
-                   float* dgamma, hipStream_t st) {
+int launch_grn_bwd(const float* gx, const double* part, int nseg, const float* gamma, const float* ds, int B, int C4,
+                   float* coef, float* dgamma, hipStream_t st) {
   if (C4 > 1024) {
     set_error("grn_bwd: 4C > 1024");
     return STY_EINVAL;
   }
-  hipLaunchKernelGGL(grn_bwd_kernel, dim3(B), dim3(256), 0, st, part, nseg, gamma, ds, C4, coef, dgamma);
+  if (!gx && !part) {
+    set_error("grn_bwd: neither the forward's norms nor its partials");
+    return STY_EINVAL;
+  }
+  ProfScope prof("grn_bwd_kernel", 0.0, 4.0 * B * C4 * 4, st, gx ? "gx" : "part");
+  hipLaunchKernelGGL(grn_bwd_kernel, dim3(B), dim3(256), 0, st, gx, part, nseg, gamma, ds, C4, coef, dgamma);
   STY_LAUNCH_CHECK();
   return STY_OK;
 }
@@ -801,7 +781,8 @@
 __global__ __launch_bounds__(256) void act_bwd_kernel(int kind, const float* __restrict__ x,
                                                       const float* __restrict__ dy, const float* __restrict__ alpha,
                                                       int C, int T, float* __restrict__ dx, int accumulate,
-                                                      float* __restrict__ dalpha) {
+                                                      float* __restrict__ dalpha, const float* __restrict__ h,
+                                                      const float* __restrict__ coef) {
   __shared__ double red[1][4];
   const int c = blockIdx.x, b = blockIdx.y;
   double acc[1] = {0.0};
@@ -818,6 +799,7 @@
   }
   const size_t row = ((size_t)b * C + c) * T;
   const float al = kind == ACT_SNAKE ? alpha[c] : 1.f;
+  const float cf = h ? coef[(size_t)b * C + c] : 0.f;
   auto one = [&](float v, float d) -> float {
     float g = d;
     if (kind == ACT_RELU) g = v > 0.f ? d : 0.f;
@@ -838,12 +820,18 @@
     }
     return g;
   };
-  if ((T & 3) == 0 && ((((size_t)(x + row) | (size_t)(dy + row) | (size_t)(dx + row)) & 15) == 0)) {
+  if ((T & 3) == 0 && ((((size_t)(x + row) | (size_t)(dy + row) | (size_t)(dx + row) | (size_t)(h ? h + row : nullptr)) & 15) == 0)) {
     const float4* x4 = reinterpret_cast<const float4*>(x + row);
     const float4* d4 = reinterpret_cast<const float4*>(dy + row);
     float4* o4 = reinterpret_cast<float4*>(dx + row);
+    const float4* h4 = h ? reinterpret_cast<const float4*>(h + row) : nullptr;
     for (int t = threadIdx.x; t < T / 4; t += 256) {
-      const float4 v = x4[t], d = d4[t];
+      const float4 v = x4[t];
+      float4 d = d4[t];
+      if (h) {
+        const float4 hv = h4[t];
+        d = make_float4(fmaf(hv.x, cf, d.x), fmaf(hv.y, cf, d.y), fmaf(hv.z, cf, d.z), fmaf(hv.w, cf, d.w));
+      }
       float4 g;
       g.x = one(v.x, d.x);
       g.y = one(v.y, d.y);
@@ -857,7 +845,9 @@
     }
   } else
   for (int t = threadIdx.x; t < T; t += 256) {
-    const float v = x[row + t], d = dy[row + t];
+    const float v = x[row + t];
+    float d = dy[row + t];
+    if (h) d = fmaf(h[row + t], cf, d);
     float g = d;
     if (kind == ACT_RELU) g = v > 0.f ? d : 0.f;
     else if (kind == ACT_SWISH) {
@@ -883,8 +873,13 @@
   }
 }
 int launch_act_bwd(int kind, const float* x, const float* dy, const float* alpha, int B, int C, int T, float* dx,
-                   int accumulate, float* dalpha, hipStream_t st) {
-  hipLaunchKernelGGL(act_bwd_kernel, dim3(C, B), dim3(256), 0, st, kind, x, dy, alpha, C, T, dx, accumulate, dalpha);
+                   int accumulate, float* dalpha, hipStream_t st, const float* h, const float* coef) {
+  if (h && (kind == ACT_GLU || !coef)) {
+    set_error("act_bwd: a row term needs its coefficients and a one-to-one activation");
+    return STY_EINVAL;
+  }
+  ProfScope prof("act_bwd_kernel", 0.0, 4.0 * B * C * T * (3.0 + (accumulate ? 1 : 0) + (h ? 1 : 0)), st, h ? "row term" : nullptr);
+  hipLaunchKernelGGL(act_bwd_kernel, dim3(C, B), dim3(256), 0, st, kind, x, dy, alpha, C, T, dx, accumulate, dalpha, h, coef);
   STY_LAUNCH_CHECK();
   return STY_OK;
 }
@@ -910,6 +905,7 @@
   reinterpret_cast<float4*>(dst)[idx] = d;
 }
 int launch_row_scale_add(const float* src, const float* coef, float k, int rows, int T, float* dst, hipStream_t st) {
+  ProfScope prof(coef ? "row_scale_add_kernel[coef]" : "row_scale_add_kernel", 0.0, 12.0 * rows * T, st);
   const size_t n4 = (size_t)rows * (T / 4);
   if (vec4_ok(n4, T, src, dst)) {
     hipLaunchKernelGGL(row_scale_add4_kernel, dim3((unsigned)((n4 + 255) / 256)), dim3(256), 0, st, src, coef, k,
diff --git a/stylish_tts_amd/csrc/model.h b/stylish_tts_amd/csrc/model.h
--- a/stylish_tts_amd/csrc/model.h
+++ b/stylish_tts_amd/csrc/model.h
@@ -262,19 +262,17 @@
 int launch_pro_bwd_adain(const void* u, int uh, const void* x, int xh, int B, int C, int T, const float* pa, const float* ps,
                          const float* alpha, const float* mean, const float* rstd, const float* gb, void* dx, int dh,
                          int accumulate, float* dgb, float* dalpha, int hw, hipStream_t st, const void* dsrc = nullptr);
-int launch_adain_stats(const double* part, int nseg, int rows, int T, float eps, float* mean, float* rstd,
-                       hipStream_t st);
 int launch_cast_f32_to_16(const float* x, size_t n, void* y16, hipStream_t st);
 int launch_cast_16_to_f32(const void* x16, size_t n, float* y, hipStream_t st);
 bool chan_ln32_eligible(int B, int C, int T, int relu);
 int launch_chan_ln_bwd(const float* x, const float* dy, const float* y, int B, int C, int T, float eps, int ada,
                        const float* w, const float* gb, int relu, const float* out_mask, float* dx, int accumulate,
                        float* mu_tmp, float* r_tmp, float* dgb, float* dw, float* db, hipStream_t st, int h16 = 0);
-int launch_grn_bwd(const double* part, int nseg, const float* gamma, const float* ds, int B, int C4, float* coef,
-                   float* dgamma, hipStream_t st);
+int launch_grn_bwd(const float* gx, const double* part, int nseg, const float* gamma, const float* ds, int B, int C4,
+                   float* coef, float* dgamma, hipStream_t st);
 int launch_act_fwd(int kind, const float* x, const float* alpha, int B, int C, int T, float* y, hipStream_t st);
 int launch_act_bwd(int kind, const float* x, const float* dy, const float* alpha, int B, int C, int T, float* dx,
-                   int accumulate, float* dalpha, hipStream_t st);
+                   int accumulate, float* dalpha, hipStream_t st, const float* h = nullptr, const float* coef = nullptr);
 int launch_row_scale_add(const float* src, const float* coef, float k, int rows, int T, float* dst, hipStream_t st);
 int launch_dwconv_fwd(const float* x, const float* w, const float* bias, int B, int C, int T, int K, int pad, float* y,
                       hipStream_t st);
diff --git a/stylish_tts_amd/csrc/norms.hip b/stylish_tts_amd/csrc/norms.hip
--- a/stylish_tts_amd/csrc/norms.hip
+++ b/stylish_tts_amd/csrc/norms.hip
@@ -70,7 +70,8 @@
 
 __global__ __launch_bounds__(256) void adain_finalize_kernel(const double* __restrict__ part, int nseg,
                                                              const float* __restrict__ gb, int B, int C, int T, float eps,
-                                                             float* __restrict__ a, float* __restrict__ s) {
+                                                             float* __restrict__ a, float* __restrict__ s,
+                                                             float* __restrict__ mean_out, float* __restrict__ rstd_out) {
   const int i = blockIdx.x * 4 + (threadIdx.x >> 6), lane = threadIdx.x & 63;
   if (i >= B * C) return;
   const int b = i / C, c = i % C;
@@ -92,18 +93,23 @@
   const float av = g * rstd;
   a[i] = av;
   s[i] = be - av * (float)mean;
+  if (mean_out) {
+    mean_out[i] = (float)mean;
+    rstd_out[i] = rstd;
+  }
 }
 
 int launch_adain_finalize(const double* part, int nseg, const float* gb, int B, int C, int T, float eps, float* a,
-                          float* s, hipStream_t st) {
-  hipLaunchKernelGGL(adain_finalize_kernel, dim3(cdiv(B * C, 4)), dim3(256), 0, st, part, nseg, gb, B, C, T, eps, a, s);
+                          float* s, hipStream_t st, float* mean, float* rstd) {
+  hipLaunchKernelGGL(adain_finalize_kernel, dim3(cdiv(B * C, 4)), dim3(256), 0, st, part, nseg, gb, B, C, T, eps, a, s, mean,
+                     rstd);
   STY_LAUNCH_CHECK();
   return STY_OK;
 }
 
 __global__ __launch_bounds__(1024) void grn_finalize_kernel(const double* __restrict__ part, int nseg, int G,
                                                             const float* __restrict__ gamma, int C4,
-                                                            float* __restrict__ scale) {
+                                                            float* __restrict__ scale, float* __restrict__ gx_out) {
   __shared__ float red[16];
   __shared__ float gxs[1024];
   const int b = blockIdx.x, wave = threadIdx.x >> 6, lane = threadIdx.x & 63;
@@ -120,6 +126,7 @@
     if (gl == 0 && c < C4) {
       const float gx = (float)sqrt(sq);
       gxs[c] = gx;
+      if (gx_out) gx_out[(size_t)b * C4 + c] = gx;
       loc += gx;
     }
   }
@@ -134,14 +141,14 @@
 }
 
 int launch_grn_finalize(const double* part, int nseg, const float* gamma, int B, int C4, float* scale,
-                        hipStream_t st) {
+                        hipStream_t st, float* gx) {
   if (C4 > 1024) {
     set_error("grn_finalize: 4C = %d > 1024", C4);
     return STY_EINVAL;
   }
   int G = 1;
   while (G < 64 && G < nseg) G <<= 1;
-  hipLaunchKernelGGL(grn_finalize_kernel, dim3(B), dim3(1024), 0, st, part, nseg, G, gamma, C4, scale);
+  hipLaunchKernelGGL(grn_finalize_kernel, dim3(B), dim3(1024), 0, st, part, nseg, G, gamma, C4, scale, gx);
   STY_LAUNCH_CHECK();
   return STY_OK;
 }
diff --git a/stylish_tts_amd/csrc/sty_common.h b/stylish_tts_amd/csrc/sty_common.h
--- a/stylish_tts_amd/csrc/sty_common.h
+++ b/stylish_tts_amd/csrc/sty_common.h
@@ -273,8 +273,9 @@
 int row_stats_nseg(int T);
 int launch_row_stats(const float* x, int rows, int T, double* part, hipStream_t st);
 int launch_adain_finalize(const double* part, int nseg, const float* gb, int B, int C, int T, float eps, float* a,
-                          float* s, hipStream_t st);
-int launch_grn_finalize(const double* part, int nseg, const float* gamma, int B, int C4, float* scale, hipStream_t st);
+                          float* s, hipStream_t st, float* mean = nullptr, float* rstd = nullptr);
+int launch_grn_finalize(const double* part, int nseg, const float* gamma, int B, int C4, float* scale, hipStream_t st,
+                        float* gx = nullptr);
 int launch_chan_layernorm(const float* x, float* y, int B, int C, int T, float eps, int ada, const float* w,
                           const float* bvec, const float* gb, int relu, const float* out_mask, hipStream_t st);
 int launch_embedding(const int64_t* tokens, const float* emb, int B, int L, int H, int ntok, float scale, float* y,
diff --git a/stylish_tts_amd/csrc/train.hip b/stylish_tts_amd/csrc/train.hip
--- a/stylish_tts_amd/csrc/train.hip
+++ b/stylish_tts_amd/csrc/train.hip
@@ -57,6 +57,7 @@
     g_no_fp32.clear();
     lazy_mask.clear();
     pend_up.clear();
+    pend_row.clear();
     nograd.clear();
     half_.clear();
     g16_ok.clear();
@@ -142,6 +143,7 @@
     }
     if (br_end) (void)hipStreamWaitEvent(st, br_end, 0);
     while (flush_up && rc == STY_OK && !pend_up.empty()) up_flush(pend_up.begin()->first);
+    while (rc == STY_OK && !pend_row.empty()) row_flush(pend_row.begin()->first);
     side_join();
     if (fc && rc == STY_OK) style_fc_backward();
   }
@@ -373,8 +375,29 @@
     chk(launch_pro_bwd(PRO_LRELU, g, C, 0, act, B, C, n, nullptr, nullptr, C, 0, nullptr, nullptr, g, 0, nullptr, nullptr,
                        nullptr, st));
   }
-  float* G(const float* act, size_t n, bool raw = false, bool keep_lazy = false) {
+  struct PendRow {
+    const float* coef;
+    int rows, T;
+  };
+  std::unordered_map<const float*, PendRow> pend_row;
+  void row_flush(const float* act) {
+    auto it = pend_row.find(act);
+    if (it == pend_row.end()) return;
+    const PendRow p = it->second;
+    pend_row.erase(it);
+    float* g = G(act, (size_t)p.rows * p.T);
+    if (live()) chk(launch_row_scale_add(act, p.coef, 0.f, p.rows, p.T, g, st));
+  }
+  const float* take_row(const float* act) {
+    auto it = pend_row.find(act);
+    if (it == pend_row.end()) return nullptr;
+    const float* coef = it->second.coef;
+    pend_row.erase(it);
+    return coef;
+  }
+  float* G(const float* act, size_t n, bool raw = false, bool keep_lazy = false, bool keep_row = false) {
     if (!pend_up.empty()) up_flush(act);
+    if (!keep_row && !pend_row.empty()) row_flush(act);
     if (!raw && !ungated.empty()) gate_flush(act);
     if (!keep_lazy && !lazy_mask.empty()) mask_flush(act);
     auto it = gmap.find(act);
@@ -393,6 +416,7 @@
   }
   float* Gw(const float* act, size_t n, int& acc) {
     if (!pend_up.empty()) up_flush(act);
+    if (!pend_row.empty()) row_flush(act);
     if (!ungated.empty()) gate_flush(act);
     if (mask_pending(act)) {
       tw_g.erase(lazy_mask[act].dst);
@@ -649,11 +673,12 @@
     if (live()) chk(launch_act_fwd(kind, x, alpha, B, C, Tt, y, st));
     tape.push_back([=]() {
       const int Cin = kind == ACT_GLU ? 2 * C : C;
-      float* gY = G(y, (size_t)B * C * Tt);
+      float* gY = G(y, (size_t)B * C * Tt, false, false, kind != ACT_GLU);
+      const float* row = take_row(y);
       int acc = 1;
       float* gX = Gw(x, (size_t)B * Cin * Tt, acc);
       float* dal = kind == ACT_SNAKE ? PG(alpha, C) : nullptr;
-      if (live()) chk(launch_act_bwd(kind, x, gY, alpha, B, C, Tt, gX, acc, dal, st));
+      if (live()) chk(launch_act_bwd(kind, x, gY, alpha, B, C, Tt, gX, acc, dal, st, row ? y : nullptr, row));
     });
     return y;
   }
@@ -741,10 +766,7 @@
       if (live()) chk(launch_row_stats(x, B * C, Tt, p2, st));
       part = p2;
     }
-    if (live()) {
-      chk(launch_adain_finalize(part, nseg, gbp(fc), B, C, Tt, 1e-5f, a, s, st));
-      chk(launch_adain_stats(part, nseg, B * C, Tt, 1e-5f, mean, rstd, st));
-    }
+    if (live()) chk(launch_adain_finalize(part, nseg, gbp(fc), B, C, Tt, 1e-5f, a, s, st, mean, rstd));
     const float* gbl = gbp(fc);
     float* dgl = dgbp(fc);
     float* aa = a;
@@ -810,6 +832,7 @@
     const size_t n32 = (size_t)B * 32 * Tt, n128 = (size_t)B * 128 * Tt;
     double* part = take<double>((size_t)B * 128 * nt * 2);
     float* scale = take<float>((size_t)B * 128);
+    float* gxn = take<float>((size_t)B * 128);
     float* y = take<float>(n32);
     const bool lean = m->topts.compute_bf16 && Tt % 8 == 0 && getenv("STY_NO_WGRADB") == nullptr &&
                       getenv("STY_NO_CNX_LEAN") == nullptr;
@@ -835,7 +858,7 @@
       a.bf16 = m->topts.compute_bf16;
       a.h16 = h16;
       chk(launch_convnext32(a, B, 1, st));
-      chk(launch_grn_finalize(part, nt, c.grn_gamma, B, 128, scale, st));
+      chk(launch_grn_finalize(part, nt, c.grn_gamma, B, 128, scale, st, gxn));
       chk(launch_convnext32(a, B, 2, st));
     }
     if (lean && grad16_stream_on()) g16_ok.insert(y);
@@ -942,7 +965,7 @@
         if (live()) {
           chk(launch_wgrad_cnx(1, h16, gY, B, Tt, pM, 1, st, 1, gy16));
           chk(launch_cnx_m_finish(pM, B, SB, c.w2_raw, scale, ds, frozen ? nullptr : gw2, frozen ? nullptr : gb2, st));
-          chk(launch_grn_bwd(part, nt, c.grn_gamma, ds, B, 128, coef, PG(c.grn_gamma, 128), st));
+          chk(launch_grn_bwd(gxn, nullptr, 0, c.grn_gamma, ds, B, 128, coef, PG(c.grn_gamma, 128), st));
           chk(launch_convnext32_bwd(a, B, 2, st));
           chk(launch_cnx_partial_sum(pgb, B, 64, nt_b, 2, dgl, st));
         }
@@ -952,7 +975,7 @@
         a1.ntiles = nt;
         chk(launch_convnext32_bwd(a1, B, 1, st));
         chk(launch_cnx_partial_sum(pds, B, 128, nt, 0, ds, st));
-        chk(launch_grn_bwd(part, nt, c.grn_gamma, ds, B, 128, coef, PG(c.grn_gamma, 128), st));
+        chk(launch_grn_bwd(gxn, nullptr, 0, c.grn_gamma, ds, B, 128, coef, PG(c.grn_gamma, 128), st));
         chk(launch_convnext32_bwd(a, B, 2, st));
         chk(launch_cnx_partial_sum(pds, B, 128, nt_b, 1, dal, st));
         chk(launch_cnx_partial_sum(pgb, B, 64, nt_b, 2, dgl, st));
@@ -1021,21 +1044,18 @@
     const int nseg = row_stats_nseg(Tt);
     double* part = take<double>((size_t)B * 4 * C * nseg * 2);
     float* scale = take<float>((size_t)B * 4 * C);
+    float* gxn = take<float>((size_t)B * 4 * C);
     if (live()) {
       chk(launch_row_stats(h, B * 4 * C, Tt, part, st));
-      chk(launch_grn_finalize(part, nseg, c.grn_gamma, B, 4 * C, scale, st));
+      chk(launch_grn_finalize(part, nseg, c.grn_gamma, B, 4 * C, scale, st, gxn));
     }
     const float* gamma = c.grn_gamma;
     tape.push_back([=]() {
       float* dsc = G(scale, (size_t)B * 4 * C);
-      float* gH = G(h, (size_t)B * 4 * C * Tt);
-      const size_t mark = ws.off;
+      G(h, (size_t)B * 4 * C * Tt);
       float* coef = take<float>((size_t)B * 4 * C);
-      if (live()) {
-        chk(launch_grn_bwd(part, nseg, gamma, dsc, B, 4 * C, coef, PG(gamma, 4 * C), st));
-        chk(launch_row_scale_add(h, coef, 0.f, B * 4 * C, Tt, gH, st));
-      }
-      ws.off = mark;
+      if (live()) chk(launch_grn_bwd(gxn, nullptr, 0, gamma, dsc, B, 4 * C, coef, PG(gamma, 4 * C), st));
+      pend_row[h] = PendRow{coef, B * 4 * C, Tt};
     });
     float* y = take<float>((size_t)B * C * Tt);
     ConvArgs b2 = base(c.pw2, h, Tt, y);
diff --git a/stylish_tts_amd/lib.py b/stylish_tts_amd/lib.py
--- a/stylish_tts_amd/lib.py
+++ b/stylish_tts_amd/lib.py
@@ -111,6 +111,10 @@
     "sty_conv1d_bwd_workspace_bytes": (C.c_int, [_I, _I, _I, _I, _I, _SZP]),
     "sty_conv1d_bwd": (C.c_int, [_I, _I, _I, _I, _I, _I, _P, _P, _P, _P, _P, _P, _P, C.c_size_t, _I, _P]),
     "sty_partial_sum": (C.c_int, [_I, _P, _I, _I, _I, _P, _P, _P]),
+    "sty_grn_bwd_workspace_bytes": (C.c_int, [_I, _I, _I, _SZP]),
+    "sty_grn_bwd": (C.c_int, [_I, _I, _I, _P, _P, _P, _I, _P, _P, _P, C.c_size_t, _P]),
+    "sty_act_bwd": (C.c_int, [_I, _I, _I, _I, _P, _P, _P, _P, _P, _I, _P, _I, _P, _P]),
+    "sty_adain_finalize": (C.c_int, [_I, _I, _I, _I, _P, _P, C.c_float, _P, _P, _P, _P, _P]),
     "sty_adamw_step": (C.c_int, [C.c_size_t, _P, _P, _P, _P, C.c_float, C.c_float, C.c_float, C.c_float, C.c_float,
                                  _I, C.c_float, _P]),
     "sty_adamw_step_scaled": (C.c_int, [C.c_size_t, _P, _P, _P, _P, C.c_double, _P, C.c_float, C.c_float, C.c_float,
```

Result: faster. 399,800 frames/s (median of 6 runs) (+1.1%).
